# myscale/MyScaleDB

Hardware: NVIDIA B200
Metric: QPS @ recall@10>=0.95 (exact: recall 1.0), FLAT brute-force IP top-10, 10M x 768-d bf16, batch 1024 (higher is better)
Workload: dtype bf16

## Files before the change

include/b200_search.h:

```cpp
#ifndef B200_SEARCH_H
#define B200_SEARCH_H

#include <stddef.h>
#include <stdint.h>

#ifdef __cplusplus
extern "C" {
#endif

#define B200_OK 0
#define B200_ERR_INVALID 1
#define B200_ERR_CUDA 2
#define B200_ERR_UNSUPPORTED 3
#define B200_ERR_NO_DEVICE 4
#define B200_ERR_NOMEM 5
#define B200_ERR_NOT_FOUND 6

#define B200_METRIC_L2 0
#define B200_METRIC_IP 1
#define B200_METRIC_COSINE 2
#define B200_METRIC_HAMMING 3
#define B200_METRIC_JACCARD 4

#define B200_DTYPE_F32 0
#define B200_DTYPE_BF16 1
#define B200_DTYPE_BIN 2

const char *b200_last_error(void);
const char *b200_version(void);
int b200_device_count(int *out_n);
int b200_set_device(int device);

int b200_flat_knn(int metric, const float *x, int64_t nx, const float *y, int64_t ny, int d, int k,
                  const uint8_t *alive_bits , float *out_dis, int64_t *out_ids);

int b200_binary_knn(int metric, const uint8_t *x, int64_t nx, const uint8_t *y, int64_t ny, int nbytes, int k,
                    const uint8_t *alive_bits , float *out_dis, int64_t *out_ids);

int b200_part_scan(int metric, const void *x, int64_t nx, const void *y, int64_t ny, int d, int k,
                   int64_t block_rows, const uint8_t *row_exists , const uint8_t *filter_bits ,
                   float *out_dis, int64_t *out_ids);

typedef struct b200_corpus b200_corpus;

int b200_corpus_create(int metric, int dtype, int d, int64_t capacity_rows, b200_corpus **out);
int b200_corpus_append(b200_corpus *c, const void *rows, int64_t n);
int b200_corpus_adopt_device(b200_corpus *c, const void *device_rows, int64_t n);
int b200_corpus_size(const b200_corpus *c, int64_t *out_rows);
int b200_corpus_free(b200_corpus *c);

int b200_corpus_search(b200_corpus *c, const float *queries, int64_t nq, int k, const uint8_t *alive_bits ,
                       float *out_dis, int64_t *out_ids);
int b200_corpus_search_device(b200_corpus *c, const float *d_queries, int64_t nq, int k,
                              const uint8_t *d_alive_bits , int64_t id_offset, float *d_out_dis,
                              int64_t *d_out_ids, void *stream);
int b200_corpus_set_path(b200_corpus *c, int path);
#define B200_KERNEL_SCAN 1
#define B200_KERNEL_GEMM_BF16 2
#define B200_KERNEL_GEMM_TS 3
#define B200_KERNEL_GEMM_TF32X3 4
int b200_corpus_last_variant(b200_corpus *c, int *kernel, int *cta_group, int *pairs_per_cluster, int *grid);
int b200_corpus_enable_timing(b200_corpus *c, int on);
int b200_corpus_kernel_time(b200_corpus *c, int reset, double *out_total_ms, int64_t *out_launches);
int64_t b200_launch_count(int reset);
int b200_thread_release(void);

int b200_topk_merge_device(const float *d_dis, const int64_t *d_ids, int n_lists, int64_t nq, int k, int descending,
                           float *d_out_dis, int64_t *d_out_ids, void *stream);

int b200_topk_merge_device_strided(const float *d_dis, const int64_t *d_ids, int n_lists, int64_t dis_list_stride,
                                   int64_t ids_list_stride, int64_t nq, int k, int descending, float *d_out_dis,
                                   int64_t *d_out_ids, void *stream);
int b200_topk_merge_device_ex(const float *d_dis, const int64_t *d_ids, int n_lists, int64_t dis_list_stride,
                              int64_t ids_list_stride, int64_t nq, int k_in, int k, int descending, int tie_mode,
                              float *d_out_dis, int64_t *d_out_ids, int32_t *d_out_list , void *stream);

typedef struct b200_index b200_index;
int b200_index_create(const char *type, int metric, int d, const char *params, b200_index **out);
int b200_index_build(b200_index *ix, const float *rows, int64_t n);
int b200_index_reserve(b200_index *ix, int64_t total_rows);
int b200_index_train(b200_index *ix, const float *rows, int64_t n);
int b200_index_train_device(b200_index *ix, const float *d_rows, int64_t n);
int b200_index_add(b200_index *ix, const float *rows, int64_t n);
int b200_index_add_device(b200_index *ix, const float *d_rows, int64_t n);
int b200_index_finalize(b200_index *ix);
int b200_index_info(const b200_index *ix, int64_t *n, int *nlist, int *m, int *uses_ivf);
int b200_index_search(b200_index *ix, const float *queries, int64_t nq, int k, const char *params, int first_stage_only,
                      const uint8_t *alive_bits , float *out_dis, int64_t *out_ids, int64_t *out_num_candidates);
int b200_index_search_device(b200_index *ix, const float *d_queries, int64_t nq, int k, const char *params, int first_stage_only,
                             const uint8_t *d_alive_bits , int64_t id_offset, float *d_out_dis, int64_t *d_out_ids,
                             void *stream);
int b200_index_phase_ms(b200_index *ix, double out_ms[5]);
int b200_index_list_sizes(const b200_index *ix, uint32_t *out_sizes , int capacity);
int b200_index_enable_timing(b200_index *ix, int on);
int b200_index_last_scan(b200_index *ix, int64_t *rows_streamed, int64_t *payload_row_bytes, int64_t *work_items,
                         double *kernel_ms_total, int64_t *kernel_launches, int reset);
int b200_index_refine(b200_index *ix, const float *queries, int64_t nq, const int64_t *cand_ids, int64_t ncand, int k,
                      float *out_dis, int64_t *out_ids);
int b200_index_save(b200_index *ix, const char *path);
int b200_index_load(const char *path, b200_index **out);
int b200_index_save_cb(b200_index *ix, int (*write)(void *ctx, const void *data, size_t bytes), void *ctx);
int b200_index_load_cb(int (*read)(void *ctx, void *data, size_t bytes), void *ctx, b200_index **out);
int b200_index_free(b200_index *ix);

typedef struct b200_comm b200_comm;
int b200_comm_unique_id(const char *nccl_lib_path , void *out_id_128_bytes);
int b200_comm_create(const char *nccl_lib_path , const void *unique_id_128_bytes, int rank, int world, b200_comm **out);
int b200_comm_info(const b200_comm *c, int *rank, int *world);
int b200_comm_free(b200_comm *c);
int b200_comm_local_buffers(b200_comm *c, int64_t nq, int k, float **d_dis, int64_t **d_ids);
int b200_comm_gather_merge(b200_comm *c, int64_t nq, int k, int descending, float *d_out_dis, int64_t *d_out_ids, void *stream);
int b200_comm_gather_merge_host(b200_comm *c, const float *h_dis, const int64_t *h_ids, int64_t nq, int k, int descending,
                                float *h_out_dis, int64_t *h_out_ids);
int b200_comm_allreduce_sum_u64(b200_comm *c, uint64_t *host_counters, int64_t n);
int b200_sharded_corpus_search(b200_comm *cm, b200_corpus *corpus, const float *d_queries, int64_t nq, int k,
                               const uint8_t *d_alive_bits , int64_t id_offset, float *d_out_dis, int64_t *d_out_ids,
                               void *stream, int use_graph);
int b200_sharded_corpus_search_host(b200_comm *cm, b200_corpus *corpus, const float *queries, int64_t nq, int d, int k,
                                    int64_t id_offset, float *out_dis, int64_t *out_ids, void *stream, int use_graph);
int b200_sharded_index_search(b200_comm *cm, b200_index *ix, int metric, const float *d_queries, int64_t nq, int k, const char *params,
                              const uint8_t *d_alive_bits , int64_t id_offset, float *d_out_dis, int64_t *d_out_ids,
                              void *stream);

#define B200_CACHE_CORPUS 0
#define B200_CACHE_INDEX 1
#define B200_CACHE_BM25 2
#define B200_CACHE_OPAQUE 3
int b200_cache_set_capacity(uint64_t bytes);
int b200_cache_get(const char *key, void **handle, int *kind);
int b200_cache_put(const char *key, int kind, void *handle, uint64_t bytes, void **resident);
int b200_cache_put_opaque(const char *key, void *handle, uint64_t bytes, void (*deleter)(void *), void **resident);
int b200_cache_release_handle(const char *key, const void *handle);
int b200_cache_release(const char *key);
int b200_cache_expire(const char *key);
int b200_cache_expire_prefix(const char *prefix, int64_t *out_removed);
int b200_cache_stats(uint64_t *capacity, uint64_t *used, uint64_t *items, uint64_t *hits, uint64_t *misses,
                     uint64_t *evictions);
int b200_corpus_memory_bytes(const b200_corpus *c, uint64_t *out_bytes);
int b200_index_memory_bytes(const b200_index *ix, uint64_t *out_bytes);

int b200_bitmap_from_offsets_device(const uint64_t *d_offsets, int64_t n, int64_t nbits, uint8_t *d_out_bits, void *stream);
int b200_bitmap_from_row_exists_device(const uint8_t *d_row_exists, int64_t n, uint8_t *d_out_bits, void *stream);
int b200_bitmap_and_device(const uint8_t *d_a, const uint8_t *d_b, int64_t nbits, uint8_t *d_out, void *stream);
int b200_bitmap_and(const uint8_t *a, const uint8_t *b, int64_t nbits, uint8_t *out);
int b200_real_bitmap(const uint8_t *filter_bits, int64_t n_new_rows, const uint64_t *inverted_row_ids_map,
                     const uint8_t *inverted_row_sources_map, uint32_t own_id, int64_t total_vec, uint8_t *out_bits);
int b200_remap_labels(const uint64_t *row_ids_map, int64_t map_len, int64_t *labels, int64_t n);
int b200_transfer_to_old_row_ids(const int64_t *new_ids, const float *new_dis, int64_t num_candidates,
                                 const uint64_t *inverted_row_ids_map, const uint8_t *inverted_row_sources_map, int64_t map_len,
                                 uint32_t own_id, int64_t *out_ids, float *out_dis, int64_t *out_n);

typedef struct b200_bm25 b200_bm25;
int b200_bm25_create(uint32_t n_fields, b200_bm25 **out);
int b200_bm25_free(b200_bm25 *ix);
int b200_bm25_add_doc(b200_bm25 *ix, uint64_t row_id);
int b200_bm25_add_text(b200_bm25 *ix, uint32_t field, const char *text);
int b200_bm25_commit(b200_bm25 *ix);
int b200_bm25_save(b200_bm25 *ix, const char *path);
int b200_bm25_load(const char *path, b200_bm25 **out);
int b200_bm25_total_docs(const b200_bm25 *ix, uint64_t *out);
int b200_bm25_total_tokens(const b200_bm25 *ix, uint32_t field, uint64_t *out);
int b200_bm25_doc_freq(const b200_bm25 *ix, uint32_t field, const char *term, uint64_t *out);
int b200_bm25_query_terms(const char *sentence, char *buf, size_t buf_len, uint32_t *out_n);
int b200_bm25_search(b200_bm25 *ix, const char *sentence, const uint32_t *fields, uint32_t n_fields_q, uint32_t topk,
                     const uint8_t *alive_bits , int use_filter, int operator_or, uint64_t stat_total_docs,
                     const uint64_t *stat_total_tokens, const uint64_t *stat_doc_freq, uint64_t *out_rows,
                     float *out_scores, uint32_t *out_n);
int b200_bm25_last_timing(b200_bm25 *ix, double *kernel_ms, double *call_ms, uint64_t *postings);
int b200_bm25_search_batch(b200_bm25 *ix, const char *const *sentences, int64_t nq, const uint32_t *fields,
                           uint32_t n_fields_q, uint32_t topk, const uint8_t *alive_bits, int use_filter, int operator_or,
                           uint64_t stat_total_docs, const uint64_t *stat_total_tokens, const uint64_t *stat_doc_freq,
                           uint64_t *out_rows , float *out_scores, uint32_t *out_counts );

int b200_hybrid_fusion_batch(int fusion_type, int64_t nq, const uint32_t *vec_shard, const uint64_t *vec_part,
                             const uint64_t *vec_label, const float *vec_score, const uint32_t *vec_count, int64_t vec_stride,
                             const uint32_t *txt_shard, const uint64_t *txt_part, const uint64_t *txt_label,
                             const float *txt_score, const uint32_t *txt_count, int64_t txt_stride, float fusion_weight,
                             uint64_t fusion_k, int vector_scan_direction, uint32_t top_k, uint32_t *out_shard,
                             uint64_t *out_part, uint64_t *out_label, float *out_score, uint32_t *out_count);

#ifdef __cplusplus
}
#endif
#endif
```

myscaledb_b200/csrc/capi.cu:

```cuda
#include <algorithm>
#include <cstdlib>
#include <cstring>
#include <mutex>
#include <vector>

#include "common.cuh"
#include "kernels.h"

namespace b200 {

thread_local std::string g_error;
thread_local int64_t g_launches = 0;

void set_error(const std::string &msg) { g_error = msg; }
int fail(int code, const std::string &msg) {
    g_error = msg;
    return code;
}

static int ensure_device() {
    int n = 0;
    cudaError_t e = cudaGetDeviceCount(&n);
    if (e != cudaSuccess || n == 0) {
        cudaGetLastError();
        return fail(B200_ERR_NO_DEVICE, std::string("no CUDA device visible (") +
                                            (e != cudaSuccess ? cudaGetErrorString(e) : "count = 0") +
                                            "); libb200search has no CPU fallback");
    }
    int dev = 0;
    B200_CUDA_OK(cudaGetDevice(&dev));
    int major = 0;
    B200_CUDA_OK(cudaDeviceGetAttribute(&major, cudaDevAttrComputeCapabilityMajor, dev));
    if (major != 10)
        return fail(B200_ERR_NO_DEVICE, "device compute capability major is " + std::to_string(major) +
                                            "; this library carries sm_100a code only");
    return B200_OK;
}

static int num_sms() {
    int dev = 0, n = 148;
    if (cudaGetDevice(&dev) == cudaSuccess) cudaDeviceGetAttribute(&n, cudaDevAttrMultiProcessorCount, dev);
    return n;
}

struct DevBuf {
    void *p = nullptr;
    size_t cap = 0;
    int reserve(size_t bytes) {
        if (bytes <= cap) return B200_OK;
        if (p) cudaFree(p);
        p = nullptr;
        cap = 0;
        size_t want = bytes + bytes / 4 + 256;
        cudaError_t e = cudaMalloc(&p, want);
        if (e != cudaSuccess) {
            cudaGetLastError();
            return fail(B200_ERR_NOMEM, "cudaMalloc(" + std::to_string(want) + ") failed: " + cudaGetErrorString(e));
        }
        cap = want;
        return B200_OK;
    }
    void release() {
        if (p) cudaFree(p);
        p = nullptr;
        cap = 0;
    }
    template <typename T>
    T *as() {
        return reinterpret_cast<T *>(p);
    }
};

}

using namespace b200;

struct b200_corpus {
    int metric = 0, dtype = 0, d = 0, d_pad = 0;
    int64_t cap = 0, n = 0;
    int64_t row_bytes = 0;
    void *data = nullptr;
    size_t data_cap_bytes = 0;
    int64_t side_cap_rows = 0;
    bool owns = true;
    float *row_scale = nullptr;
    float *row_bias = nullptr;
    int device = 0;
    int path = 0;
    int gemm_cta_group = 0;
    int sms = 148;
    cudaStream_t stream = nullptr;
    std::mutex mu;
    DevBuf w_raw, w_q32, w_qbf, w_qlo, w_qnorm, w_pk, w_pi, w_lk, w_li, w_alive, w_odis, w_oids, w_stage, w_prog;
    int sync_slack = 2;
    void *h_pin = nullptr;
    size_t h_pin_bytes = 0;
    unsigned int *d_tickets = nullptr;
    unsigned int fused_seq = 0;
    int d_tickets_d = 0;
    int fused_enabled = 1;
    int rescore_l2 = 1;
    int gemm_multicast = 1;
    int gemm_ts = 0;
    int last_cg = 0, last_mc = 0, last_ts = 0, last_grid = 0, last_kernel = 0;
    bool timing = false;
    std::vector<std::pair<cudaEvent_t, cudaEvent_t>> ev_used, ev_free;
    double timed_ms = 0;
    int64_t timed_launches = 0;
};

static void timing_begin(b200_corpus *c, cudaStream_t s, std::pair<cudaEvent_t, cudaEvent_t> &ev) {
    if (!c->timing) return;
    if (c->ev_free.empty()) {
        cudaEventCreate(&ev.first);
        cudaEventCreate(&ev.second);
    } else {
        ev = c->ev_free.back();
        c->ev_free.pop_back();
    }
    cudaEventRecord(ev.first, s);
}
static void timing_drain(b200_corpus *c) {
    for (auto &ev : c->ev_used) {
        float ms = 0;
        if (cudaEventSynchronize(ev.second) == cudaSuccess && cudaEventElapsedTime(&ms, ev.first, ev.second) == cudaSuccess) {
            c->timed_ms += ms;
            c->timed_launches++;
        }
        c->ev_free.push_back(ev);
    }
    c->ev_used.clear();
}
static void timing_end(b200_corpus *c, cudaStream_t s, std::pair<cudaEvent_t, cudaEvent_t> &ev) {
    if (!c->timing) return;
    cudaEventRecord(ev.second, s);
    c->ev_used.push_back(ev);
    if (c->ev_used.size() >= 1024) timing_drain(c);
}

static int corpus_alloc(b200_corpus *c, int64_t rows);
static int corpus_norms(b200_corpus *c, int64_t first, int64_t n);

namespace b200 {
int corpus_metric(const b200_corpus *c) { return c->metric; }
bool corpus_timing_enabled(const b200_corpus *c) { return c->timing; }
const void *corpus_device_rows(const b200_corpus *c) { return c->data; }
int corpus_append_device(b200_corpus *c, const float *d_rows, int64_t n, cudaStream_t s) {
    if (!c || (!d_rows && n > 0) || n < 0) return fail(B200_ERR_INVALID, "bad arguments");
    if (c->dtype == B200_DTYPE_BIN) return fail(B200_ERR_UNSUPPORTED, "device append: float corpora only");
    if (n == 0) return B200_OK;
    std::lock_guard<std::mutex> lk(c->mu);
    B200_CUDA_OK(cudaSetDevice(c->device));
    B200_TRY(corpus_alloc(c, std::max(c->n + n, c->cap)));
    char *dst = reinterpret_cast<char *>(c->data) + c->n * c->row_bytes;
    if (c->dtype == B200_DTYPE_BF16) B200_CUDA_OK(launch_f32_to_bf16_rows(d_rows, c->d, dst, c->d_pad, n, s));
    else B200_CUDA_OK(launch_pad_rows_f32(d_rows, c->d, reinterpret_cast<float *>(dst), c->d_pad, n, s));
    B200_CUDA_OK(cudaStreamSynchronize(s));
    B200_TRY(corpus_norms(c, c->n, n));
    B200_CUDA_OK(cudaStreamSynchronize(c->stream));
    c->n += n;
    return B200_OK;
}
int corpus_normalize_rows(b200_corpus *c) {
    if (c->dtype != B200_DTYPE_F32) return fail(B200_ERR_UNSUPPORTED, "normalise: fp32 corpora only");
    B200_CUDA_OK(cudaSetDevice(c->device));
    B200_CUDA_OK(launch_normalize_rows_f32(reinterpret_cast<float *>(c->data), c->d_pad, c->n, c->stream));
    B200_CUDA_OK(cudaStreamSynchronize(c->stream));
    return B200_OK;
}
}

static bool is_float_metric(int m) { return m == B200_METRIC_L2 || m == B200_METRIC_IP || m == B200_METRIC_COSINE; }
static bool is_bin_metric(int m) { return m == B200_METRIC_HAMMING || m == B200_METRIC_JACCARD; }

static int pad_for(int dtype, int d) {
    if (dtype == B200_DTYPE_BF16) return (int)round_up(d, 64);
    if (dtype == B200_DTYPE_F32) return (int)round_up(d, 4);
    return d / 8;
}

extern "C" const char *b200_last_error(void) { return g_error.c_str(); }
extern "C" const char *b200_version(void) { return "b200search 0.1 (sm_100a)"; }

extern "C" int b200_device_count(int *out_n) {
    if (!out_n) return fail(B200_ERR_INVALID, "out_n is null");
    int n = 0;
    if (cudaGetDeviceCount(&n) != cudaSuccess) {
        cudaGetLastError();
        n = 0;
    }
    *out_n = n;
    return B200_OK;
}

extern "C" int b200_set_device(int device) {
    B200_TRY(ensure_device());
    B200_CUDA_OK(cudaSetDevice(device));
    return B200_OK;
}

extern "C" int64_t b200_launch_count(int reset) {
    int64_t v = g_launches;
    if (reset) g_launches = 0;
    return v;
}

extern "C" int b200_corpus_create(int metric, int dtype, int d, int64_t capacity_rows, b200_corpus **out) {
    if (!out) return fail(B200_ERR_INVALID, "out is null");
    *out = nullptr;
    if (d <= 0 || capacity_rows < 0) return fail(B200_ERR_INVALID, "bad d / capacity");
    if (dtype == B200_DTYPE_BIN) {
        if (!is_bin_metric(metric)) return fail(B200_ERR_INVALID, "binary corpus needs HAMMING or JACCARD");
        if (d % 8) return fail(B200_ERR_INVALID, "binary dimension must be a multiple of 8 bits");
    } else if (dtype == B200_DTYPE_F32 || dtype == B200_DTYPE_BF16) {
        if (!is_float_metric(metric)) return fail(B200_ERR_INVALID, "float corpus needs L2, IP or COSINE");
    } else {
        return fail(B200_ERR_INVALID, "unknown dtype");
    }
    B200_TRY(ensure_device());
    b200_corpus *c = new b200_corpus();
    c->metric = metric;
    c->dtype = dtype;
    c->d = d;
    c->d_pad = pad_for(dtype, d);
    c->row_bytes = dtype == B200_DTYPE_BIN ? c->d_pad : (int64_t)c->d_pad * (dtype == B200_DTYPE_BF16 ? 2 : 4);
    c->cap = capacity_rows;
    cudaGetDevice(&c->device);
    c->sms = num_sms();
    if (const char *ev = getenv("B200_GEMM_SYNC_SLACK")) c->sync_slack = atoi(ev);
    if (const char *ev = getenv("B200_GEMM_RESCORE_L2")) c->rescore_l2 = atoi(ev);
    if (const char *ev = getenv("B200_FUSED_SCAN")) c->fused_enabled = atoi(ev);
    if (const char *ev = getenv("B200_GEMM_TS")) c->gemm_ts = atoi(ev);
    if (const char *ev = getenv("B200_GEMM_MULTICAST")) c->gemm_multicast = atoi(ev);
    cudaError_t e = cudaStreamCreateWithFlags(&c->stream, cudaStreamNonBlocking);
    if (e != cudaSuccess) {
        delete c;
        return fail(B200_ERR_CUDA, std::string("cudaStreamCreate: ") + cudaGetErrorString(e));
    }
    *out = c;
    return B200_OK;
}

static int corpus_alloc(b200_corpus *c, int64_t rows) {
    if (c->data && !c->owns) return fail(B200_ERR_INVALID, "corpus adopted device memory; cannot append");
    const size_t need = (size_t)(rows + 1) * c->row_bytes + 256;
    const bool want_scale = c->metric == B200_METRIC_COSINE, want_bias = c->metric == B200_METRIC_L2;
    if (!c->data || c->data_cap_bytes < need) {
        void *nd = nullptr;
        cudaError_t e = cudaMalloc(&nd, need);
        if (e != cudaSuccess) {
            cudaGetLastError();
            return fail(B200_ERR_NOMEM, std::string("cudaMalloc corpus: ") + cudaGetErrorString(e));
        }
        if (c->data && c->n) {
            cudaMemcpyAsync(nd, c->data, (size_t)c->n * c->row_bytes, cudaMemcpyDeviceToDevice, c->stream);
            cudaStreamSynchronize(c->stream);
        }
        if (c->data) cudaFree(c->data);
        c->data = nd;
        c->data_cap_bytes = need;
    }
    if ((want_scale && (!c->row_scale || c->side_cap_rows < rows)) || (want_bias && (!c->row_bias || c->side_cap_rows < rows))) {
        float *ns = nullptr, *nb = nullptr;
        if (want_scale && cudaMalloc(&ns, (size_t)rows * 4 + 256) != cudaSuccess) return fail(B200_ERR_NOMEM, "cudaMalloc row_scale");
        if (want_bias && cudaMalloc(&nb, (size_t)rows * 4 + 256) != cudaSuccess) return fail(B200_ERR_NOMEM, "cudaMalloc row_bias");
        if (c->n) {
            if (ns && c->row_scale) cudaMemcpyAsync(ns, c->row_scale, (size_t)c->n * 4, cudaMemcpyDeviceToDevice, c->stream);
            if (nb && c->row_bias) cudaMemcpyAsync(nb, c->row_bias, (size_t)c->n * 4, cudaMemcpyDeviceToDevice, c->stream);
            cudaStreamSynchronize(c->stream);
        }
        if (c->row_scale) cudaFree(c->row_scale);
        if (c->row_bias) cudaFree(c->row_bias);
        c->row_scale = ns;
        c->row_bias = nb;
        c->side_cap_rows = rows;
    }
    c->cap = std::max(c->cap, rows);
    c->owns = true;
    return B200_OK;
}

static int corpus_norms(b200_corpus *c, int64_t first, int64_t n) {
    const char *rows = reinterpret_cast<const char *>(c->data) + first * c->row_bytes;
    if (c->metric == B200_METRIC_COSINE)
        B200_CUDA_OK(launch_row_norms(rows, c->dtype == B200_DTYPE_BF16, c->d_pad, n, 1, c->row_scale + first, c->stream));
    if (c->metric == B200_METRIC_L2)
        B200_CUDA_OK(launch_row_norms(rows, c->dtype == B200_DTYPE_BF16, c->d_pad, n, 0, c->row_bias + first, c->stream));
    return B200_OK;
}

extern "C" int b200_corpus_append(b200_corpus *c, const void *rows, int64_t n) {
    if (!c || (!rows && n > 0) || n < 0) return fail(B200_ERR_INVALID, "bad arguments");
    if (n == 0) return B200_OK;
    std::lock_guard<std::mutex> lk(c->mu);
    B200_CUDA_OK(cudaSetDevice(c->device));
    B200_TRY(corpus_alloc(c, std::max(c->n + n, c->cap)));
    char *dst = reinterpret_cast<char *>(c->data) + c->n * c->row_bytes;
    if (c->dtype == B200_DTYPE_BIN || (c->dtype == B200_DTYPE_F32 && c->d == c->d_pad)) {
        B200_TRY(staged_h2d(dst, rows, (size_t)n * c->row_bytes, c->device, c->stream));
    } else {
        const int64_t chunk = std::max<int64_t>(1, (int64_t)(256ll << 20) / ((int64_t)c->d * 4));
        for (int64_t off = 0; off < n; off += chunk) {
            const int64_t m = std::min(chunk, n - off);
            B200_TRY(c->w_raw.reserve((size_t)m * c->d * 4));
            B200_TRY(staged_h2d(c->w_raw.p, reinterpret_cast<const float *>(rows) + off * c->d, (size_t)m * c->d * 4, c->device,
                                c->stream));
            char *dd = dst + off * c->row_bytes;
            if (c->dtype == B200_DTYPE_BF16)
                B200_CUDA_OK(launch_f32_to_bf16_rows(c->w_raw.as<float>(), c->d, dd, c->d_pad, m, c->stream));
            else
                B200_CUDA_OK(launch_pad_rows_f32(c->w_raw.as<float>(), c->d, reinterpret_cast<float *>(dd), c->d_pad, m, c->stream));
            B200_CUDA_OK(cudaStreamSynchronize(c->stream));
        }
    }
    if (c->dtype != B200_DTYPE_BIN) B200_TRY(corpus_norms(c, c->n, n));
    B200_CUDA_OK(cudaStreamSynchronize(c->stream));
    c->n += n;
    return B200_OK;
}

extern "C" int b200_corpus_memory_bytes(const b200_corpus *c, uint64_t *out_bytes) {
    if (!c || !out_bytes) return fail(B200_ERR_INVALID, "bad arguments");
    uint64_t b = c->owns ? (uint64_t)c->data_cap_bytes : (uint64_t)c->n * (uint64_t)c->row_bytes;
    if (c->row_scale) b += (uint64_t)std::max(c->side_cap_rows, c->n) * 4;
    if (c->row_bias) b += (uint64_t)std::max(c->side_cap_rows, c->n) * 4;
    *out_bytes = b;
    return B200_OK;
}

extern "C" int b200_corpus_adopt_device(b200_corpus *c, const void *device_rows, int64_t n) {
    if (!c || !device_rows || n < 0) return fail(B200_ERR_INVALID, "bad arguments");
    std::lock_guard<std::mutex> lk(c->mu);
    if (c->data) return fail(B200_ERR_INVALID, "corpus already holds data");
    if (c->dtype != B200_DTYPE_BIN && c->d != c->d_pad)
        return fail(B200_ERR_INVALID, "adopted rows must already be padded (d % 64 == 0 for bf16, d % 4 == 0 for f32)");
    B200_CUDA_OK(cudaSetDevice(c->device));
    c->data = const_cast<void *>(device_rows);
    c->owns = false;
    c->n = n;
    c->cap = n;
    if (c->metric == B200_METRIC_COSINE) B200_CUDA_OK(cudaMalloc(&c->row_scale, (size_t)n * 4 + 256));
    if (c->metric == B200_METRIC_L2) B200_CUDA_OK(cudaMalloc(&c->row_bias, (size_t)n * 4 + 256));
    c->side_cap_rows = n;
    if (c->dtype != B200_DTYPE_BIN) B200_TRY(corpus_norms(c, 0, n));
    B200_CUDA_OK(cudaStreamSynchronize(c->stream));
    return B200_OK;
}

extern "C" int b200_corpus_size(const b200_corpus *c, int64_t *out_rows) {
    if (!c || !out_rows) return fail(B200_ERR_INVALID, "null argument");
    *out_rows = c->n;
    return B200_OK;
}

namespace b200 {
int list_cap_for(int k) {
    static const int min_k = getenv("B200_LIST_APPEND_MIN_K") ? atoi(getenv("B200_LIST_APPEND_MIN_K")) : 0;
    static const int tourn_k = getenv("B200_LIST_TOURN_MIN_K") ? atoi(getenv("B200_LIST_TOURN_MIN_K")) : 17;
    if (min_k > 0 && k >= min_k) return list_cap_append(k);
    if (tourn_k > 0 && k >= tourn_k) return list_cap_tourn(k);
    return k;
}
}

extern "C" int b200_corpus_set_path(b200_corpus *c, int path) {
    if (!c || path < 0 || path > 7) return fail(B200_ERR_INVALID, "path must be 0..7");
    std::lock_guard<std::mutex> lk(c->mu);
    c->path = path >= 2 ? 2 : path;
    c->gemm_cta_group = path == 3 ? 1 : 0;
    c->gemm_ts = path == 7 ? 2 : 0;
    c->gemm_multicast = path == 4 ? 0 : path == 5 ? 2 : 1;
    if (path == 0) {
        if (const char *ev = getenv("B200_GEMM_TS")) c->gemm_ts = atoi(ev);
        if (const char *ev = getenv("B200_GEMM_MULTICAST")) c->gemm_multicast = atoi(ev);
    }
    return B200_OK;
}

extern "C" int b200_corpus_last_variant(b200_corpus *c, int *kernel, int *cta_group, int *pairs_per_cluster, int *grid) {
    if (!c) return fail(B200_ERR_INVALID, "null corpus");
    std::lock_guard<std::mutex> lk(c->mu);
    if (kernel) *kernel = c->last_kernel;
    if (cta_group) *cta_group = c->last_cg;
    if (pairs_per_cluster) *pairs_per_cluster = c->last_mc;
    if (grid) *grid = c->last_grid;
    return B200_OK;
}

extern "C" int b200_corpus_enable_timing(b200_corpus *c, int on) {
    if (!c) return fail(B200_ERR_INVALID, "null corpus");
    std::lock_guard<std::mutex> lk(c->mu);
    c->timing = on != 0;
    return B200_OK;
}

extern "C" int b200_corpus_kernel_time(b200_corpus *c, int reset, double *out_total_ms, int64_t *out_launches) {
    if (!c || !out_total_ms || !out_launches) return fail(B200_ERR_INVALID, "null argument");
    std::lock_guard<std::mutex> lk(c->mu);
    B200_CUDA_OK(cudaSetDevice(c->device));
    timing_drain(c);
    *out_total_ms = c->timed_ms;
    *out_launches = c->timed_launches;
    if (reset) {
        c->timed_ms = 0;
        c->timed_launches = 0;
    }
    return B200_OK;
}

extern "C" int b200_corpus_free(b200_corpus *c) {
    if (!c) return B200_OK;
    cudaSetDevice(c->device);
    if (c->stream) cudaStreamSynchronize(c->stream);
    if (c->data && c->owns) cudaFree(c->data);
    if (c->row_scale) cudaFree(c->row_scale);
    if (c->row_bias) cudaFree(c->row_bias);
    if (c->h_pin) cudaFreeHost(c->h_pin);
    if (c->d_tickets) cudaFree(c->d_tickets);
    for (DevBuf *b : {&c->w_raw, &c->w_q32, &c->w_qbf, &c->w_qlo, &c->w_qnorm, &c->w_pk, &c->w_pi, &c->w_lk, &c->w_li, &c->w_alive,
                      &c->w_odis, &c->w_oids, &c->w_stage, &c->w_prog})
        b->release();
    for (auto *v : {&c->ev_used, &c->ev_free})
        for (auto &ev : *v) {
            cudaEventDestroy(ev.first);
            cudaEventDestroy(ev.second);
        }
    if (c->stream) cudaStreamDestroy(c->stream);
    delete c;
    return B200_OK;
}

static int search_core(b200_corpus *c, const void *d_queries, int64_t nq, int k, const uint8_t *d_alive, int64_t id_offset,
                       int ip_min_quirk, float *d_out_dis, int64_t *d_out_ids, cudaStream_t s) {
    if (k <= 0) return fail(B200_ERR_INVALID, "k must be positive");
    if (nq == 0) return B200_OK;
    if (c->n >= (int64_t)0xffffffffll) return fail(B200_ERR_UNSUPPORTED, "corpus shards are limited to 2^32 - 1 rows");
    const int sms = c->sms;

    if (c->dtype == B200_DTYPE_BIN) {
        if (k > 1024) return fail(B200_ERR_UNSUPPORTED, "k > 1024 not supported on the binary scan path");
        int blocks_x = (int)std::min<int64_t>(std::max<int64_t>(1, ceil_div(c->n, 256)), std::max<int64_t>(1, (2 * sms) / std::max<int64_t>(1, std::min<int64_t>(nq, 2 * sms))));
        B200_TRY(c->w_pk.reserve((size_t)nq * blocks_x * k * 4));
        B200_TRY(c->w_pi.reserve((size_t)nq * blocks_x * k * 4));
        BinaryScanParams bp{};
        bp.corpus = reinterpret_cast<const uint8_t *>(c->data);
        bp.queries = reinterpret_cast<const uint8_t *>(d_queries);
        bp.alive = d_alive;
        bp.part_keys = c->w_pk.as<float>();
        bp.part_ids = c->w_pi.as<uint32_t>();
        bp.n = c->n;
        bp.nq = nq;
        bp.nbytes = c->d_pad;
        bp.k = k;
        bp.jaccard = c->metric == B200_METRIC_JACCARD;
        B200_CUDA_OK(launch_binary_scan(bp, blocks_x, s));
        MergeParams mp{};
        mp.in_keys = bp.part_keys;
        mp.in_ids = bp.part_ids;
        mp.list_stride = k;
        mp.q_stride = (int64_t)blocks_x * k;
        mp.n_lists = blocks_x;
        mp.k_in = k;
        mp.k = k;
        mp.nq = nq;
        mp.out_mode = kOutKey;
        mp.id_offset = id_offset;
        mp.out_dis = d_out_dis;
        mp.out_ids = d_out_ids;
        B200_CUDA_OK(launch_topk_merge(mp, false, s));
        return B200_OK;
    }

    B200_TRY(c->w_q32.reserve((size_t)nq * c->d_pad * 4));
    float *q32 = c->w_q32.as<float>();
    B200_CUDA_OK(launch_pad_rows_f32(reinterpret_cast<const float *>(d_queries), c->d, q32, c->d_pad, nq, s));
    int path = c->path;
    if (path == 0) {
        const int64_t min_nq = c->metric == B200_METRIC_L2 ? 20 : (c->dtype == B200_DTYPE_BF16 ? 2 : 5);
        path = (nq >= min_nq && k <= (c->dtype == B200_DTYPE_BF16 ? 1024 : 256)) ? 2 : 1;
    }
    if (c->n == 0) path = 1;
    if (c->metric == B200_METRIC_COSINE && path == 1) B200_CUDA_OK(launch_normalize_rows_f32(q32, c->d_pad, nq, s));

    const int out_mode_scan = c->metric == B200_METRIC_L2 ? kOutKey : c->metric == B200_METRIC_IP ? kOutNeg : kOutOnePlus;

    if (path == 1) {
        if (k > 2048) return fail(B200_ERR_UNSUPPORTED, "k > 2048 not supported on the scan path");
        int qt = nq == 1 ? 1 : nq <= 4 ? 4 : 8;
        while (qt > 1 && scan_smem_bytes(qt, c->d_pad, k) > 100 * 1024) qt = qt == 8 ? 4 : 1;
        if (scan_smem_bytes(qt, c->d_pad, k) > 200 * 1024)
            return fail(B200_ERR_UNSUPPORTED, "d * 4 + 64 * k exceeds the shared-memory budget of the scan kernel");
        const int elems = c->dtype == B200_DTYPE_BF16 ? 8 : 4;
        const int chunks = c->d_pad / elems;
        int group = 1;
        while (group < 32 && group < chunks) group <<= 1;
        const int64_t y_tiles = ceil_div(nq, qt);
        const int64_t rows_per_block_step = 8 * (32 / group);
        int64_t bx = std::max<int64_t>(1, (2 * sms) / std::min<int64_t>(y_tiles, 2 * sms));
        bx = std::min<int64_t>(bx, std::max<int64_t>(1, ceil_div(c->n, rows_per_block_step)));
        const int blocks_x = (int)bx;
        B200_TRY(c->w_pk.reserve((size_t)nq * blocks_x * k * 4));
        B200_TRY(c->w_pi.reserve((size_t)nq * blocks_x * k * 4));
        ScanParams sp{};
        sp.corpus = c->data;
        sp.queries = q32;
        sp.row_scale = c->metric == B200_METRIC_COSINE ? c->row_scale : nullptr;
        sp.alive = d_alive;
        sp.part_keys = c->w_pk.as<float>();
        sp.part_ids = c->w_pi.as<uint32_t>();
        sp.n = c->n;
        sp.nq = nq;
        sp.row_bytes = c->row_bytes;
        sp.d_pad = c->d_pad;
        sp.k = k;
        sp.group = group;
        sp.l2 = c->metric == B200_METRIC_L2;
        sp.bf16 = c->dtype == B200_DTYPE_BF16;
        std::pair<cudaEvent_t, cudaEvent_t> ev;
        timing_begin(c, s, ev);
        B200_CUDA_OK(launch_flat_scan(sp, qt, blocks_x, s));
        timing_end(c, s, ev);
        c->last_kernel = B200_KERNEL_SCAN; c->last_cg = 0; c->last_mc = 0; c->last_grid = blocks_x;
        MergeParams mp{};
        mp.in_keys = sp.part_keys;
        mp.in_ids = sp.part_ids;
        mp.list_stride = k;
        mp.q_stride = (int64_t)blocks_x * k;
        mp.n_lists = blocks_x;
        mp.k_in = k;
        mp.k = k;
        mp.nq = nq;
        mp.out_mode = out_mode_scan;
        mp.ip_min_quirk = ip_min_quirk && c->metric == B200_METRIC_IP;
        mp.id_offset = id_offset;
        mp.out_dis = d_out_dis;
        mp.out_ids = d_out_ids;
        B200_CUDA_OK(launch_topk_merge(mp, false, s));
        return B200_OK;
    }

    if (k > 1024) return fail(B200_ERR_UNSUPPORTED, "k > 1024 not supported on the GEMM path");
    const int64_t QCHUNK = 1024;
    for (int64_t qb = 0; qb < nq; qb += QCHUNK) {
        const int64_t nq_c = std::min(QCHUNK, nq - qb);
        const bool f32 = c->dtype == B200_DTYPE_F32;
        const int cta_group = (nq_c > 128 && c->gemm_cta_group != 1) ? 2 : 1;
        const int nq_pad = (int)round_up(nq_c, 128 * cta_group);
        const int q_tiles = nq_pad / 128;
        if (f32) {
            B200_TRY(c->w_qbf.reserve((size_t)nq_pad * c->d_pad * 4));
            B200_TRY(c->w_qlo.reserve((size_t)nq_pad * c->d_pad * 4));
            B200_CUDA_OK(launch_split_tf32(q32 + qb * c->d_pad, nq_c, c->d_pad, c->w_qbf.as<float>(), c->w_qlo.as<float>(), nq_pad, s));
        } else {
            B200_TRY(c->w_qbf.reserve((size_t)nq_pad * c->d_pad * 2));
            B200_CUDA_OK(cudaMemsetAsync(c->w_qbf.p, 0, (size_t)nq_pad * c->d_pad * 2, s));
            B200_CUDA_OK(launch_f32_to_bf16_rows(q32 + qb * c->d_pad, c->d_pad, c->w_qbf.p, c->d_pad, nq_c, s));
        }
        const float *q_add = nullptr;
        if (c->metric == B200_METRIC_L2 || c->metric == B200_METRIC_COSINE) {
            B200_TRY(c->w_qnorm.reserve((size_t)nq_pad * 4));
            if (f32)
                B200_CUDA_OK(launch_row_norms(q32 + qb * c->d_pad, 0, c->d_pad, nq_c, c->metric == B200_METRIC_L2 ? 0 : 1,
                                              c->w_qnorm.as<float>(), s));
            else
                B200_CUDA_OK(launch_row_norms(c->w_qbf.p, 1, c->d_pad, nq_c, c->metric == B200_METRIC_L2 ? 0 : 1,
                                              c->w_qnorm.as<float>(), s));
            q_add = c->w_qnorm.as<float>();
        }
        int pairs = 1;
        if (cta_group == 2 && c->gemm_multicast && !f32) {
            const int want = c->gemm_multicast == 1 ? 4 : c->gemm_multicast;
            if (want >= 4 && q_tiles % 8 == 0) pairs = 4;
            else if (want >= 2 && q_tiles % 4 == 0) pairs = 2;
        }
        int grid = gemm_topk_grid(q_tiles, c->n, sms);
        while (pairs > 1) {
            const int maxc = gemm_topk_max_clusters(2, pairs, k);
            const int groups = q_tiles / (2 * pairs);
            const int per_group = maxc / groups;
            if (per_group >= 1) {
                grid = std::min(grid, per_group * groups * 2 * pairs);
                break;
            }
            pairs /= 2;
        }
        grid = (grid / q_tiles) * q_tiles;
        if (grid < q_tiles) grid = q_tiles;
        B200_TRY(c->w_pk.reserve((size_t)grid * 128 * k * 4));
        B200_TRY(c->w_pi.reserve((size_t)grid * 128 * k * 4));
        GemmTopkParams gp{};
        gp.corpus_bf16 = c->data;
        gp.queries_bf16 = c->w_qbf.p;
        gp.queries_lo = f32 ? c->w_qlo.p : nullptr;
        gp.row_scale = c->metric == B200_METRIC_COSINE ? c->row_scale : nullptr;
        gp.scale_const = c->metric == B200_METRIC_L2 ? -2.f : -1.f;
        gp.row_bias = c->metric == B200_METRIC_L2 ? c->row_bias : nullptr;
        gp.alive = d_alive;
        gp.part_keys = c->w_pk.as<float>();
        gp.part_ids = c->w_pi.as<uint32_t>();
        {
            B200_TRY(c->w_lk.reserve((size_t)grid * 128 * list_cap_for(k) * 4));
            B200_TRY(c->w_li.reserve((size_t)grid * 128 * list_cap_for(k) * 4));
            gp.list_keys_gmem = c->w_lk.as<float>();
            gp.list_ids_gmem = c->w_li.as<uint32_t>();
        }
        gp.n = c->n;
        gp.nq_pad = nq_pad;
        gp.nq_valid = (int)nq_c;
        gp.d_pad = c->d_pad;
        gp.k = k;
        gp.q_tiles = q_tiles;
        gp.cta_group = cta_group;
        gp.pairs_per_cluster = pairs;
        if (const char *dv = getenv("B200_GEMM_DEBUG")) gp.debug = atoi(dv);
        if (q_tiles > cta_group && c->sync_slack > 0) {
            B200_TRY(c->w_prog.reserve((size_t)grid * 4));
            B200_CUDA_OK(cudaMemsetAsync(c->w_prog.p, 0, (size_t)grid * 4, s));
            gp.progress = c->w_prog.as<int>();
            gp.sync_slack = c->sync_slack;
        }
        const char *detail = nullptr;
        std::pair<cudaEvent_t, cudaEvent_t> ev;
        timing_begin(c, s, ev);
        const bool use_ts = !f32 && cta_group == 2 && k <= 30 && gemm_topk_ts_supported(c->d_pad, q_tiles) &&
                            (c->gemm_ts == 2 || (c->gemm_ts == 1 && c->d_pad <= 512));
        cudaError_t e = f32 ? launch_gemm3_topk(gp, grid, s, &detail)
                            : use_ts ? launch_gemm_topk_ts(gp, grid, s, &detail) : launch_gemm_topk(gp, grid, s, &detail);
        timing_end(c, s, ev);
        c->last_kernel = f32 ? B200_KERNEL_GEMM_TF32X3 : use_ts ? B200_KERNEL_GEMM_TS : B200_KERNEL_GEMM_BF16;
        c->last_cg = cta_group; c->last_mc = (f32 || use_ts) ? 1 : pairs; c->last_grid = grid;
        if (e != cudaSuccess)
            return fail(B200_ERR_CUDA, std::string("gemm_topk launch: ") + (detail ? detail : cudaGetErrorString(e)));
        MergeParams mp{};
        mp.in_keys = gp.part_keys;
        mp.in_ids = gp.part_ids;
        mp.list_stride = (int64_t)nq_pad * k;
        mp.q_stride = k;
        mp.n_lists = grid / q_tiles;
        mp.k_in = k;
        mp.k = k;
        mp.nq = nq_c;
        mp.out_mode = c->metric == B200_METRIC_L2 ? kOutAddQ : c->metric == B200_METRIC_IP ? kOutNeg : kOutCosQ;
        mp.q_add = q_add;
        mp.ip_min_quirk = ip_min_quirk && c->metric == B200_METRIC_IP;
        mp.id_offset = id_offset;
        mp.out_dis = d_out_dis + qb * k;
        mp.out_ids = d_out_ids + qb * k;
        B200_CUDA_OK(launch_topk_merge(mp, false, s));
        if (c->metric == B200_METRIC_L2 && k <= 1024 && c->rescore_l2)
            B200_CUDA_OK(launch_rescore_l2(c->data, c->dtype == B200_DTYPE_BF16, c->row_bytes, c->d_pad, q32 + qb * c->d_pad, nq_c, id_offset, k,
                                           d_out_dis + qb * k, d_out_ids + qb * k, s));
    }
    return B200_OK;
}

extern "C" int b200_corpus_search_device(b200_corpus *c, const float *d_queries, int64_t nq, int k,
                                         const uint8_t *d_alive_bits, int64_t id_offset, float *d_out_dis,
                                         int64_t *d_out_ids, void *stream) {
    if (!c || (!d_queries && nq > 0) || !d_out_dis || !d_out_ids || nq < 0)
        return fail(B200_ERR_INVALID, "bad arguments");
    std::lock_guard<std::mutex> lk(c->mu);
    B200_CUDA_OK(cudaSetDevice(c->device));
    cudaStream_t s = stream ? reinterpret_cast<cudaStream_t>(stream) : c->stream;
    B200_TRY(search_core(c, d_queries, nq, k, d_alive_bits, id_offset, 0, d_out_dis, d_out_ids, s));
    if (!stream) B200_CUDA_OK(cudaStreamSynchronize(s));
    return B200_OK;
}

static int search_host_fused(b200_corpus *c, const float *queries, int64_t nq, int k, const uint8_t *alive_bits, int ip_min_quirk,
                             float *out_dis, int64_t *out_ids, bool *done) {
    *done = false;
    if (!c->fused_enabled || c->dtype == B200_DTYPE_BIN || nq > 8 || k > 1024 || c->n == 0) return B200_OK;
    int path = c->path;
    if (path == 0) {
        const int64_t min_nq = c->metric == B200_METRIC_L2 ? 20 : (c->dtype == B200_DTYPE_BF16 ? 2 : 5);
        path = (nq >= min_nq) ? 2 : 1;
    }
    if (path != 1) return B200_OK;
    int qt = nq == 1 ? 1 : nq <= 4 ? 4 : 8;
    while (qt > 1 && scan_smem_bytes(qt, c->d_pad, k) > 100 * 1024) qt = qt == 8 ? 4 : 1;
    if (scan_smem_bytes(qt, c->d_pad, k) > 200 * 1024) return B200_OK;
    cudaStream_t s = c->stream;
    const size_t need = (size_t)8 * c->d * 4 + (size_t)8 * k * 12 + 64;
    if (need > c->h_pin_bytes) {
        if (c->h_pin) cudaFreeHost(c->h_pin);
        c->h_pin = nullptr;
        c->h_pin_bytes = 0;
        if (cudaHostAlloc(&c->h_pin, need, cudaHostAllocMapped) != cudaSuccess) {
            cudaGetLastError();
            return B200_OK;
        }
        c->h_pin_bytes = need;
    }
    if (!c->d_tickets || c->d_tickets_d != c->d) {
        if (c->d_tickets) cudaFree(c->d_tickets);
        c->d_tickets = nullptr;
        B200_CUDA_OK(cudaMalloc(&c->d_tickets, 64 + (size_t)8 * c->d * 4));
        B200_CUDA_OK(cudaMemsetAsync(c->d_tickets, 0, 64, s));
        c->d_tickets_d = c->d;
    }
    float *d_q = reinterpret_cast<float *>(reinterpret_cast<char *>(c->d_tickets) + 64);
    char *hp = reinterpret_cast<char *>(c->h_pin);
    float *h_q = reinterpret_cast<float *>(hp);
    float *h_dis = reinterpret_cast<float *>(hp + (size_t)8 * c->d * 4);
    int64_t *h_ids = reinterpret_cast<int64_t *>(hp + (size_t)8 * c->d * 4 + (size_t)round_up(8 * k * 4, 8));
    volatile unsigned int *h_flag = reinterpret_cast<volatile unsigned int *>(hp + need - 16);
    void *dp = nullptr;
    B200_CUDA_OK(cudaHostGetDevicePointer(&dp, c->h_pin, 0));
    char *dpc = reinterpret_cast<char *>(dp);
    const bool q_inline = nq * c->d <= 256;
    if (!q_inline) {
        memcpy(h_q, queries, (size_t)nq * c->d * 4);
        B200_CUDA_OK(cudaMemcpyAsync(d_q, h_q, (size_t)nq * c->d * 4, cudaMemcpyHostToDevice, s));
    }
    const uint8_t *d_alive = nullptr;
    if (alive_bits) {
        const size_t ab = (size_t)ceil_div(c->n, 8);
        B200_TRY(c->w_alive.reserve(ab + 16));
        B200_CUDA_OK(cudaMemcpyAsync(c->w_alive.p, alive_bits, ab, cudaMemcpyHostToDevice, s));
        d_alive = c->w_alive.as<uint8_t>();
    }
    const int elems = c->dtype == B200_DTYPE_BF16 ? 8 : 4;
    const int chunks = c->d_pad / elems;
    int group = 1;
    while (group < 32 && group < chunks) group <<= 1;
    const int64_t y_tiles = ceil_div(nq, qt);
    const int64_t rows_per_block_step = 8 * (32 / group);
    int64_t bx = std::max<int64_t>(1, (2 * c->sms) / std::min<int64_t>(y_tiles, 2 * c->sms));
    bx = std::min<int64_t>(bx, std::max<int64_t>(1, ceil_div(c->n, rows_per_block_step)));
    const int blocks_x = (int)bx;
    B200_TRY(c->w_pk.reserve((size_t)nq * blocks_x * k * 4));
    B200_TRY(c->w_pi.reserve((size_t)nq * blocks_x * k * 4));
    ScanParams sp{};
    sp.corpus = c->data;
    sp.queries = d_q;
    sp.row_scale = c->metric == B200_METRIC_COSINE ? c->row_scale : nullptr;
    sp.alive = d_alive;
    sp.part_keys = c->w_pk.as<float>();
    sp.part_ids = c->w_pi.as<uint32_t>();
    sp.n = c->n;
    sp.nq = nq;
    sp.row_bytes = c->row_bytes;
    sp.d_pad = c->d_pad;
    sp.k = k;
    sp.group = group;
    sp.l2 = c->metric == B200_METRIC_L2;
    sp.bf16 = c->dtype == B200_DTYPE_BF16;
    sp.fused = 1;
    sp.q_dim = c->d;
    sp.cosine = c->metric == B200_METRIC_COSINE;
    sp.out_mode = c->metric == B200_METRIC_L2 ? kOutKey : c->metric == B200_METRIC_IP ? kOutNeg : kOutOnePlus;
    sp.ip_min_quirk = ip_min_quirk && c->metric == B200_METRIC_IP;
    sp.id_offset = 0;
    sp.tickets = c->d_tickets;
    sp.tiles_done = c->d_tickets + 8;
    sp.out_dis = reinterpret_cast<float *>(dpc + (reinterpret_cast<char *>(h_dis) - hp));
    sp.out_ids = reinterpret_cast<int64_t *>(dpc + (reinterpret_cast<char *>(h_ids) - hp));
    sp.done_flag = reinterpret_cast<volatile unsigned int *>(dpc + need - 16);
    sp.done_value = ++c->fused_seq ? c->fused_seq : ++c->fused_seq;
    sp.q_inline = q_inline ? 1 : 0;
    if (q_inline) memcpy(sp.qinline, queries, (size_t)nq * c->d * 4);
    static unsigned long long *dbg_ts = nullptr;
    static const bool dbg_on = getenv("B200_FUSED_DEBUG_TS") && atoi(getenv("B200_FUSED_DEBUG_TS"));
    if (dbg_on && !dbg_ts) cudaMallocManaged(&dbg_ts, 16 * sizeof(unsigned long long));
    sp.debug_ts = dbg_on ? dbg_ts : nullptr;
    *h_flag = 0;
    std::pair<cudaEvent_t, cudaEvent_t> ev;
    timing_begin(c, s, ev);
    B200_CUDA_OK(launch_flat_scan(sp, qt, blocks_x, s));
    timing_end(c, s, ev);
    c->last_kernel = B200_KERNEL_SCAN; c->last_cg = 0; c->last_mc = 0; c->last_grid = blocks_x;
    for (uint64_t spin = 1;; spin++) {
        if (*h_flag == sp.done_value) break;
        if ((spin & 0x3fff) == 0) {
            const cudaError_t qe = cudaStreamQuery(s);
            if (qe == cudaSuccess) {
                if (*h_flag == sp.done_value) break;
                return fail(B200_ERR_CUDA, "fused scan finished without publishing its result");
            }
            if (qe != cudaErrorNotReady) return fail(B200_ERR_CUDA, std::string("fused scan: ") + cudaGetErrorString(qe));
        }
#if defined(__x86_64__)
        __builtin_ia32_pause();
#endif
    }
    if (dbg_on && (c->fused_seq & 63) == 0) {
        cudaStreamSynchronize(s);
        fprintf(stderr, "fused ts (us since block 0 start): scan_done %.1f tail_start %.1f fence %.1f staged %.1f bounds %.1f compacted %.1f lists %.1f merged %.1f written %.1f sysfence %.1f survivors %llu\n",
                (dbg_ts[1] - dbg_ts[0]) * 1e-3, (dbg_ts[2] - dbg_ts[0]) * 1e-3, (dbg_ts[3] - dbg_ts[0]) * 1e-3, (dbg_ts[4] - dbg_ts[0]) * 1e-3,
                (dbg_ts[5] - dbg_ts[0]) * 1e-3, (dbg_ts[6] - dbg_ts[0]) * 1e-3, (dbg_ts[7] - dbg_ts[0]) * 1e-3, (dbg_ts[8] - dbg_ts[0]) * 1e-3,
                (dbg_ts[9] - dbg_ts[0]) * 1e-3, (dbg_ts[10] - dbg_ts[0]) * 1e-3, dbg_ts[15]);
    }
    memcpy(out_dis, h_dis, (size_t)nq * k * 4);
    memcpy(out_ids, h_ids, (size_t)nq * k * 8);
    *done = true;
    return B200_OK;
}

static int search_host(b200_corpus *c, const void *queries, int64_t nq, int k, const uint8_t *alive_bits, int ip_min_quirk,
                       float *out_dis, int64_t *out_ids) {
    if (!c || (!queries && nq > 0) || !out_dis || !out_ids || nq < 0 || k <= 0)
        return fail(B200_ERR_INVALID, "bad arguments");
    if (nq == 0) return B200_OK;
    std::lock_guard<std::mutex> lk(c->mu);
    B200_CUDA_OK(cudaSetDevice(c->device));
    {
        bool done = false;
        B200_TRY(search_host_fused(c, reinterpret_cast<const float *>(queries), nq, k, alive_bits, ip_min_quirk, out_dis, out_ids, &done));
        if (done) return B200_OK;
    }
    cudaStream_t s = c->stream;
    const size_t q_bytes = c->dtype == B200_DTYPE_BIN ? (size_t)nq * c->d_pad : (size_t)nq * c->d * 4;
    B200_TRY(c->w_stage.reserve(q_bytes));
    B200_TRY(c->w_odis.reserve((size_t)nq * k * 4));
    B200_TRY(c->w_oids.reserve((size_t)nq * k * 8));
    B200_CUDA_OK(cudaMemcpyAsync(c->w_stage.p, queries, q_bytes, cudaMemcpyHostToDevice, s));
    const uint8_t *d_alive = nullptr;
    if (alive_bits) {
        const size_t ab = (size_t)ceil_div(c->n, 8);
        B200_TRY(c->w_alive.reserve(ab + 16));
        B200_CUDA_OK(cudaMemcpyAsync(c->w_alive.p, alive_bits, ab, cudaMemcpyHostToDevice, s));
        d_alive = c->w_alive.as<uint8_t>();
    }
    B200_TRY(search_core(c, c->w_stage.p, nq, k, d_alive, 0, ip_min_quirk, c->w_odis.as<float>(), c->w_oids.as<int64_t>(), s));
    B200_CUDA_OK(cudaMemcpyAsync(out_dis, c->w_odis.p, (size_t)nq * k * 4, cudaMemcpyDeviceToHost, s));
    B200_CUDA_OK(cudaMemcpyAsync(out_ids, c->w_oids.p, (size_t)nq * k * 8, cudaMemcpyDeviceToHost, s));
    B200_CUDA_OK(cudaStreamSynchronize(s));
    return B200_OK;
}

extern "C" int b200_corpus_search(b200_corpus *c, const float *queries, int64_t nq, int k, const uint8_t *alive_bits,
                                  float *out_dis, int64_t *out_ids) {
    return search_host(c, queries, nq, k, alive_bits, 0, out_dis, out_ids);
}

struct ScratchCorpus {
    b200_corpus *c = nullptr;
    ~ScratchCorpus() {
        if (c) b200_corpus_free(c);
    }
};
static thread_local ScratchCorpus t_scratch;

extern "C" int b200_thread_release(void) {
    if (t_scratch.c) {
        b200_corpus_free(t_scratch.c);
        t_scratch.c = nullptr;
    }
    return B200_OK;
}

static int scratch_corpus(int metric, int dtype, int d, int64_t rows, b200_corpus **out) {
    b200_corpus *c = t_scratch.c;
    int dev = 0;
    cudaGetDevice(&dev);
    if (c && (c->device != dev || !c->owns)) {
        b200_corpus_free(c);
        c = t_scratch.c = nullptr;
    }
    if (!c) {
        B200_TRY(b200_corpus_create(metric, dtype, d, rows, &c));
        t_scratch.c = c;
        *out = c;
        return B200_OK;
    }
    c->metric = metric;
    c->dtype = dtype;
    c->d = d;
    c->d_pad = pad_for(dtype, d);
    c->row_bytes = dtype == B200_DTYPE_BIN ? c->d_pad : (int64_t)c->d_pad * (dtype == B200_DTYPE_BF16 ? 2 : 4);
    c->n = 0;
    c->cap = 0;
    c->path = 0;
    (void)rows;
    *out = c;
    return B200_OK;
}

static void fill_empty(int metric, int64_t n, float *dis, int64_t *ids, int quirk) {
    for (int64_t i = 0; i < n; i++) {
        ids[i] = -1;
        dis[i] = quirk ? FLT_MIN : (metric == B200_METRIC_IP ? -FLT_MAX : FLT_MAX);
    }
}

extern "C" int b200_flat_knn(int metric, const float *x, int64_t nx, const float *y, int64_t ny, int d, int k,
                             const uint8_t *alive_bits, float *out_dis, int64_t *out_ids) {
    if (!is_float_metric(metric)) return fail(B200_ERR_INVALID, "b200_flat_knn: metric must be L2, IP or COSINE");
    if (nx < 0 || ny < 0 || d <= 0 || k <= 0 || !out_dis || !out_ids) return fail(B200_ERR_INVALID, "bad arguments");
    B200_TRY(ensure_device());
    if (nx == 0) return B200_OK;
    if (ny == 0) {
        fill_empty(metric, nx * k, out_dis, out_ids, 0);
        return B200_OK;
    }
    b200_corpus *c = nullptr;
    B200_TRY(scratch_corpus(metric, B200_DTYPE_F32, d, ny, &c));
    int rc = b200_corpus_append(c, y, ny);
    if (rc == B200_OK) rc = search_host(c, x, nx, k, alive_bits, 0, out_dis, out_ids);
    return rc;
}

extern "C" int b200_binary_knn(int metric, const uint8_t *x, int64_t nx, const uint8_t *y, int64_t ny, int nbytes, int k,
                               const uint8_t *alive_bits, float *out_dis, int64_t *out_ids) {
    if (!is_bin_metric(metric)) return fail(B200_ERR_INVALID, "b200_binary_knn: metric must be HAMMING or JACCARD");
    if (nx < 0 || ny < 0 || nbytes <= 0 || k <= 0 || !out_dis || !out_ids) return fail(B200_ERR_INVALID, "bad arguments");
    B200_TRY(ensure_device());
    if (nx == 0) return B200_OK;
    if (ny == 0) {
        fill_empty(metric, nx * k, out_dis, out_ids, 0);
        return B200_OK;
    }
    b200_corpus *c = nullptr;
    B200_TRY(scratch_corpus(metric, B200_DTYPE_BIN, nbytes * 8, ny, &c));
    int rc = b200_corpus_append(c, y, ny);
    if (rc == B200_OK) rc = search_host(c, x, nx, k, alive_bits, 0, out_dis, out_ids);
    return rc;
}

extern "C" int b200_part_scan(int metric, const void *x, int64_t nx, const void *y, int64_t ny, int d, int k,
                              int64_t block_rows, const uint8_t *row_exists, const uint8_t *filter_bits, float *out_dis,
                              int64_t *out_ids) {
    (void)block_rows;
    if (nx < 0 || ny < 0 || d <= 0 || k <= 0 || !out_dis || !out_ids) return fail(B200_ERR_INVALID, "bad arguments");
    if (!is_float_metric(metric) && !is_bin_metric(metric)) return fail(B200_ERR_INVALID, "unknown metric");
    B200_TRY(ensure_device());
    if (nx == 0) return B200_OK;
    const int quirk = metric == B200_METRIC_IP;
    if (ny == 0) {
        fill_empty(metric, nx * k, out_dis, out_ids, quirk);
        return B200_OK;
    }
    std::vector<uint8_t> alive;
    const uint8_t *alive_ptr = filter_bits;
    if (!filter_bits && row_exists) {
        alive.assign((size_t)ceil_div(ny, 8), 0);
        for (int64_t i = 0; i < ny; i++)
            if (row_exists[i]) alive[i >> 3] |= (uint8_t)(1u << (i & 7));
        alive_ptr = alive.data();
    }
    b200_corpus *c = nullptr;
    const bool bin = is_bin_metric(metric);
    B200_TRY(scratch_corpus(metric, bin ? B200_DTYPE_BIN : B200_DTYPE_F32, d, ny, &c));
    int rc = b200_corpus_append(c, y, ny);
    if (rc == B200_OK) rc = search_host(c, x, nx, k, alive_ptr, quirk, out_dis, out_ids);
    return rc;
}

extern "C" int b200_topk_merge_device(const float *d_dis, const int64_t *d_ids, int n_lists, int64_t nq, int k,
                                      int descending, float *d_out_dis, int64_t *d_out_ids, void *stream) {
    return b200_topk_merge_device_strided(d_dis, d_ids, n_lists, nq * k, nq * k, nq, k, descending, d_out_dis, d_out_ids,
                                          stream);
}

extern "C" int b200_topk_merge_device_strided(const float *d_dis, const int64_t *d_ids, int n_lists,
                                              int64_t dis_list_stride, int64_t ids_list_stride, int64_t nq, int k,
                                              int descending, float *d_out_dis, int64_t *d_out_ids, void *stream) {
    return b200_topk_merge_device_ex(d_dis, d_ids, n_lists, dis_list_stride, ids_list_stride, nq, k, k, descending, 0, d_out_dis,
                                     d_out_ids, nullptr, stream);
}

extern "C" int b200_topk_merge_device_ex(const float *d_dis, const int64_t *d_ids, int n_lists, int64_t dis_list_stride,
                                         int64_t ids_list_stride, int64_t nq, int k_in, int k, int descending, int tie_mode,
                                         float *d_out_dis, int64_t *d_out_ids, int32_t *d_out_list, void *stream) {
    if (!d_dis || !d_ids || !d_out_dis || !d_out_ids || n_lists <= 0 || nq < 0 || k <= 0 || k_in <= 0 || tie_mode < 0 || tie_mode > 1)
        return fail(B200_ERR_INVALID, "bad arguments");
    if (k > 2048) return fail(B200_ERR_UNSUPPORTED, "k > 2048 not supported by the merge kernel");
    B200_TRY(ensure_device());
    if (nq == 0) return B200_OK;
    MergeParams mp{};
    mp.in_keys = d_dis;
    mp.in_ids = d_ids;
    mp.list_stride = dis_list_stride;
    mp.id_list_stride = ids_list_stride;
    mp.q_stride = k_in;
    mp.n_lists = n_lists;
    mp.k_in = k_in;
    mp.k = k;
    mp.nq = nq;
    mp.descending = descending;
    mp.tie_mode = tie_mode;
    mp.out_list = d_out_list;
    mp.out_dis = d_out_dis;
    mp.out_ids = d_out_ids;
    cudaStream_t s = reinterpret_cast<cudaStream_t>(stream);
    B200_CUDA_OK(launch_topk_merge(mp, true, s));
    if (!stream) B200_CUDA_OK(cudaStreamSynchronize(s));
    return B200_OK;
}
```

myscaledb_b200/csrc/gemm_common.cuh:

```cuda
#pragma once
#include <cuda.h>

#include "common.cuh"
#include "kernels.h"

namespace b200 {
namespace gemm {


constexpr int BM = 128;
constexpr int BN = 256;
constexpr int BK = 64;
constexpr int ACC_STAGES = 2;
constexpr int UMMA_K = 16;
constexpr int A_BYTES = BM * BK * 2;
constexpr int NUM_THREADS = 192;
constexpr int EPI_THREADS = 128;
constexpr int TMEM_COLS = 512;
constexpr int SMEM_ALIGN_SLACK = 1024;
constexpr int MAX_STAGES = 6;

constexpr int SCRATCH_BYTES = 32 * EPI_THREADS * 4;

template <int CG>
struct Cfg {
    static constexpr int B_ROWS = BN / CG;
    static constexpr int B_BYTES = B_ROWS * BK * 2;
    static constexpr int STAGE_BYTES = A_BYTES + B_BYTES;
    static constexpr int TX_BYTES = STAGE_BYTES * CG;
    __host__ __device__ static constexpr int off_a() { return 0; }
    __host__ __device__ static constexpr int off_b(int stages) { return stages * A_BYTES; }
    __host__ __device__ static constexpr int off_side(int stages) { return stages * STAGE_BYTES; }
    __host__ __device__ static constexpr int off_bar(int stages) { return off_side(stages) + 2 * BN * 4; }
    __host__ __device__ static constexpr int off_scratch(int stages) { return off_bar(stages) + 256; }
    __host__ __device__ static constexpr int off_list(int stages) { return off_scratch(stages) + SCRATCH_BYTES; }
    __host__ __device__ static int stages_for(int k_smem) {
        const int max_stages = CG == 1 ? 4 : 6;
        int st = max_stages;
        while (st > 2 && off_list(st) + k_smem * EPI_THREADS * 8 + SMEM_ALIGN_SLACK > 232448) st--;
        return st;
    }
    __host__ __device__ static bool lists_fit(int k) {
        return off_list(2) + k * EPI_THREADS * 8 + SMEM_ALIGN_SLACK <= 232448;
    }
};

__device__ __forceinline__ void mbar_init(uint64_t *bar, uint32_t count) {
    asm volatile("mbarrier.init.shared::cta.b64 [%0], %1;" ::"r"(smem_u32(bar)), "r"(count));
}
__device__ __forceinline__ void mbar_arrive_expect_tx(uint64_t *bar, uint32_t bytes) {
    asm volatile("mbarrier.arrive.expect_tx.shared::cta.b64 _, [%0], %1;" ::"r"(smem_u32(bar)), "r"(bytes) : "memory");
}
__device__ __forceinline__ void mbar_arrive(uint64_t *bar) {
    asm volatile("mbarrier.arrive.shared::cta.b64 _, [%0];" ::"r"(smem_u32(bar)) : "memory");
}
__device__ __forceinline__ bool mbar_try_wait(uint32_t addr, uint32_t parity) {
    uint32_t ok;
    asm volatile(
        "{\n\t"
        ".reg .pred p;\n\t"
        "mbarrier.try_wait.parity.shared::cta.b64 p, [%1], %2;\n\t"
        "selp.u32 %0, 1, 0, p;\n\t"
        "}\n"
        : "=r"(ok)
        : "r"(addr), "r"(parity)
        : "memory");
    return ok != 0;
}
#ifndef B200_MBAR_BACKOFF_NS
#define B200_MBAR_BACKOFF_NS 0
#endif
__device__ __forceinline__ void mbar_wait(uint64_t *bar, uint32_t parity) {
    const uint32_t addr = smem_u32(bar);
    while (!mbar_try_wait(addr, parity)) {
#if B200_MBAR_BACKOFF_NS > 0
        __nanosleep(B200_MBAR_BACKOFF_NS);
#endif
    }
}

__device__ __forceinline__ void tma_load_2d(const CUtensorMap *map, uint64_t *bar, void *dst, int c0, int c1) {
    asm volatile(
        "cp.async.bulk.tensor.2d.shared::cluster.global.mbarrier::complete_tx::bytes [%0], [%1, {%3, %4}], [%2];" ::"r"(
            smem_u32(dst)),
        "l"(reinterpret_cast<uint64_t>(map)), "r"(smem_u32(bar)), "r"(c0), "r"(c1)
        : "memory");
}

__device__ __forceinline__ void tma_load_2d_cg2(const CUtensorMap *map, uint64_t *bar, void *dst, int c0, int c1) {
    asm volatile(
        "cp.async.bulk.tensor.2d.cta_group::2.shared::cluster.global.mbarrier::complete_tx::bytes [%0], [%1, {%3, %4}], "
        "[%2];" ::"r"(smem_u32(dst)),
        "l"(reinterpret_cast<uint64_t>(map)), "r"(smem_u32(bar) & 0xFEFFFFFFu), "r"(c0), "r"(c1)
        : "memory");
}

__device__ __forceinline__ void tma_load_2d_cg2_mc(const CUtensorMap *map, uint64_t *bar, void *dst, int c0, int c1, uint16_t cta_mask) {
    asm volatile(
        "cp.async.bulk.tensor.2d.cta_group::2.shared::cluster.global.mbarrier::complete_tx::bytes.multicast::cluster "
        "[%0], [%1, {%3, %4}], [%2], %5;" ::"r"(smem_u32(dst)),
        "l"(reinterpret_cast<uint64_t>(map)), "r"(smem_u32(bar) & 0xFEFFFFFFu), "r"(c0), "r"(c1), "h"(cta_mask)
        : "memory");
}

__device__ __forceinline__ uint32_t cluster_ctarank() {
    uint32_t r;
    asm volatile("mov.u32 %0, %%cluster_ctarank;" : "=r"(r));
    return r;
}
__device__ __forceinline__ void cluster_sync_all() {
    asm volatile("barrier.cluster.arrive.release.aligned;" ::: "memory");
    asm volatile("barrier.cluster.wait.acquire.aligned;" ::: "memory");
}
__device__ __forceinline__ void mbar_arrive_remote(uint64_t *bar, uint32_t cta) {
    asm volatile(
        "{\n\t"
        ".reg .b32 remote;\n\t"
        "mapa.shared::cluster.u32 remote, %0, %1;\n\t"
        "mbarrier.arrive.shared::cluster.b64 _, [remote];\n\t"
        "}\n" ::"r"(smem_u32(bar)),
        "r"(cta)
        : "memory");
}
__device__ __forceinline__ bool elect_one() {
    uint32_t pred;
    asm volatile(
        "{\n\t"
        ".reg .pred P;\n\t"
        "elect.sync _|P, 0xffffffff;\n\t"
        "selp.b32 %0, 1, 0, P;\n\t"
        "}\n"
        : "=r"(pred));
    return pred != 0;
}

__device__ __forceinline__ uint64_t make_smem_desc(uint32_t smem_addr) {
    uint64_t d = 0;
    d |= (uint64_t)((smem_addr >> 4) & 0x3FFF);
    d |= (uint64_t)1 << 16;
    d |= (uint64_t)(1024 >> 4) << 32;
    d |= (uint64_t)1 << 46;
    d |= (uint64_t)2 << 61;
    return d;
}

__device__ __forceinline__ constexpr uint32_t make_idesc(int cg) {
    return (1u << 4) | (1u << 7) | (1u << 10) | ((uint32_t)(BN >> 3) << 17) | ((uint32_t)((BM * cg) >> 4) << 24);
}

__device__ __forceinline__ void umma(uint32_t tmem_d, uint64_t adesc, uint64_t bdesc, uint32_t idesc, uint32_t accum) {
    asm volatile(
        "{\n\t"
        ".reg .pred p;\n\t"
        "setp.ne.b32 p, %4, 0;\n\t"
        "tcgen05.mma.cta_group::1.kind::f16 [%0], %1, %2, %3, p;\n\t"
        "}\n" ::"r"(tmem_d),
        "l"(adesc), "l"(bdesc), "r"(idesc), "r"(accum)
        : "memory");
}
__device__ __forceinline__ void umma_commit(uint64_t *bar) {
    asm volatile("tcgen05.commit.cta_group::1.mbarrier::arrive::one.shared::cluster.b64 [%0];" ::"r"(smem_u32(bar))
                 : "memory");
}
__device__ __forceinline__ void umma_cg2(uint32_t tmem_d, uint64_t adesc, uint64_t bdesc, uint32_t idesc, uint32_t accum) {
    asm volatile(
        "{\n\t"
        ".reg .pred p;\n\t"
        "setp.ne.b32 p, %4, 0;\n\t"
        "tcgen05.mma.cta_group::2.kind::f16 [%0], %1, %2, %3, p;\n\t"
        "}\n" ::"r"(tmem_d),
        "l"(adesc), "l"(bdesc), "r"(idesc), "r"(accum)
        : "memory");
}
__device__ __forceinline__ void umma_commit_cg2(uint64_t *bar, uint16_t mask = 3) {
    asm volatile(
        "tcgen05.commit.cta_group::2.mbarrier::arrive::one.shared::cluster.multicast::cluster.b64 [%0], %1;" ::"r"(
            smem_u32(bar)),
        "h"(mask)
        : "memory");
}
__device__ __forceinline__ void tc_fence_before() { asm volatile("tcgen05.fence::before_thread_sync;" ::: "memory"); }
__device__ __forceinline__ void tc_fence_after() { asm volatile("tcgen05.fence::after_thread_sync;" ::: "memory"); }

__device__ __forceinline__ void tmem_ld32_issue(uint32_t taddr, float (&v)[32]) {
    asm volatile(
        "tcgen05.ld.sync.aligned.32x32b.x32.b32 "
        "{%0, %1, %2, %3, %4, %5, %6, %7, %8, %9, %10, %11, %12, %13, %14, %15, "
        "%16, %17, %18, %19, %20, %21, %22, %23, %24, %25, %26, %27, %28, %29, %30, %31}, [%32];"
        : "=f"(v[0]), "=f"(v[1]), "=f"(v[2]), "=f"(v[3]), "=f"(v[4]), "=f"(v[5]), "=f"(v[6]), "=f"(v[7]), "=f"(v[8]),
          "=f"(v[9]), "=f"(v[10]), "=f"(v[11]), "=f"(v[12]), "=f"(v[13]), "=f"(v[14]), "=f"(v[15]), "=f"(v[16]),
          "=f"(v[17]), "=f"(v[18]), "=f"(v[19]), "=f"(v[20]), "=f"(v[21]), "=f"(v[22]), "=f"(v[23]), "=f"(v[24]),
          "=f"(v[25]), "=f"(v[26]), "=f"(v[27]), "=f"(v[28]), "=f"(v[29]), "=f"(v[30]), "=f"(v[31])
        : "r"(taddr)
        : "memory");
}
__device__ __forceinline__ void tmem_ld_wait() { asm volatile("tcgen05.wait::ld.sync.aligned;" ::: "memory"); }

struct ThreadTopK {
    float *keys;
    uint32_t *ids;
    int k, n, worst;
    int cap;
    int stride;
    int coop;
    int append;
    int tourn;
    float thr_key;
    uint32_t thr_id;
};

#ifndef B200_LIST_COOP_MIN_K
#define B200_LIST_COOP_MIN_K (1 << 30)
#endif
constexpr int kListCoopMinK = B200_LIST_COOP_MIN_K;
#if B200_LIST_COOP_MIN_K >= (1 << 30)
#define LIST_STRIDE(t) EPI_THREADS
#else
#define LIST_STRIDE(t) ((t).stride)
#endif
__device__ __forceinline__ void list_bind(ThreadTopK &t, float *keys_base, uint32_t *ids_base, int row, int k, int cap) {
    t.k = k;
    t.cap = cap;
    t.append = cap >= 2 * k + 32 ? 1 : 0;
    t.tourn = (!t.append && cap > k && cap == list_cap_tourn(k)) ? 1 : 0;
    t.coop = (cap == k && k >= kListCoopMinK) ? 1 : 0;
    t.stride = t.coop ? 1 : EPI_THREADS;
    t.keys = keys_base + (t.coop ? (size_t)row * cap : (size_t)row);
    t.ids = ids_base + (t.coop ? (size_t)row * cap : (size_t)row);
}


struct ListThr {
    float key;
    uint32_t id;
};

#ifdef B200_LIST_STATS
__device__ unsigned long long g_list_stats[4];
#define B200_LIST_STAT(i, v) atomicAdd(&g_list_stats[i], (unsigned long long)(v))
#else
#define B200_LIST_STAT(i, v)
#endif

static __device__ __noinline__ ListThr list_compact(float *keys, uint32_t *ids, int k, int n, int stride) {
    float lo_k = 0.f, hi_k = 0.f;
    uint32_t lo_i = 0, hi_i = 0;
    bool have_lo = false, have_hi = false;
    float pk = keys[(n - 1) * stride];
    uint32_t pi = ids[(n - 1) * stride];
    uint32_t salt = 0x9E3779B1u;
    for (;;) {
        int rank = 0;
        float ck_lo = 0.f, ck_hi = 0.f;
        uint32_t ci_lo = 0, ci_hi = 0, h_lo = 0xffffffffu, h_hi = 0xffffffffu;
        for (int j = 0; j < n; j++) {
            const float kj = keys[j * stride];
            const uint32_t ij = ids[j * stride];
            const uint32_t h = ((uint32_t)j + 1u) * salt;
            if (better(kj, ij, pk, pi)) {
                rank++;
                if ((!have_lo || better(lo_k, lo_i, kj, ij)) && h <= h_lo) {
                    h_lo = h;
                    ck_lo = kj;
                    ci_lo = ij;
                }
            } else if (better(pk, pi, kj, ij)) {
                if ((!have_hi || better(kj, ij, hi_k, hi_i)) && h <= h_hi) {
                    h_hi = h;
                    ck_hi = kj;
                    ci_hi = ij;
                }
            }
        }
        rank++;
        B200_LIST_STAT(2, 1);
        if (rank == k) break;
        if (rank < k) {
            lo_k = pk; lo_i = pi; have_lo = true;
            pk = ck_hi; pi = ci_hi;
        } else {
            hi_k = pk; hi_i = pi; have_hi = true;
            pk = ck_lo; pi = ci_lo;
        }
        salt = salt * 0x85EBCA6Bu + 0xC2B2AE35u;
        salt |= 1u;
    }
    int dst = 0;
    for (int j = k; j < n; j++) {
        const float kj = keys[j * stride];
        const uint32_t ij = ids[j * stride];
        if (!better(pk, pi, kj, ij)) {
            while (!better(pk, pi, keys[dst * stride], ids[dst * stride])) dst++;
            keys[dst * stride] = kj;
            ids[dst * stride] = ij;
            dst++;
        }
    }
    ListThr r;
    r.key = pk;
    r.id = pi;
    return r;
}

__device__ __forceinline__ void list_compact_if_over(ThreadTopK &t) {
    if (t.n > t.k) {
        const ListThr r = list_compact(t.keys, t.ids, t.k, t.n, LIST_STRIDE(t));
        t.n = t.k;
        t.thr_key = r.key;
        t.thr_id = r.id;
    }
}

__device__ __forceinline__ void list_insert(ThreadTopK &t, float key, uint32_t id) {
    if (!better(key, id, t.thr_key, t.thr_id)) return;
    if (t.append) {
        B200_LIST_STAT(3, 1);
        t.keys[t.n * LIST_STRIDE(t)] = key;
        t.ids[t.n * LIST_STRIDE(t)] = id;
        t.n++;
        return;
    }
    if (t.tourn) {
        const int G = list_tourn_group(t.k);
        const int ng = (t.k + G - 1) / G;
        float *gk = t.keys + (size_t)t.k * LIST_STRIDE(t);
        uint32_t *gi = t.ids + (size_t)t.k * LIST_STRIDE(t);
        if (t.n < t.k) {
            t.keys[t.n * LIST_STRIDE(t)] = key;
            t.ids[t.n * LIST_STRIDE(t)] = id;
            t.n++;
            if (t.n < t.k) return;
            for (int g = 0; g < ng; g++) {
                const int base = g * G, end = base + G < t.k ? base + G : t.k;
                float wk = t.keys[base * LIST_STRIDE(t)];
                uint32_t wi = t.ids[base * LIST_STRIDE(t)];
                for (int j = base + 1; j < end; j++) {
                    const float kj = t.keys[j * LIST_STRIDE(t)];
                    const uint32_t ij = t.ids[j * LIST_STRIDE(t)];
                    if (better(wk, wi, kj, ij)) {
                        wk = kj;
                        wi = ij;
                    }
                }
                gk[g * LIST_STRIDE(t)] = wk;
                gi[g * LIST_STRIDE(t)] = wi;
            }
        } else {
            const int g = t.worst;
            const int base = g * G, end = base + G < t.k ? base + G : t.k;
            float wk = 0.f;
            uint32_t wi = 0;
            int slot = -1;
            bool have = false;
            for (int j = base; j < end; j++) {
                float kj = t.keys[j * LIST_STRIDE(t)];
                uint32_t ij = t.ids[j * LIST_STRIDE(t)];
                if (slot < 0 && kj == t.thr_key && ij == t.thr_id) {
                    slot = j;
                    kj = key;
                    ij = id;
                }
                if (!have || better(wk, wi, kj, ij)) {
                    wk = kj;
                    wi = ij;
                    have = true;
                }
            }
            if (slot < 0) slot = base;
            t.keys[slot * LIST_STRIDE(t)] = key;
            t.ids[slot * LIST_STRIDE(t)] = id;
            gk[g * LIST_STRIDE(t)] = wk;
            gi[g * LIST_STRIDE(t)] = wi;
        }
        float wk = gk[0];
        uint32_t wi = gi[0];
        int wg = 0;
        for (int g = 1; g < ng; g++) {
            const float kg = gk[g * LIST_STRIDE(t)];
            const uint32_t ig = gi[g * LIST_STRIDE(t)];
            if (better(wk, wi, kg, ig)) {
                wk = kg;
                wi = ig;
                wg = g;
            }
        }
        t.worst = wg;
        t.thr_key = wk;
        t.thr_id = wi;
        return;
    }
    if (t.n < t.k) {
        t.keys[t.n * LIST_STRIDE(t)] = key;
        t.ids[t.n * LIST_STRIDE(t)] = id;
        t.n++;
        if (t.n < t.k) return;
    } else {
        t.keys[t.worst * LIST_STRIDE(t)] = key;
        t.ids[t.worst * LIST_STRIDE(t)] = id;
    }
    float wk = t.keys[0];
    uint32_t wi = t.ids[0];
    int wp = 0;
    for (int j = 1; j < t.k; j++) {
        const float kj = t.keys[j * LIST_STRIDE(t)];
        const uint32_t ij = t.ids[j * LIST_STRIDE(t)];
        if (better(wk, wi, kj, ij)) {
            wk = kj;
            wi = ij;
            wp = j;
        }
    }
    t.worst = wp;
    t.thr_key = wk;
    t.thr_id = wi;
}

static __device__ __noinline__ void list_publish(ThreadTopK &t, float *out_keys, uint32_t *out_ids) {
    list_compact_if_over(t);
    for (int i = 1; i < t.n; i++) {
        const float ki = t.keys[i * LIST_STRIDE(t)];
        const uint32_t ii = t.ids[i * LIST_STRIDE(t)];
        int j = i;
        while (j > 0 && better(ki, ii, t.keys[(j - 1) * LIST_STRIDE(t)], t.ids[(j - 1) * LIST_STRIDE(t)])) {
            t.keys[j * LIST_STRIDE(t)] = t.keys[(j - 1) * LIST_STRIDE(t)];
            t.ids[j * LIST_STRIDE(t)] = t.ids[(j - 1) * LIST_STRIDE(t)];
            j--;
        }
        t.keys[j * LIST_STRIDE(t)] = ki;
        t.ids[j * LIST_STRIDE(t)] = ii;
    }
    for (int j = 0; j < t.k; j++) {
        out_keys[j] = j < t.n ? t.keys[j * LIST_STRIDE(t)] : FLT_MAX;
        out_ids[j] = j < t.n ? t.ids[j * LIST_STRIDE(t)] : kNoId;
    }
}

__device__ __forceinline__ void side_fma32(float (&v)[32], const float *scale, const float *bias) {
    const uint32_t sa = smem_u32(scale), ba = smem_u32(bias);
#pragma unroll
    for (int j = 0; j < 32; j += 4) {
        float s0, s1, s2, s3, b0, b1, b2, b3;
        asm volatile("ld.shared.v4.f32 {%0, %1, %2, %3}, [%4];" : "=f"(s0), "=f"(s1), "=f"(s2), "=f"(s3) : "r"(sa + j * 4));
        asm volatile("ld.shared.v4.f32 {%0, %1, %2, %3}, [%4];" : "=f"(b0), "=f"(b1), "=f"(b2), "=f"(b3) : "r"(ba + j * 4));
        v[j] = fmaf(v[j], s0, b0);
        v[j + 1] = fmaf(v[j + 1], s1, b1);
        v[j + 2] = fmaf(v[j + 2], s2, b2);
        v[j + 3] = fmaf(v[j + 3], s3, b3);
    }
}

__device__ __forceinline__ void list_insert_coop(ThreadTopK &t, int src, float key, uint32_t id) {
    const int lane = threadIdx.x & 31;
    key = __shfl_sync(0xffffffffu, key, src);
    id = __shfl_sync(0xffffffffu, id, src);
    const float thr_key = __shfl_sync(0xffffffffu, t.thr_key, src);
    const uint32_t thr_id = __shfl_sync(0xffffffffu, t.thr_id, src);
    if (!better(key, id, thr_key, thr_id)) return;
    const unsigned long long kp = __shfl_sync(0xffffffffu, (unsigned long long)reinterpret_cast<uintptr_t>(t.keys), src);
    const unsigned long long ip = __shfl_sync(0xffffffffu, (unsigned long long)reinterpret_cast<uintptr_t>(t.ids), src);
    float *lk = reinterpret_cast<float *>((uintptr_t)kp);
    uint32_t *li = reinterpret_cast<uint32_t *>((uintptr_t)ip);
    int n = __shfl_sync(0xffffffffu, t.n, src);
    const int k = t.k;
    if (n < k) {
        if (lane == 0) {
            lk[n] = key;
            li[n] = id;
        }
        n++;
        if (n < k) {
            if (lane == src) t.n = n;
            return;
        }
    } else {
        const int worst = __shfl_sync(0xffffffffu, t.worst, src);
        if (lane == 0) {
            lk[worst] = key;
            li[worst] = id;
        }
    }
    __syncwarp();
    float wk = 0.f;
    uint32_t wi = 0;
    int wp = -1;
    for (int j = lane; j < k; j += 32) {
        const float kj = lk[j];
        const uint32_t ij = li[j];
        if (wp < 0 || better(wk, wi, kj, ij)) {
            wk = kj;
            wi = ij;
            wp = j;
        }
    }
#pragma unroll
    for (int o = 16; o > 0; o >>= 1) {
        const float ok = __shfl_xor_sync(0xffffffffu, wk, o);
        const uint32_t oi = __shfl_xor_sync(0xffffffffu, wi, o);
        const int op = __shfl_xor_sync(0xffffffffu, wp, o);
        if (op >= 0 && (wp < 0 || better(wk, wi, ok, oi))) {
            wk = ok;
            wi = oi;
            wp = op;
        }
    }
    if (lane == src) {
        t.n = n;
        t.worst = wp;
        t.thr_key = wk;
        t.thr_id = wi;
    }
    __syncwarp();
}

__device__ __forceinline__ void epilogue_chunk(ThreadTopK &list, float (&v)[32], bool use_side, const float *scale,
                                               const float *bias, uint32_t id0, bool tail, int64_t n, float *scratch,
                                               float ext_bound = FLT_MAX ) {
    float thr = fminf(list.thr_key, ext_bound);
    bool mine;
    if (use_side) {
        side_fma32(v, scale, bias);
        float m0 = fminf(v[0], v[1]), m1 = fminf(v[2], v[3]), m2 = fminf(v[4], v[5]), m3 = fminf(v[6], v[7]);
#pragma unroll
        for (int j = 8; j < 32; j += 8) {
            m0 = fminf(m0, fminf(v[j], v[j + 1]));
            m1 = fminf(m1, fminf(v[j + 2], v[j + 3]));
            m2 = fminf(m2, fminf(v[j + 4], v[j + 5]));
            m3 = fminf(m3, fminf(v[j + 6], v[j + 7]));
        }
        mine = fminf(fminf(m0, m1), fminf(m2, m3)) <= thr;
    } else {
        float m0 = fmaxf(v[0], v[1]), m1 = fmaxf(v[2], v[3]), m2 = fmaxf(v[4], v[5]), m3 = fmaxf(v[6], v[7]);
#pragma unroll
        for (int j = 8; j < 32; j += 8) {
            m0 = fmaxf(m0, fmaxf(v[j], v[j + 1]));
            m1 = fmaxf(m1, fmaxf(v[j + 2], v[j + 3]));
            m2 = fmaxf(m2, fmaxf(v[j + 4], v[j + 5]));
            m3 = fmaxf(m3, fmaxf(v[j + 6], v[j + 7]));
        }
        mine = fmaxf(fmaxf(m0, m1), fmaxf(m2, m3)) >= -thr;
    }
    if (__any_sync(0xffffffffu, mine)) {
        if ((threadIdx.x & 31) == 0) B200_LIST_STAT(0, 1);
        if (list.append && __any_sync(0xffffffffu, list.n + 32 > list.cap)) {
            if ((threadIdx.x & 31) == 0) B200_LIST_STAT(1, 1);
            list_compact_if_over(list);
            thr = fminf(list.thr_key, ext_bound);
        }
        uint32_t mask = 0;
#pragma unroll
        for (int j = 0; j < 32; j++) {
            const float key = use_side ? v[j] : -v[j];
            scratch[j * EPI_THREADS] = key;
            if (key <= thr) mask |= 1u << j;
        }
        if (tail && !use_side) {
            const int64_t left = n - (int64_t)id0;
            mask = left >= 32 ? mask : left <= 0 ? 0u : (mask & ((1u << left) - 1u));
        }
        if (list.coop) {
            unsigned pending = __ballot_sync(0xffffffffu, mask != 0);
            while (pending) {
                const int src = __ffs(pending) - 1;
                float ckey = 0.f;
                uint32_t cid = 0;
                if ((int)(threadIdx.x & 31) == src) {
                    const int j = __ffs(mask) - 1;
                    mask &= mask - 1;
                    ckey = scratch[j * EPI_THREADS];
                    cid = id0 + (uint32_t)j;
                }
                list_insert_coop(list, src, ckey, cid);
                pending = __ballot_sync(0xffffffffu, mask != 0);
            }
        } else {
            while (__any_sync(0xffffffffu, mask != 0)) {
                if (mask) {
                    const int j = __ffs(mask) - 1;
                    mask &= mask - 1;
                    list_insert(list, scratch[j * EPI_THREADS], id0 + (uint32_t)j);
                }
            }
        }
    }
}

typedef CUresult (*EncodeTiledFn)(CUtensorMap *, CUtensorMapDataType, cuuint32_t, void *, const cuuint64_t *,
                                  const cuuint64_t *, const cuuint32_t *, const cuuint32_t *, CUtensorMapInterleave,
                                  CUtensorMapSwizzle, CUtensorMapL2promotion, CUtensorMapFloatOOBfill);

inline EncodeTiledFn get_encode_fn() {
    static EncodeTiledFn fn = nullptr;
    static bool tried = false;
    if (!tried) {
        tried = true;
        void *ptr = nullptr;
        cudaDriverEntryPointQueryResult qres;
        if (cudaGetDriverEntryPoint("cuTensorMapEncodeTiled", &ptr, cudaEnableDefault, &qres) == cudaSuccess &&
            qres == cudaDriverEntryPointSuccess)
            fn = reinterpret_cast<EncodeTiledFn>(ptr);
    }
    return fn;
}

inline bool encode_rows_map(CUtensorMap *map, const void *base, int64_t rows, int d_pad, int box_rows) {
    EncodeTiledFn fn = get_encode_fn();
    if (!fn) return false;
    const cuuint64_t dims[2] = {(cuuint64_t)d_pad, (cuuint64_t)rows};
    const cuuint64_t strides[1] = {(cuuint64_t)d_pad * 2};
    const cuuint32_t box[2] = {(cuuint32_t)BK, (cuuint32_t)box_rows};
    const cuuint32_t estr[2] = {1, 1};
    return fn(map, CU_TENSOR_MAP_DATA_TYPE_BFLOAT16, 2, const_cast<void *>(base), dims, strides, box, estr,
              CU_TENSOR_MAP_INTERLEAVE_NONE, CU_TENSOR_MAP_SWIZZLE_128B, CU_TENSOR_MAP_L2_PROMOTION_L2_256B,
              CU_TENSOR_MAP_FLOAT_OOB_FILL_NONE) == CUDA_SUCCESS;
}

}
}
```

myscaledb_b200/csrc/ip_gemm_sm100.cu:

```cuda
#include <cstdlib>

#include "gemm_common.cuh"

namespace b200 {
namespace gemm {

template <int CG, int MC>
__global__ void __launch_bounds__(NUM_THREADS, 1)
gemm_topk_kernel(const __grid_constant__ CUtensorMap map_q, const __grid_constant__ CUtensorMap map_c,
                 const GemmTopkParams p) {
    using C = Cfg<CG>;
    const int STAGES = p.stages;
    extern __shared__ unsigned char smem_dyn[];
    unsigned char *smem = reinterpret_cast<unsigned char *>((reinterpret_cast<uintptr_t>(smem_dyn) + 1023) & ~(uintptr_t)1023);
    unsigned char *sA = smem + C::off_a();
    unsigned char *sB = smem + C::off_b(STAGES);
    float *side_scale = reinterpret_cast<float *>(smem + C::off_side(STAGES));
    float *side_bias = side_scale + BN;
    uint64_t *full_bar = reinterpret_cast<uint64_t *>(smem + C::off_bar(STAGES));
    uint64_t *empty_bar = full_bar + MAX_STAGES;
    uint64_t *tmem_full_bar = empty_bar + MAX_STAGES;
    uint64_t *tmem_empty_bar = tmem_full_bar + ACC_STAGES;
    uint32_t *tmem_base_slot = reinterpret_cast<uint32_t *>(tmem_empty_bar + ACC_STAGES);

    const int warp = threadIdx.x >> 5, lane = threadIdx.x & 31;
    const uint32_t cta_rank = CG == 2 ? cluster_ctarank() : 0;
    const uint32_t half = cta_rank & 1;
    const uint32_t pair_in_cluster = cta_rank >> 1;
    const uint32_t leader_rank = cta_rank & ~1u;
    const bool is_leader = half == 0;
    const bool paces = cta_rank == 0;

    const int qt = blockIdx.x % p.q_tiles;
    const int worker = blockIdx.x / p.q_tiles;
    const int W = gridDim.x / p.q_tiles;
    const int64_t n_tiles = (p.n + BN - 1) / BN;
    const int kb_count = p.d_pad / BK;
    const int KPS = p.kps;
    const int NST = STAGES / KPS;

    if (warp == 0 && lane == 0) {
        asm volatile("prefetch.tensormap [%0];" ::"l"(reinterpret_cast<uint64_t>(&map_q)) : "memory");
        asm volatile("prefetch.tensormap [%0];" ::"l"(reinterpret_cast<uint64_t>(&map_c)) : "memory");
        for (int i = 0; i < STAGES; i++) {
            mbar_init(&full_bar[i], 1);
            mbar_init(&empty_bar[i], MC);
        }
        for (int i = 0; i < ACC_STAGES; i++) {
            mbar_init(&tmem_full_bar[i], 1);
            mbar_init(&tmem_empty_bar[i], 4 * CG);
        }
        asm volatile("fence.mbarrier_init.release.cluster;" ::: "memory");
    }
    if (warp == 1) {
        if (CG == 1) {
            asm volatile("tcgen05.alloc.cta_group::1.sync.aligned.shared::cta.b32 [%0], %1;" ::"r"(smem_u32(tmem_base_slot)),
                         "n"(TMEM_COLS)
                         : "memory");
            asm volatile("tcgen05.relinquish_alloc_permit.cta_group::1.sync.aligned;" ::: "memory");
        } else {
            asm volatile("tcgen05.alloc.cta_group::2.sync.aligned.shared::cta.b32 [%0], %1;" ::"r"(smem_u32(tmem_base_slot)),
                         "n"(TMEM_COLS)
                         : "memory");
            asm volatile("tcgen05.relinquish_alloc_permit.cta_group::2.sync.aligned;" ::: "memory");
        }
    }
    tc_fence_before();
    if (CG == 2) cluster_sync_all(); else __syncthreads();
    tc_fence_after();
    const uint32_t tmem_base = *tmem_base_slot;

    if (warp == 0) {
        int stage = 0;
        uint32_t phase = 0;
        int ordinal = 0;
        bool pacing = p.progress != nullptr;
        for (int64_t t = worker; t < n_tiles; t += W, ordinal++) {
            if (pacing && paces) {
                int ok = 1;
                if (lane == 0) {
                    volatile int *prog = p.progress + (size_t)worker * p.q_tiles;
                    prog[qt] = ordinal + 1;
                    int spins = 0;
                    for (int g = 0; g < p.q_tiles; g += CG * MC)
                        while (prog[g] < ordinal + 1 - p.sync_slack && spins < 256) {
                            __nanosleep(200);
                            spins++;
                        }
                    if (spins >= 256) prog[qt] = 0x7fffffff;
                    ok = spins < 256;
                }
                pacing = __shfl_sync(0xffffffffu, ok, 0) != 0;
            }
            __syncwarp();
            for (int kb0 = 0; kb0 < kb_count; kb0 += KPS) {
                mbar_wait(&empty_bar[stage], phase ^ 1);
                if (p.debug & 4) {
                    if (is_leader && elect_one()) mbar_arrive(&full_bar[stage]);
                } else if (elect_one()) {
                    if (CG == 1 || is_leader) mbar_arrive_expect_tx(&full_bar[stage], C::TX_BYTES * KPS);
                    for (int sub = 0; sub < KPS; sub++) {
                        const int kb = kb0 + sub, slot = stage * KPS + sub;
                        if (CG == 1) {
                            tma_load_2d(&map_q, &full_bar[stage], sA + slot * A_BYTES, kb * BK, qt * BM);
                            tma_load_2d(&map_c, &full_bar[stage], sB + slot * C::B_BYTES, kb * BK, (int)(t * BN));
                        } else {
                            tma_load_2d_cg2(&map_q, &full_bar[stage], sA + slot * A_BYTES, kb * BK, qt * BM);
                            if (MC == 1) {
                                tma_load_2d_cg2(&map_c, &full_bar[stage], sB + slot * C::B_BYTES, kb * BK,
                                                (int)(t * BN + half * C::B_ROWS));
                            } else {
                                constexpr int SLICE_ROWS = C::B_ROWS / MC;
                                uint16_t mask = 0;
                                for (int pp = 0; pp < MC; pp++) mask |= (uint16_t)(1u << (pp * 2 + half));
                                tma_load_2d_cg2_mc(&map_c, &full_bar[stage],
                                                   sB + slot * C::B_BYTES + pair_in_cluster * (SLICE_ROWS * BK * 2), kb * BK,
                                                   (int)(t * BN + half * C::B_ROWS + pair_in_cluster * SLICE_ROWS), mask);
                            }
                        }
                    }
                }
                __syncwarp();
                if (++stage == NST) {
                    stage = 0;
                    phase ^= 1;
                }
            }
        }
    } else if (warp == 1) {
        if (is_leader) {
            constexpr uint32_t idesc = make_idesc(CG);
            const uint64_t adesc0 = make_smem_desc(smem_u32(sA));
            const uint64_t bdesc0 = make_smem_desc(smem_u32(sB));
            int stage = 0, as = 0;
            uint32_t phase = 0, aphase = 0;
            for (int64_t t = worker; t < n_tiles; t += W) {
                mbar_wait(&tmem_empty_bar[as], aphase ^ 1);
                tc_fence_after();
                const uint32_t tmem_d = tmem_base + (uint32_t)(as * BN);
                for (int kb0 = 0; kb0 < kb_count; kb0 += KPS) {
                    mbar_wait(&full_bar[stage], phase);
                    tc_fence_after();
                    if (elect_one()) {
                        for (int sub = 0; sub < KPS; sub++) {
                            const int slot = stage * KPS + sub;
                            const uint64_t adesc = adesc0 + (uint64_t)(slot * (A_BYTES >> 4));
                            const uint64_t bdesc = bdesc0 + (uint64_t)(slot * (C::B_BYTES >> 4));
#pragma unroll
                            for (int k = 0; k < BK / UMMA_K; k++) {
                                const uint32_t acc = (kb0 | sub | k) != 0 ? 1u : 0u;
                                if (CG == 1) umma(tmem_d, adesc + k * (UMMA_K * 2 >> 4), bdesc + k * (UMMA_K * 2 >> 4), idesc, acc);
                                else umma_cg2(tmem_d, adesc + k * (UMMA_K * 2 >> 4), bdesc + k * (UMMA_K * 2 >> 4), idesc, acc);
                            }
                        }
                        if (CG == 1) umma_commit(&empty_bar[stage]);
                        else umma_commit_cg2(&empty_bar[stage], (uint16_t)((1u << (CG * MC)) - 1));
                        if (kb0 + KPS >= kb_count) {
                            if (CG == 1) umma_commit(&tmem_full_bar[as]);
                            else umma_commit_cg2(&tmem_full_bar[as], (uint16_t)(3u << leader_rank));
                        }
                    }
                    __syncwarp();
                    if (++stage == NST) {
                        stage = 0;
                        phase ^= 1;
                    }
                }
                if (++as == ACC_STAGES) {
                    as = 0;
                    aphase ^= 1;
                }
            }
        }
    } else {
        const int quarter = warp & 3;
        const int row = quarter * 32 + lane;
        const int et = threadIdx.x - 64;
        const bool use_side = p.row_scale || p.row_bias || p.alive || p.scale_const != -1.f;
        float *scratch = reinterpret_cast<float *>(smem + C::off_scratch(STAGES)) + et;
        ThreadTopK list;
        list.n = 0;
        list.worst = 0;
        list.thr_key = (qt * BM + row < p.nq_valid) ? FLT_MAX : -FLT_MAX;
        list.thr_id = 0;
        if (p.lists_in_smem)
            list_bind(list, reinterpret_cast<float *>(smem + C::off_list(STAGES)),
                      reinterpret_cast<uint32_t *>(smem + C::off_list(STAGES) + (size_t)p.list_cap * EPI_THREADS * 4), row, p.k, p.list_cap);
        else
            list_bind(list, p.list_keys_gmem + (size_t)blockIdx.x * p.list_cap * EPI_THREADS,
                      p.list_ids_gmem + (size_t)blockIdx.x * p.list_cap * EPI_THREADS, row, p.k, p.list_cap);
        int as = 0;
        uint32_t aphase = 0;
        for (int64_t t = worker; t < n_tiles; t += W) {
            const int64_t n0 = t * BN;
            if (use_side) {
                asm volatile("bar.sync 1, 128;" ::: "memory");
                for (int c = et; c < BN; c += EPI_THREADS) {
                    const int64_t r = n0 + c;
                    bool ok = r < p.n;
                    if (ok && p.alive) ok = (p.alive[r >> 3] >> (r & 7)) & 1;
                    side_scale[c] = ok ? (p.row_scale ? p.row_scale[r] : p.scale_const) : 0.f;
                    side_bias[c] = ok ? (p.row_bias ? p.row_bias[r] : 0.f) : __int_as_float(0x7f800000);
                }
                asm volatile("bar.sync 1, 128;" ::: "memory");
            }
#if defined(B200_EPI_SINGLE_POLL) && B200_EPI_SINGLE_POLL
            if (lane == 0) mbar_wait(&tmem_full_bar[as], aphase);
            __syncwarp();
#else
            mbar_wait(&tmem_full_bar[as], aphase);
#endif
            tc_fence_after();
            const uint32_t taddr = tmem_base + ((uint32_t)(quarter * 32) << 16) + (uint32_t)(as * BN);
            const bool tail = n0 + BN > p.n;
            if (p.debug & 1) {
                tc_fence_before();
                __syncwarp();
                if (lane == 0) {
                    if (CG == 1 || is_leader) mbar_arrive(&tmem_empty_bar[as]);
                    else mbar_arrive_remote(&tmem_empty_bar[as], leader_rank);
                }
                if (++as == ACC_STAGES) {
                    as = 0;
                    aphase ^= 1;
                }
                continue;
            }
            float va[32], vb[32];
            __syncwarp();
            tmem_ld32_issue(taddr, va);
            tmem_ld_wait();
#pragma unroll 1
            for (int chunk = 0; chunk < BN / 32; chunk += 2) {
                __syncwarp();
                tmem_ld32_issue(taddr + (chunk + 1) * 32, vb);
                if (!(p.debug & 2))
                    epilogue_chunk(list, va, use_side, side_scale + chunk * 32, side_bias + chunk * 32,
                                   (uint32_t)(n0 + chunk * 32), tail, p.n, scratch);
                else if (va[3] == 12345.678f) list.n = 0;
                tmem_ld_wait();
                __syncwarp();
                if (chunk + 2 < BN / 32) tmem_ld32_issue(taddr + (chunk + 2) * 32, va);
                if (!(p.debug & 2))
                    epilogue_chunk(list, vb, use_side, side_scale + (chunk + 1) * 32, side_bias + (chunk + 1) * 32,
                                   (uint32_t)(n0 + (chunk + 1) * 32), tail, p.n, scratch);
                else if (vb[3] == 12345.678f) list.n = 0;
                tmem_ld_wait();
            }
            tc_fence_before();
            __syncwarp();
            if (lane == 0) {
                if (CG == 1 || is_leader) mbar_arrive(&tmem_empty_bar[as]);
                else mbar_arrive_remote(&tmem_empty_bar[as], leader_rank);
            }
            if (++as == ACC_STAGES) {
                as = 0;
                aphase ^= 1;
            }
        }
        float *ok = p.part_keys + ((size_t)blockIdx.x * BM + row) * p.k;
        uint32_t *oi = p.part_ids + ((size_t)blockIdx.x * BM + row) * p.k;
        list_publish(list, ok, oi);
    }

    tc_fence_before();
    if (CG == 2) cluster_sync_all(); else __syncthreads();
    if (warp == 1) {
        tc_fence_after();
        if (CG == 1)
            asm volatile("tcgen05.dealloc.cta_group::1.sync.aligned.b32 %0, %1;" ::"r"(tmem_base), "n"(TMEM_COLS) : "memory");
        else
            asm volatile("tcgen05.dealloc.cta_group::2.sync.aligned.b32 %0, %1;" ::"r"(tmem_base), "n"(TMEM_COLS) : "memory");
    }
}

template <int CG, int MC>
static cudaError_t launch_cg(const CUtensorMap &map_q, const CUtensorMap &map_c, const GemmTopkParams &p_in, int grid,
                             cudaStream_t s) {
    GemmTopkParams p = p_in;
    static const int min_stages = getenv("B200_GEMM_LIST_SMEM_MIN_STAGES") ? atoi(getenv("B200_GEMM_LIST_SMEM_MIN_STAGES")) : 2;
    p.list_cap = list_cap_for(p.k);
    p.lists_in_smem = (Cfg<CG>::lists_fit(p.list_cap) && Cfg<CG>::stages_for(p.list_cap) >= min_stages) ? 1 : 0;
    const int k_smem = p.lists_in_smem ? p.list_cap : 0;
    p.stages = Cfg<CG>::stages_for(k_smem);
    {
        static const int env_kps = getenv("B200_GEMM_KPS") ? atoi(getenv("B200_GEMM_KPS")) : 1;
        p.kps = (env_kps == 2 && (p.d_pad / BK) % 2 == 0 && p.stages >= 4) ? 2 : 1;
    }
    const size_t smem = (size_t)Cfg<CG>::off_list(p.stages) + (size_t)k_smem * EPI_THREADS * 8 + SMEM_ALIGN_SLACK;
    auto kern = gemm_topk_kernel<CG, MC>;
    cudaError_t e = cudaFuncSetAttribute(kern, cudaFuncAttributeMaxDynamicSharedMemorySize, (int)smem);
    if (e != cudaSuccess) return e;
    cudaLaunchConfig_t cfg{};
    cfg.gridDim = dim3((unsigned)grid);
    cfg.blockDim = dim3(NUM_THREADS);
    cfg.dynamicSmemBytes = smem;
    cfg.stream = s;
    cudaLaunchAttribute attr[1];
    attr[0].id = cudaLaunchAttributeClusterDimension;
    attr[0].val.clusterDim.x = CG * MC;
    attr[0].val.clusterDim.y = 1;
    attr[0].val.clusterDim.z = 1;
    cfg.attrs = attr;
    cfg.numAttrs = 1;
    e = cudaLaunchKernelEx(&cfg, kern, map_q, map_c, p);
    g_launches++;
    return e != cudaSuccess ? e : cudaGetLastError();
}

template <int CG, int MC>
static int max_clusters(int k) {
    static const int min_stages = getenv("B200_GEMM_LIST_SMEM_MIN_STAGES") ? atoi(getenv("B200_GEMM_LIST_SMEM_MIN_STAGES")) : 2;
    const int cap = list_cap_for(k);
    const int k_smem = (Cfg<CG>::lists_fit(cap) && Cfg<CG>::stages_for(cap) >= min_stages) ? cap : 0;
    const int stages = Cfg<CG>::stages_for(k_smem);
    const size_t smem = (size_t)Cfg<CG>::off_list(stages) + (size_t)k_smem * EPI_THREADS * 8 + SMEM_ALIGN_SLACK;
    auto kern = gemm_topk_kernel<CG, MC>;
    if (cudaFuncSetAttribute(kern, cudaFuncAttributeMaxDynamicSharedMemorySize, (int)smem) != cudaSuccess) return 0;
    cudaLaunchConfig_t cfg{};
    cfg.gridDim = dim3(CG * MC * 64);
    cfg.blockDim = dim3(NUM_THREADS);
    cfg.dynamicSmemBytes = smem;
    cudaLaunchAttribute attr[1];
    attr[0].id = cudaLaunchAttributeClusterDimension;
    attr[0].val.clusterDim.x = CG * MC;
    attr[0].val.clusterDim.y = 1;
    attr[0].val.clusterDim.z = 1;
    cfg.attrs = attr;
    cfg.numAttrs = 1;
    int n = 0;
    if (cudaOccupancyMaxActiveClusters(&n, kern, &cfg) != cudaSuccess) {
        cudaGetLastError();
        return 0;
    }
    return n;
}

}

int gemm_topk_grid(int q_tiles, int64_t n, int num_sms) {
    const int64_t n_tiles = ceil_div(n, gemm::BN);
    int64_t g = (int64_t)q_tiles * (n_tiles < 1 ? 1 : n_tiles);
    if (g > num_sms) g = num_sms;
    if (g < q_tiles) g = q_tiles;
    return (int)g;
}

int gemm_topk_max_clusters(int cta_group, int pairs_per_cluster, int k) {
    if (cta_group == 2 && pairs_per_cluster == 4) return gemm::max_clusters<2, 4>(k);
    if (cta_group == 2 && pairs_per_cluster == 2) return gemm::max_clusters<2, 2>(k);
    if (cta_group == 2) return gemm::max_clusters<2, 1>(k);
    return gemm::max_clusters<1, 1>(k);
}

cudaError_t launch_gemm_topk(const GemmTopkParams &p, int grid, cudaStream_t s, const char **err_detail) {
    *err_detail = nullptr;
    const int cg = p.cta_group == 2 ? 2 : 1;
    const int mc = (cg == 2 && (p.pairs_per_cluster == 2 || p.pairs_per_cluster == 4)) ? p.pairs_per_cluster : 1;
    if (grid % p.q_tiles != 0 || p.q_tiles % (cg * mc) != 0) {
        *err_detail = "grid must be a multiple of q_tiles, q_tiles a multiple of the cluster size";
        return cudaErrorInvalidValue;
    }
    CUtensorMap map_q, map_c;
    if (!gemm::encode_rows_map(&map_q, p.queries_bf16, p.nq_pad, p.d_pad, gemm::BM) ||
        !gemm::encode_rows_map(&map_c, p.corpus_bf16, p.n, p.d_pad, gemm::BN / cg / mc)) {
        *err_detail = "cuTensorMapEncodeTiled failed";
        return cudaErrorInvalidValue;
    }
    if (mc == 4) return gemm::launch_cg<2, 4>(map_q, map_c, p, grid, s);
    if (mc == 2) return gemm::launch_cg<2, 2>(map_q, map_c, p, grid, s);
    return cg == 2 ? gemm::launch_cg<2, 1>(map_q, map_c, p, grid, s) : gemm::launch_cg<1, 1>(map_q, map_c, p, grid, s);
}

}
```

myscaledb_b200/csrc/ip_gemm_tf32x3_sm100.cu:

```cuda
#include "gemm_common.cuh"

namespace b200 {
namespace gemm3 {

using namespace gemm;

constexpr int BK3 = 32;
constexpr int UMMA_K3 = 8;
constexpr int A3_BYTES = BM * BK3 * 4;
constexpr int CONV_WARPS = 4;
constexpr int NUM_THREADS3 = 64 + EPI_THREADS + CONV_WARPS * 32;
constexpr int SMEM_LIMIT = 232448;

template <int CG>
struct Cfg3 {
    static constexpr int STAGES = CG == 2 ? 3 : 2;
    static constexpr int B_ROWS = BN / CG;
    static constexpr int B_BYTES = B_ROWS * BK3 * 4;
    static constexpr int STAGE_BYTES = 2 * A3_BYTES + 2 * B_BYTES;
    static constexpr int OFF_AHI = 0;
    static constexpr int OFF_ALO = STAGES * A3_BYTES;
    static constexpr int OFF_B = 2 * STAGES * A3_BYTES;
    static constexpr int OFF_BLO = OFF_B + STAGES * B_BYTES;
    static constexpr int OFF_SIDE = STAGES * STAGE_BYTES;
    static constexpr int OFF_BAR = OFF_SIDE + 2 * BN * 4;
    static constexpr int OFF_SCRATCH = OFF_BAR + 256;
    static constexpr int OFF_LIST = OFF_SCRATCH + SCRATCH_BYTES;
    static constexpr int CONV_ITERS = B_BYTES / 16 / (CONV_WARPS * 32);
    static bool lists_fit(int k) { return OFF_LIST + k * EPI_THREADS * 8 + SMEM_ALIGN_SLACK <= SMEM_LIMIT; }
};

__device__ __forceinline__ constexpr uint32_t make_idesc_tf32(int cg) {
    return (1u << 4) | (2u << 7) | (2u << 10) | ((uint32_t)(BN >> 3) << 17) | ((uint32_t)((BM * cg) >> 4) << 24);
}

__device__ __forceinline__ void umma_tf32_cg1(uint32_t tmem_d, uint64_t adesc, uint64_t bdesc, uint32_t idesc, uint32_t accum) {
    asm volatile(
        "{\n\t"
        ".reg .pred p;\n\t"
        "setp.ne.b32 p, %4, 0;\n\t"
        "tcgen05.mma.cta_group::1.kind::tf32 [%0], %1, %2, %3, p;\n\t"
        "}\n" ::"r"(tmem_d),
        "l"(adesc), "l"(bdesc), "r"(idesc), "r"(accum)
        : "memory");
}
__device__ __forceinline__ void umma_tf32_cg2(uint32_t tmem_d, uint64_t adesc, uint64_t bdesc, uint32_t idesc, uint32_t accum) {
    asm volatile(
        "{\n\t"
        ".reg .pred p;\n\t"
        "setp.ne.b32 p, %4, 0;\n\t"
        "tcgen05.mma.cta_group::2.kind::tf32 [%0], %1, %2, %3, p;\n\t"
        "}\n" ::"r"(tmem_d),
        "l"(adesc), "l"(bdesc), "r"(idesc), "r"(accum)
        : "memory");
}

__device__ __forceinline__ void split_tf32(uint32_t x, uint32_t &hi, uint32_t &lo) {
    hi = x & 0xffffe000u;
    const float r = __uint_as_float(x) - __uint_as_float(hi);
    asm("cvt.rna.tf32.f32 %0, %1;" : "=r"(lo) : "f"(r));
}

__global__ void split_tf32_kernel(const float *__restrict__ src, int64_t n_src, int d_pad, float *__restrict__ hi,
                                  float *__restrict__ lo, int64_t n_pad) {
    const int64_t total = n_pad * d_pad;
    for (int64_t i = (int64_t)blockIdx.x * blockDim.x + threadIdx.x; i < total; i += (int64_t)gridDim.x * blockDim.x) {
        const int64_t r = i / d_pad;
        uint32_t h = 0, l = 0;
        if (r < n_src) split_tf32(__float_as_uint(src[i]), h, l);
        hi[i] = __uint_as_float(h);
        lo[i] = __uint_as_float(l);
    }
}

template <int CG>
__global__ void __launch_bounds__(NUM_THREADS3, 1)
gemm3_topk_kernel(const __grid_constant__ CUtensorMap map_qhi, const __grid_constant__ CUtensorMap map_qlo,
                  const __grid_constant__ CUtensorMap map_c, const GemmTopkParams p) {
    using C = Cfg3<CG>;
    constexpr int STAGES = C::STAGES;
    extern __shared__ unsigned char smem_dyn[];
    unsigned char *smem = reinterpret_cast<unsigned char *>((reinterpret_cast<uintptr_t>(smem_dyn) + 1023) & ~(uintptr_t)1023);
    unsigned char *sAhi = smem + C::OFF_AHI;
    unsigned char *sAlo = smem + C::OFF_ALO;
    unsigned char *sB = smem + C::OFF_B;
    unsigned char *sBlo = smem + C::OFF_BLO;
    float *side_scale = reinterpret_cast<float *>(smem + C::OFF_SIDE);
    float *side_bias = side_scale + BN;
    uint64_t *full_bar = reinterpret_cast<uint64_t *>(smem + C::OFF_BAR);
    uint64_t *bfull_bar = full_bar + STAGES;
    uint64_t *conv_bar = bfull_bar + STAGES;
    uint64_t *empty_bar = conv_bar + STAGES;
    uint64_t *tmem_full_bar = empty_bar + STAGES;
    uint64_t *tmem_empty_bar = tmem_full_bar + ACC_STAGES;
    uint32_t *tmem_base_slot = reinterpret_cast<uint32_t *>(tmem_empty_bar + ACC_STAGES);

    const int warp = threadIdx.x >> 5, lane = threadIdx.x & 31;
    const uint32_t cta_rank = CG == 2 ? cluster_ctarank() : 0;
    const uint32_t half = cta_rank & 1;
    const bool is_leader = half == 0;

    const int qt = blockIdx.x % p.q_tiles;
    const int worker = blockIdx.x / p.q_tiles;
    const int W = gridDim.x / p.q_tiles;
    const int64_t n_tiles = (p.n + BN - 1) / BN;
    const int kb_count = (p.d_pad + BK3 - 1) / BK3;

    if (warp == 0 && lane == 0) {
        asm volatile("prefetch.tensormap [%0];" ::"l"(reinterpret_cast<uint64_t>(&map_qhi)) : "memory");
        asm volatile("prefetch.tensormap [%0];" ::"l"(reinterpret_cast<uint64_t>(&map_qlo)) : "memory");
        asm volatile("prefetch.tensormap [%0];" ::"l"(reinterpret_cast<uint64_t>(&map_c)) : "memory");
        for (int i = 0; i < STAGES; i++) {
            mbar_init(&full_bar[i], 1);
            mbar_init(&bfull_bar[i], 1);
            mbar_init(&conv_bar[i], CG * CONV_WARPS);
            mbar_init(&empty_bar[i], 1);
        }
        for (int i = 0; i < ACC_STAGES; i++) {
            mbar_init(&tmem_full_bar[i], 1);
            mbar_init(&tmem_empty_bar[i], 4 * CG);
        }
        asm volatile("fence.mbarrier_init.release.cluster;" ::: "memory");
    }
    if (warp == 1) {
        if (CG == 1) {
            asm volatile("tcgen05.alloc.cta_group::1.sync.aligned.shared::cta.b32 [%0], %1;" ::"r"(smem_u32(tmem_base_slot)),
                         "n"(TMEM_COLS)
                         : "memory");
            asm volatile("tcgen05.relinquish_alloc_permit.cta_group::1.sync.aligned;" ::: "memory");
        } else {
            asm volatile("tcgen05.alloc.cta_group::2.sync.aligned.shared::cta.b32 [%0], %1;" ::"r"(smem_u32(tmem_base_slot)),
                         "n"(TMEM_COLS)
                         : "memory");
            asm volatile("tcgen05.relinquish_alloc_permit.cta_group::2.sync.aligned;" ::: "memory");
        }
    }
    tc_fence_before();
    if (CG == 2) cluster_sync_all(); else __syncthreads();
    tc_fence_after();
    const uint32_t tmem_base = *tmem_base_slot;

    if (warp == 0) {
        int stage = 0;
        uint32_t phase = 0;
        int ordinal = 0;
        bool pacing = p.progress != nullptr;
        for (int64_t t = worker; t < n_tiles; t += W, ordinal++) {
            if (pacing && is_leader) {
                int ok = 1;
                if (lane == 0) {
                    volatile int *prog = p.progress + (size_t)worker * p.q_tiles;
                    prog[qt] = ordinal + 1;
                    int spins = 0;
                    for (int g = 0; g < p.q_tiles; g += CG)
                        while (prog[g] < ordinal + 1 - p.sync_slack && spins < 256) {
                            __nanosleep(200);
                            spins++;
                        }
                    if (spins >= 256) prog[qt] = 0x7fffffff;
                    ok = spins < 256;
                }
                pacing = __shfl_sync(0xffffffffu, ok, 0) != 0;
            }
            __syncwarp();
            for (int kb = 0; kb < kb_count; kb++) {
                mbar_wait(&empty_bar[stage], phase ^ 1);
                if (elect_one()) {
                    if (CG == 1) {
                        mbar_arrive_expect_tx(&full_bar[stage], 2 * A3_BYTES);
                        tma_load_2d(&map_qhi, &full_bar[stage], sAhi + stage * A3_BYTES, kb * BK3, qt * BM);
                        tma_load_2d(&map_qlo, &full_bar[stage], sAlo + stage * A3_BYTES, kb * BK3, qt * BM);
                    } else {
                        if (is_leader) mbar_arrive_expect_tx(&full_bar[stage], 2 * 2 * A3_BYTES);
                        tma_load_2d_cg2(&map_qhi, &full_bar[stage], sAhi + stage * A3_BYTES, kb * BK3, qt * BM);
                        tma_load_2d_cg2(&map_qlo, &full_bar[stage], sAlo + stage * A3_BYTES, kb * BK3, qt * BM);
                    }
                    mbar_arrive_expect_tx(&bfull_bar[stage], C::B_BYTES);
                    tma_load_2d(&map_c, &bfull_bar[stage], sB + stage * C::B_BYTES, kb * BK3, (int)(t * BN + half * C::B_ROWS));
                }
                __syncwarp();
                if (++stage == STAGES) {
                    stage = 0;
                    phase ^= 1;
                }
            }
        }
    } else if (warp == 1) {
        if (is_leader) {
            constexpr uint32_t idesc = make_idesc_tf32(CG);
            const uint64_t ahi0 = make_smem_desc(smem_u32(sAhi));
            const uint64_t alo0 = make_smem_desc(smem_u32(sAlo));
            const uint64_t b0 = make_smem_desc(smem_u32(sB));
            const uint64_t blo0 = make_smem_desc(smem_u32(sBlo));
            int stage = 0, as = 0;
            uint32_t phase = 0, aphase = 0;
            for (int64_t t = worker; t < n_tiles; t += W) {
                mbar_wait(&tmem_empty_bar[as], aphase ^ 1);
                tc_fence_after();
                const uint32_t tmem_d = tmem_base + (uint32_t)(as * BN);
                for (int kb = 0; kb < kb_count; kb++) {
                    mbar_wait(&full_bar[stage], phase);
                    mbar_wait(&conv_bar[stage], phase);
                    tc_fence_after();
                    if (elect_one()) {
                        const uint64_t ahi = ahi0 + (uint64_t)(stage * (A3_BYTES >> 4));
                        const uint64_t alo = alo0 + (uint64_t)(stage * (A3_BYTES >> 4));
                        const uint64_t b = b0 + (uint64_t)(stage * (C::B_BYTES >> 4));
                        const uint64_t blo = blo0 + (uint64_t)(stage * (C::B_BYTES >> 4));
#pragma unroll
                        for (int k = 0; k < BK3 / UMMA_K3; k++) {
                            const uint64_t off = (uint64_t)(k * (UMMA_K3 * 4 >> 4));
                            const uint32_t acc0 = (kb | k) != 0 ? 1u : 0u;
                            if (CG == 1) {
                                umma_tf32_cg1(tmem_d, alo + off, b + off, idesc, acc0);
                                umma_tf32_cg1(tmem_d, ahi + off, blo + off, idesc, 1u);
                                umma_tf32_cg1(tmem_d, ahi + off, b + off, idesc, 1u);
                            } else {
                                umma_tf32_cg2(tmem_d, alo + off, b + off, idesc, acc0);
                                umma_tf32_cg2(tmem_d, ahi + off, blo + off, idesc, 1u);
                                umma_tf32_cg2(tmem_d, ahi + off, b + off, idesc, 1u);
                            }
                        }
                        if (CG == 1) {
                            umma_commit(&empty_bar[stage]);
                            if (kb == kb_count - 1) umma_commit(&tmem_full_bar[as]);
                        } else {
                            umma_commit_cg2(&empty_bar[stage], 3);
                            if (kb == kb_count - 1) umma_commit_cg2(&tmem_full_bar[as], 3);
                        }
                    }
                    __syncwarp();
                    if (++stage == STAGES) {
                        stage = 0;
                        phase ^= 1;
                    }
                }
                if (++as == ACC_STAGES) {
                    as = 0;
                    aphase ^= 1;
                }
            }
        }
    } else if (warp >= 6) {
        const int ct = threadIdx.x - (64 + EPI_THREADS);
        int stage = 0;
        uint32_t phase = 0;
        for (int64_t t = worker; t < n_tiles; t += W) {
            for (int kb = 0; kb < kb_count; kb++) {
                mbar_wait(&bfull_bar[stage], phase);
                uint4 *b = reinterpret_cast<uint4 *>(sB + stage * C::B_BYTES);
                uint4 *bl = reinterpret_cast<uint4 *>(sBlo + stage * C::B_BYTES);
#pragma unroll
                for (int i0 = 0; i0 < C::CONV_ITERS; i0 += 8) {
                    uint4 raw[8];
#pragma unroll
                    for (int i = 0; i < 8; i++) raw[i] = b[ct + (i0 + i) * (CONV_WARPS * 32)];
#pragma unroll
                    for (int i = 0; i < 8; i++) {
                        uint4 h, l;
                        split_tf32(raw[i].x, h.x, l.x);
                        split_tf32(raw[i].y, h.y, l.y);
                        split_tf32(raw[i].z, h.z, l.z);
                        split_tf32(raw[i].w, h.w, l.w);
                        b[ct + (i0 + i) * (CONV_WARPS * 32)] = h;
                        bl[ct + (i0 + i) * (CONV_WARPS * 32)] = l;
                    }
                }
                asm volatile("fence.proxy.async.shared::cta;" ::: "memory");
                __syncwarp();
                if (lane == 0) {
                    if (is_leader) mbar_arrive(&conv_bar[stage]);
                    else mbar_arrive_remote(&conv_bar[stage], 0);
                }
                if (++stage == STAGES) {
                    stage = 0;
                    phase ^= 1;
                }
            }
        }
    } else {
        const int quarter = warp & 3;
        const int row = quarter * 32 + lane;
        const int et = threadIdx.x - 64;
        const bool use_side = p.row_scale || p.row_bias || p.alive || p.scale_const != -1.f;
        float *scratch = reinterpret_cast<float *>(smem + C::OFF_SCRATCH) + et;
        ThreadTopK list;
        list.n = 0;
        list.worst = 0;
        list.thr_key = (qt * BM + row < p.nq_valid) ? FLT_MAX : -FLT_MAX;
        list.thr_id = 0;
        if (p.lists_in_smem)
            list_bind(list, reinterpret_cast<float *>(smem + C::OFF_LIST),
                      reinterpret_cast<uint32_t *>(smem + C::OFF_LIST + (size_t)p.list_cap * EPI_THREADS * 4), row, p.k, p.list_cap);
        else
            list_bind(list, p.list_keys_gmem + (size_t)blockIdx.x * p.list_cap * EPI_THREADS,
                      p.list_ids_gmem + (size_t)blockIdx.x * p.list_cap * EPI_THREADS, row, p.k, p.list_cap);
        int as = 0;
        uint32_t aphase = 0;
        for (int64_t t = worker; t < n_tiles; t += W) {
            const int64_t n0 = t * BN;
            if (use_side) {
                asm volatile("bar.sync 1, 128;" ::: "memory");
                for (int c = et; c < BN; c += EPI_THREADS) {
                    const int64_t r = n0 + c;
                    bool ok = r < p.n;
                    if (ok && p.alive) ok = (p.alive[r >> 3] >> (r & 7)) & 1;
                    side_scale[c] = ok ? (p.row_scale ? p.row_scale[r] : p.scale_const) : 0.f;
                    side_bias[c] = ok ? (p.row_bias ? p.row_bias[r] : 0.f) : __int_as_float(0x7f800000);
                }
                asm volatile("bar.sync 1, 128;" ::: "memory");
            }
            mbar_wait(&tmem_full_bar[as], aphase);
            tc_fence_after();
            const uint32_t taddr = tmem_base + ((uint32_t)(quarter * 32) << 16) + (uint32_t)(as * BN);
            const bool tail = n0 + BN > p.n;
            float va[32], vb[32];
            __syncwarp();
            tmem_ld32_issue(taddr, va);
            tmem_ld_wait();
#pragma unroll 1
            for (int chunk = 0; chunk < BN / 32; chunk += 2) {
                __syncwarp();
                tmem_ld32_issue(taddr + (chunk + 1) * 32, vb);
                epilogue_chunk(list, va, use_side, side_scale + chunk * 32, side_bias + chunk * 32, (uint32_t)(n0 + chunk * 32),
                               tail, p.n, scratch);
                tmem_ld_wait();
                __syncwarp();
                if (chunk + 2 < BN / 32) tmem_ld32_issue(taddr + (chunk + 2) * 32, va);
                epilogue_chunk(list, vb, use_side, side_scale + (chunk + 1) * 32, side_bias + (chunk + 1) * 32,
                               (uint32_t)(n0 + (chunk + 1) * 32), tail, p.n, scratch);
                tmem_ld_wait();
            }
            tc_fence_before();
            __syncwarp();
            if (lane == 0) {
                if (is_leader) mbar_arrive(&tmem_empty_bar[as]);
                else mbar_arrive_remote(&tmem_empty_bar[as], 0);
            }
            if (++as == ACC_STAGES) {
                as = 0;
                aphase ^= 1;
            }
        }
        float *ok = p.part_keys + ((size_t)blockIdx.x * BM + row) * p.k;
        uint32_t *oi = p.part_ids + ((size_t)blockIdx.x * BM + row) * p.k;
        list_publish(list, ok, oi);
    }

    tc_fence_before();
    if (CG == 2) cluster_sync_all(); else __syncthreads();
    if (warp == 1) {
        tc_fence_after();
        if (CG == 1)
            asm volatile("tcgen05.dealloc.cta_group::1.sync.aligned.b32 %0, %1;" ::"r"(tmem_base), "n"(TMEM_COLS) : "memory");
        else
            asm volatile("tcgen05.dealloc.cta_group::2.sync.aligned.b32 %0, %1;" ::"r"(tmem_base), "n"(TMEM_COLS) : "memory");
    }
}

static bool encode_rows_map_f32(CUtensorMap *map, const void *base, int64_t rows, int d_pad, int box_rows) {
    EncodeTiledFn fn = get_encode_fn();
    if (!fn) return false;
    const cuuint64_t dims[2] = {(cuuint64_t)d_pad, (cuuint64_t)rows};
    const cuuint64_t strides[1] = {(cuuint64_t)d_pad * 4};
    const cuuint32_t box[2] = {(cuuint32_t)BK3, (cuuint32_t)box_rows};
    const cuuint32_t estr[2] = {1, 1};
    return fn(map, CU_TENSOR_MAP_DATA_TYPE_FLOAT32, 2, const_cast<void *>(base), dims, strides, box, estr,
              CU_TENSOR_MAP_INTERLEAVE_NONE, CU_TENSOR_MAP_SWIZZLE_128B, CU_TENSOR_MAP_L2_PROMOTION_L2_256B,
              CU_TENSOR_MAP_FLOAT_OOB_FILL_NONE) == CUDA_SUCCESS;
}

}

cudaError_t launch_split_tf32(const float *src, int64_t n_src, int d_pad, float *hi, float *lo, int64_t n_pad, cudaStream_t s) {
    if (n_pad == 0) return cudaSuccess;
    int64_t b = ceil_div(n_pad * d_pad, 256);
    if (b > 148 * 8) b = 148 * 8;
    gemm3::split_tf32_kernel<<<(int)b, 256, 0, s>>>(src, n_src, d_pad, hi, lo, n_pad);
    g_launches++;
    return cudaGetLastError();
}

template <int CG>
static cudaError_t launch3_cg(const CUtensorMap &map_qhi, const CUtensorMap &map_qlo, const CUtensorMap &map_c,
                              const GemmTopkParams &p_in, int grid, cudaStream_t s) {
    using namespace gemm3;
    using C = Cfg3<CG>;
    GemmTopkParams p = p_in;
    p.list_cap = list_cap_for(p.k);
    p.lists_in_smem = C::lists_fit(p.list_cap) ? 1 : 0;
    p.stages = C::STAGES;
    const size_t smem = (size_t)C::OFF_LIST + (p.lists_in_smem ? (size_t)p.list_cap * EPI_THREADS * 8 : 0) + SMEM_ALIGN_SLACK;
    auto kern = gemm3_topk_kernel<CG>;
    cudaError_t e = cudaFuncSetAttribute(kern, cudaFuncAttributeMaxDynamicSharedMemorySize, (int)smem);
    if (e != cudaSuccess) return e;
    cudaLaunchConfig_t cfg{};
    cfg.gridDim = dim3((unsigned)grid);
    cfg.blockDim = dim3(NUM_THREADS3);
    cfg.dynamicSmemBytes = smem;
    cfg.stream = s;
    cudaLaunchAttribute attr[1];
    attr[0].id = cudaLaunchAttributeClusterDimension;
    attr[0].val.clusterDim.x = CG;
    attr[0].val.clusterDim.y = 1;
    attr[0].val.clusterDim.z = 1;
    cfg.attrs = attr;
    cfg.numAttrs = 1;
    e = cudaLaunchKernelEx(&cfg, kern, map_qhi, map_qlo, map_c, p);
    g_launches++;
    return e != cudaSuccess ? e : cudaGetLastError();
}

cudaError_t launch_gemm3_topk(const GemmTopkParams &p, int grid, cudaStream_t s, const char **err_detail) {
    using namespace gemm3;
    *err_detail = nullptr;
    const int cg = p.cta_group == 2 ? 2 : 1;
    if (p.q_tiles % cg != 0 || grid % p.q_tiles != 0 || !p.queries_lo) {
        *err_detail = "gemm3: q_tiles must be a multiple of cta_group, grid a multiple of q_tiles, queries_lo set";
        return cudaErrorInvalidValue;
    }
    CUtensorMap map_qhi, map_qlo, map_c;
    if (!encode_rows_map_f32(&map_qhi, p.queries_bf16, p.nq_pad, p.d_pad, BM) ||
        !encode_rows_map_f32(&map_qlo, p.queries_lo, p.nq_pad, p.d_pad, BM) ||
        !encode_rows_map_f32(&map_c, p.corpus_bf16, p.n, p.d_pad, BN / cg)) {
        *err_detail = "cuTensorMapEncodeTiled failed";
        return cudaErrorInvalidValue;
    }
    return cg == 2 ? launch3_cg<2>(map_qhi, map_qlo, map_c, p, grid, s) : launch3_cg<1>(map_qhi, map_qlo, map_c, p, grid, s);
}

}
```

myscaledb_b200/csrc/kernels.h:

```cpp
#pragma once
#include <cuda_runtime.h>
#include <stdint.h>

namespace b200 {

struct ScanParams {
    const void *corpus;
    const float *queries;
    const float *row_scale;
    const uint8_t *alive;
    float *part_keys;
    uint32_t *part_ids;
    int64_t n, nq;
    int64_t row_bytes;
    int d_pad, k, group;
    int l2, bf16;
    int fused;
    int q_dim;
    int cosine;
    int out_mode, ip_min_quirk;
    int64_t id_offset;
    unsigned int *tickets;
    float *out_dis;
    int64_t *out_ids;
    volatile unsigned int *done_flag;
    unsigned int done_value;
    unsigned int *tiles_done;
    int q_inline;
    unsigned long long *debug_ts;
    int stage_cap;
    float qinline[256];
};

struct BinaryScanParams {
    const uint8_t *corpus;
    const uint8_t *queries;
    const uint8_t *alive;
    float *part_keys;
    uint32_t *part_ids;
    int64_t n, nq;
    int nbytes, k, jaccard;
};

enum { kOutKey = 0, kOutNeg = 1, kOutOnePlus = 2, kOutAddQ = 3, kOutCosQ = 4 };

struct MergeParams {
    const void *in_keys;
    const void *in_ids;
    int64_t list_stride, q_stride;
    int64_t id_list_stride;
    int n_lists, k_in, k;
    int64_t nq;
    int descending;
    int tie_mode;
    int32_t *out_list;
    int out_mode;
    int ip_min_quirk;
    const float *q_add;
    int64_t id_offset;
    float *out_dis;
    int64_t *out_ids;
};

size_t scan_smem_bytes(int qt, int d_pad, int k);
cudaError_t launch_flat_scan(const ScanParams &p, int qt, int blocks_x, cudaStream_t s);
cudaError_t launch_binary_scan(const BinaryScanParams &p, int blocks_x, cudaStream_t s);
cudaError_t launch_topk_merge(const MergeParams &p, bool external, cudaStream_t s);
cudaError_t launch_rescore_l2(const void *corpus, int bf16, int64_t row_bytes, int d_pad, const float *queries, int64_t nq, int64_t id_offset,
                              int k, float *dis, int64_t *ids, cudaStream_t s);

struct GemmTopkParams {
    const void *corpus_bf16;
    const void *queries_bf16;
    const void *queries_lo;
    const float *row_scale;
    float scale_const;
    const float *row_bias;
    const uint8_t *alive;
    float *part_keys;
    uint32_t *part_ids;
    float *list_keys_gmem;
    uint32_t *list_ids_gmem;
    int64_t n;
    int nq_pad, d_pad, k;
    int nq_valid;
    int q_tiles;
    int cta_group;
    int pairs_per_cluster;
    int *progress;
    int stages;
    int kps;
    int lists_in_smem;
    int list_cap;
    int debug;
    int sync_slack;
};
constexpr int kGemmSmemK = 128;
__host__ __device__ inline int list_cap_append(int k) { return 2 * k + 32; }
__host__ __device__ inline int list_tourn_group(int k) { return k <= 64 ? 8 : 16; }
__host__ __device__ inline int list_cap_tourn(int k) { return k + (k + list_tourn_group(k) - 1) / list_tourn_group(k); }
int list_cap_for(int k);
int gemm_topk_grid(int q_tiles, int64_t n, int num_sms);
cudaError_t launch_gemm_topk(const GemmTopkParams &p, int grid, cudaStream_t s, const char **err_detail);
int gemm_topk_max_clusters(int cta_group, int pairs_per_cluster, int k);
bool gemm_topk_ts_supported(int d_pad, int q_tiles);
int gemm_topk_ts_tile_rows(int d_pad);
cudaError_t launch_gemm_topk_ts(const GemmTopkParams &p, int grid, cudaStream_t s, const char **err_detail);

cudaError_t launch_split_tf32(const float *src, int64_t n_src, int d_pad, float *hi, float *lo, int64_t n_pad, cudaStream_t s);
cudaError_t launch_gemm3_topk(const GemmTopkParams &p, int grid, cudaStream_t s, const char **err_detail);

int staged_h2d(void *dst, const void *src, size_t bytes, int device, cudaStream_t s);

cudaError_t launch_f32_to_bf16_rows(const float *src, int d, void *dst, int d_pad, int64_t n, cudaStream_t s);
cudaError_t launch_pad_rows_f32(const float *src, int d, float *dst, int d_pad, int64_t n, cudaStream_t s);
cudaError_t launch_row_norms(const void *rows, int bf16, int d_pad, int64_t n, int mode, float *out, cudaStream_t s);
cudaError_t launch_normalize_rows_f32(float *rows, int d_pad, int64_t n, cudaStream_t s);

}
```

myscaledb_b200/search.py:

```python
from __future__ import annotations

import ctypes as C

import numpy as np

from ._lib import lib

L2, IP, COSINE, HAMMING, JACCARD = 0, 1, 2, 3, 4
METRIC_NAMES = {"L2": L2, "IP": IP, "COSINE": COSINE, "HAMMING": HAMMING, "JACCARD": JACCARD}
F32, BF16, BIN = 0, 1, 2
PATH_AUTO, PATH_SCAN, PATH_TENSOR, PATH_CG1, PATH_CG2, PATH_CG2_MC2, PATH_CG2_MC4, PATH_TS = range(8)
KERNEL_SCAN, KERNEL_GEMM_BF16, KERNEL_GEMM_TS, KERNEL_GEMM_TF32X3 = 1, 2, 3, 4


class B200Error(RuntimeError):
    def __init__(self, code, msg):
        super().__init__(f"b200 error {code}: {msg}")
        self.code = code


def _check(rc):
    if rc != 0:
        raise B200Error(rc, lib().b200_last_error().decode(errors="replace"))


def _p(a, t):
    return None if a is None else a.ctypes.data_as(C.POINTER(t))


def _bits(a):
    return None if a is None else np.ascontiguousarray(a, np.uint8)


def flat_knn(metric, x, y, k, alive_bits=None):
    x = np.ascontiguousarray(x, np.float32)
    y = np.ascontiguousarray(y, np.float32)
    nx, d = x.shape
    ny = y.shape[0]
    dis = np.empty((nx, k), np.float32)
    ids = np.empty((nx, k), np.int64)
    ab = _bits(alive_bits)
    _check(lib().b200_flat_knn(C.c_int(metric), _p(x, C.c_float), C.c_int64(nx), _p(y, C.c_float), C.c_int64(ny),
                               C.c_int(d), C.c_int(k), _p(ab, C.c_uint8), _p(dis, C.c_float), _p(ids, C.c_int64)))
    return dis, ids


def binary_knn(metric, x, y, k, alive_bits=None):
    x = np.ascontiguousarray(x, np.uint8)
    y = np.ascontiguousarray(y, np.uint8)
    nx, nb = x.shape
    ny = y.shape[0]
    dis = np.empty((nx, k), np.float32)
    ids = np.empty((nx, k), np.int64)
    ab = _bits(alive_bits)
    _check(lib().b200_binary_knn(C.c_int(metric), _p(x, C.c_uint8), C.c_int64(nx), _p(y, C.c_uint8), C.c_int64(ny),
                                 C.c_int(nb), C.c_int(k), _p(ab, C.c_uint8), _p(dis, C.c_float), _p(ids, C.c_int64)))
    return dis, ids


def part_scan(metric, x, y, k, block_rows=8192, row_exists=None, filter_bits=None):
    binary = metric in (HAMMING, JACCARD)
    if binary:
        x = np.ascontiguousarray(x, np.uint8)
        y = np.ascontiguousarray(y, np.uint8)
        d = x.shape[1] * 8
    else:
        x = np.ascontiguousarray(x, np.float32)
        y = np.ascontiguousarray(y, np.float32)
        d = x.shape[1]
    nx, ny = x.shape[0], y.shape[0]
    dis = np.empty((nx, k), np.float32)
    ids = np.empty((nx, k), np.int64)
    re_ = None if row_exists is None else np.ascontiguousarray(row_exists, np.uint8)
    fb = _bits(filter_bits)
    _check(lib().b200_part_scan(C.c_int(metric), x.ctypes.data_as(C.c_void_p), C.c_int64(nx),
                                y.ctypes.data_as(C.c_void_p), C.c_int64(ny), C.c_int(d), C.c_int(k),
                                C.c_int64(block_rows), _p(re_, C.c_uint8), _p(fb, C.c_uint8), _p(dis, C.c_float),
                                _p(ids, C.c_int64)))
    return dis, ids


class Corpus:

    def __init__(self, metric, d, dtype=F32, capacity=0):
        self._h = C.c_void_p()
        self.metric, self.d, self.dtype = metric, d, dtype
        _check(lib().b200_corpus_create(C.c_int(metric), C.c_int(dtype), C.c_int(d), C.c_int64(capacity), C.byref(self._h)))

    @classmethod
    def borrowed(cls, handle: int, metric, d, dtype=F32):
        self = cls.__new__(cls)
        self._h = C.c_void_p(handle)
        self.metric, self.d, self.dtype = metric, d, dtype
        self.close = lambda: None
        return self

    def append(self, rows):
        rows = np.ascontiguousarray(rows, np.uint8 if self.dtype == BIN else np.float32)
        _check(lib().b200_corpus_append(self._h, rows.ctypes.data_as(C.c_void_p), C.c_int64(rows.shape[0])))
        return self

    def adopt_device(self, data_ptr: int, n: int):
        _check(lib().b200_corpus_adopt_device(self._h, C.c_void_p(data_ptr), C.c_int64(n)))
        return self

    def set_path(self, path: int):
        _check(lib().b200_corpus_set_path(self._h, C.c_int(path)))
        return self

    def last_variant(self):
        kern, cg, mc, grid = C.c_int(), C.c_int(), C.c_int(), C.c_int()
        _check(lib().b200_corpus_last_variant(self._h, C.byref(kern), C.byref(cg), C.byref(mc), C.byref(grid)))
        return kern.value, cg.value, mc.value, grid.value

    @property
    def size(self):
        n = C.c_int64()
        _check(lib().b200_corpus_size(self._h, C.byref(n)))
        return n.value

    def search(self, queries, k, alive_bits=None):
        q = np.ascontiguousarray(queries, np.uint8 if self.dtype == BIN else np.float32)
        nq = q.shape[0]
        dis = np.empty((nq, k), np.float32)
        ids = np.empty((nq, k), np.int64)
        ab = _bits(alive_bits)
        _check(lib().b200_corpus_search(self._h, q.ctypes.data_as(C.POINTER(C.c_float)), C.c_int64(nq), C.c_int(k),
                                        _p(ab, C.c_uint8), _p(dis, C.c_float), _p(ids, C.c_int64)))
        return dis, ids

    def search_device(self, q_ptr: int, nq: int, k: int, out_dis_ptr: int, out_ids_ptr: int, id_offset=0,
                      alive_ptr: int = 0, stream: int = 0):
        _check(lib().b200_corpus_search_device(self._h, C.c_void_p(q_ptr), C.c_int64(nq), C.c_int(k),
                                               C.c_void_p(alive_ptr or None), C.c_int64(id_offset),
                                               C.c_void_p(out_dis_ptr), C.c_void_p(out_ids_ptr),
                                               C.c_void_p(stream or None)))

    def enable_timing(self, on=True):
        _check(lib().b200_corpus_enable_timing(self._h, C.c_int(1 if on else 0)))

    def kernel_time(self, reset=False):
        ms, n = C.c_double(), C.c_int64()
        _check(lib().b200_corpus_kernel_time(self._h, C.c_int(1 if reset else 0), C.byref(ms), C.byref(n)))
        return ms.value, n.value

    def close(self):
        if self._h:
            lib().b200_corpus_free(self._h)
            self._h = C.c_void_p()

    def __del__(self):
        try:
            self.close()
        except Exception:
            pass


def topk_merge_device(dis_ptr, ids_ptr, n_lists, nq, k, descending, out_dis_ptr, out_ids_ptr, stream=0):
    _check(lib().b200_topk_merge_device(C.c_void_p(dis_ptr), C.c_void_p(ids_ptr), C.c_int(n_lists), C.c_int64(nq),
                                        C.c_int(k), C.c_int(1 if descending else 0), C.c_void_p(out_dis_ptr),
                                        C.c_void_p(out_ids_ptr), C.c_void_p(stream or None)))


def topk_merge_device_strided(dis_ptr, ids_ptr, n_lists, dis_stride, ids_stride, nq, k, descending, out_dis_ptr,
                              out_ids_ptr, stream=0):
    _check(lib().b200_topk_merge_device_strided(C.c_void_p(dis_ptr), C.c_void_p(ids_ptr), C.c_int(n_lists),
                                                C.c_int64(dis_stride), C.c_int64(ids_stride), C.c_int64(nq), C.c_int(k),
                                                C.c_int(1 if descending else 0), C.c_void_p(out_dis_ptr),
                                                C.c_void_p(out_ids_ptr), C.c_void_p(stream or None)))


def topk_merge_device_ex(dis_ptr, ids_ptr, n_lists, dis_stride, ids_stride, nq, k_in, k, descending, tie_mode, out_dis_ptr,
                         out_ids_ptr, out_list_ptr=0, stream=0):
    _check(lib().b200_topk_merge_device_ex(C.c_void_p(dis_ptr), C.c_void_p(ids_ptr), C.c_int(n_lists), C.c_int64(dis_stride),
                                           C.c_int64(ids_stride), C.c_int64(nq), C.c_int(k_in), C.c_int(k),
                                           C.c_int(1 if descending else 0), C.c_int(tie_mode), C.c_void_p(out_dis_ptr),
                                           C.c_void_p(out_ids_ptr), C.c_void_p(out_list_ptr or None), C.c_void_p(stream or None)))


def launch_count(reset=False) -> int:
    return int(lib().b200_launch_count(C.c_int(1 if reset else 0)))


class BM25Index:

    def __init__(self, n_fields: int = 1):
        self._h = C.c_void_p()
        self.n_fields = n_fields
        _check(lib().b200_bm25_create(C.c_uint32(n_fields), C.byref(self._h)))

    def add_doc(self, row_id: int, texts):
        _check(lib().b200_bm25_add_doc(self._h, C.c_uint64(row_id)))
        if isinstance(texts, str):
            texts = [texts]
        for f, t in enumerate(texts):
            for piece in ([t] if isinstance(t, str) else t):
                _check(lib().b200_bm25_add_text(self._h, C.c_uint32(f), piece.encode()))

    def commit(self):
        _check(lib().b200_bm25_commit(self._h))
        return self

    def save(self, path):
        _check(lib().b200_bm25_save(self._h, str(path).encode()))

    @classmethod
    def load(cls, path, n_fields=1):
        self = cls.__new__(cls)
        self._h = C.c_void_p()
        self.n_fields = n_fields
        _check(lib().b200_bm25_load(str(path).encode(), C.byref(self._h)))
        return self

    @property
    def total_docs(self):
        v = C.c_uint64()
        _check(lib().b200_bm25_total_docs(self._h, C.byref(v)))
        return v.value

    def total_tokens(self, field=0):
        v = C.c_uint64()
        _check(lib().b200_bm25_total_tokens(self._h, C.c_uint32(field), C.byref(v)))
        return v.value

    def doc_freq(self, term, field=0):
        v = C.c_uint64()
        _check(lib().b200_bm25_doc_freq(self._h, C.c_uint32(field), term.encode(), C.byref(v)))
        return v.value

    _qt_tls = __import__("threading").local()

    @staticmethod
    def query_terms(sentence):
        tls = BM25Index._qt_tls
        if not hasattr(tls, "buf"):
            tls.buf = (C.create_string_buffer(4096), C.c_uint32())
        buf, n = tls.buf
        _check(lib().b200_bm25_query_terms(sentence.encode(), buf, C.c_size_t(4096), C.byref(n)))
        out, off = [], 0
        base = C.addressof(buf)
        for _ in range(n.value):
            t = C.string_at(base + off)
            out.append(t.decode())
            off += len(t) + 1
        return out

    def search_batch(self, sentences, topk, fields=(0,), alive_bits=None, operator_or=True, stats=None):
        nq = len(sentences)
        arr = (C.c_char_p * nq)(*[s.encode() for s in sentences])
        f = np.array(fields, np.uint32)
        rows = np.empty((nq, topk), np.uint64)
        scores = np.empty((nq, topk), np.float32)
        counts = np.zeros(nq, np.uint32)
        st_docs, st_tok, st_df = 0, None, None
        if stats is not None:
            st_docs = int(stats["total_docs"])
            st_tok = np.zeros(self.n_fields, np.uint64)
            for fi, v in stats["total_tokens"].items():
                st_tok[fi] = v
            st_df = np.zeros((nq, len(fields), 64), np.uint64)
            for qi, sent in enumerate(sentences):
                for ti, t in enumerate(self.query_terms(sent)[:64]):
                    for fi, fld in enumerate(fields):
                        st_df[qi, fi, ti] = stats["doc_freq"].get((fld, t), 0)
        ab = _bits(alive_bits)
        _check(lib().b200_bm25_search_batch(self._h, arr, C.c_int64(nq), _p(f, C.c_uint32), C.c_uint32(len(fields)),
                                            C.c_uint32(topk), _p(ab, C.c_uint8), C.c_int(0 if ab is None else 1),
                                            C.c_int(1 if operator_or else 0), C.c_uint64(st_docs), _p(st_tok, C.c_uint64),
                                            _p(st_df, C.c_uint64), _p(rows, C.c_uint64), _p(scores, C.c_float),
                                            _p(counts, C.c_uint32)))
        return [(rows[q, :counts[q]].copy(), scores[q, :counts[q]].copy()) for q in range(nq)]

    def last_timing(self):
        km, cm, po = C.c_double(), C.c_double(), C.c_uint64()
        _check(lib().b200_bm25_last_timing(self._h, C.byref(km), C.byref(cm), C.byref(po)))
        return dict(kernel_ms=km.value, call_ms=cm.value, postings=po.value)

    def search(self, sentence, topk, **kw):
        return self.search_batch([sentence], topk, **kw)[0]

    def close(self):
        if self._h:
            lib().b200_bm25_free(self._h)
            self._h = C.c_void_p()

    def __del__(self):
        try:
            self.close()
        except Exception:
            pass


def hybrid_fusion_batch(fusion_type, vec_lists, txt_lists, top_k, fusion_weight=0.5, fusion_k=60, vector_scan_direction=1):
    nq = len(vec_lists)
    assert len(txt_lists) == nq
    vs = max([len(v) for v in vec_lists] + [1])
    ts = max([len(t) for t in txt_lists] + [1])

    def pack(lists, stride):
        sh = np.zeros((nq, stride), np.uint32); pa = np.zeros((nq, stride), np.uint64)
        la = np.zeros((nq, stride), np.uint64); sc = np.zeros((nq, stride), np.float32)
        cnt = np.zeros(nq, np.uint32)
        for q, lst in enumerate(lists):
            cnt[q] = len(lst)
            for i, (a, b, c, d) in enumerate(lst):
                sh[q, i], pa[q, i], la[q, i], sc[q, i] = a, b, c, d
        return sh, pa, la, sc, cnt
    v = pack(vec_lists, vs)
    t = pack(txt_lists, ts)
    o_sh = np.zeros((nq, top_k), np.uint32); o_pa = np.zeros((nq, top_k), np.uint64)
    o_la = np.zeros((nq, top_k), np.uint64); o_sc = np.zeros((nq, top_k), np.float32); o_cnt = np.zeros(nq, np.uint32)
    ft = {"rsf": 0, "rrf": 1}[fusion_type.lower()]
    _check(lib().b200_hybrid_fusion_batch(
        C.c_int(ft), C.c_int64(nq), _p(v[0], C.c_uint32), _p(v[1], C.c_uint64), _p(v[2], C.c_uint64), _p(v[3], C.c_float),
        _p(v[4], C.c_uint32), C.c_int64(vs), _p(t[0], C.c_uint32), _p(t[1], C.c_uint64), _p(t[2], C.c_uint64),
        _p(t[3], C.c_float), _p(t[4], C.c_uint32), C.c_int64(ts), C.c_float(fusion_weight), C.c_uint64(fusion_k),
        C.c_int(vector_scan_direction), C.c_uint32(top_k), _p(o_sh, C.c_uint32), _p(o_pa, C.c_uint64), _p(o_la, C.c_uint64),
        _p(o_sc, C.c_float), _p(o_cnt, C.c_uint32)))
    return [[(int(o_sh[q, i]), int(o_pa[q, i]), int(o_la[q, i]), float(o_sc[q, i])) for i in range(o_cnt[q])]
            for q in range(nq)]


def hybrid_fusion_arrays(fusion_type, vec_ids, vec_scores, txt_ids, txt_scores, top_k, fusion_weight=0.5, fusion_k=60,
                         vector_scan_direction=1):
    vec_ids = np.ascontiguousarray(vec_ids, np.int64); txt_ids = np.ascontiguousarray(txt_ids, np.int64)
    nq, kv = vec_ids.shape
    kt = txt_ids.shape[1]
    v_cnt = (vec_ids >= 0).sum(1).astype(np.uint32); t_cnt = (txt_ids >= 0).sum(1).astype(np.uint32)
    v_la = np.where(vec_ids >= 0, vec_ids, 0).astype(np.uint64); t_la = np.where(txt_ids >= 0, txt_ids, 0).astype(np.uint64)
    v_sc = np.ascontiguousarray(vec_scores, np.float32); t_sc = np.ascontiguousarray(np.where(txt_ids >= 0, txt_scores, 0), np.float32)
    v_sh = np.zeros((nq, kv), np.uint32); v_pa = np.zeros((nq, kv), np.uint64)
    t_sh = np.zeros((nq, kt), np.uint32); t_pa = np.zeros((nq, kt), np.uint64)
    o_sh = np.zeros((nq, top_k), np.uint32); o_pa = np.zeros((nq, top_k), np.uint64)
    o_la = np.zeros((nq, top_k), np.uint64); o_sc = np.zeros((nq, top_k), np.float32); o_cnt = np.zeros(nq, np.uint32)
    ft = {"rsf": 0, "rrf": 1}[fusion_type.lower()]
    _check(lib().b200_hybrid_fusion_batch(
        C.c_int(ft), C.c_int64(nq), _p(v_sh, C.c_uint32), _p(v_pa, C.c_uint64), _p(v_la, C.c_uint64), _p(v_sc, C.c_float),
        _p(v_cnt, C.c_uint32), C.c_int64(kv), _p(t_sh, C.c_uint32), _p(t_pa, C.c_uint64), _p(t_la, C.c_uint64),
        _p(t_sc, C.c_float), _p(t_cnt, C.c_uint32), C.c_int64(kt), C.c_float(fusion_weight), C.c_uint64(fusion_k),
        C.c_int(vector_scan_direction), C.c_uint32(top_k), _p(o_sh, C.c_uint32), _p(o_pa, C.c_uint64), _p(o_la, C.c_uint64),
        _p(o_sc, C.c_float), _p(o_cnt, C.c_uint32)))
    ids = np.where(np.arange(top_k)[None, :] < o_cnt[:, None], o_la.astype(np.int64), -1)
    return ids, o_sc, o_cnt


class VectorIndex:

    def __init__(self, index_type, metric, d, params=""):
        self._h = C.c_void_p()
        self.d = d
        _check(lib().b200_index_create(index_type.encode(), C.c_int(metric), C.c_int(d), params.encode(), C.byref(self._h)))

    def build(self, rows):
        rows = np.ascontiguousarray(rows, np.float32)
        _check(lib().b200_index_build(self._h, _p(rows, C.c_float), C.c_int64(rows.shape[0])))
        return self

    def reserve(self, total_rows):
        _check(lib().b200_index_reserve(self._h, C.c_int64(total_rows)))
        return self

    def train(self, rows):
        rows = np.ascontiguousarray(rows, np.float32)
        _check(lib().b200_index_train(self._h, _p(rows, C.c_float), C.c_int64(rows.shape[0])))
        return self

    def add(self, rows):
        rows = np.ascontiguousarray(rows, np.float32)
        _check(lib().b200_index_add(self._h, _p(rows, C.c_float), C.c_int64(rows.shape[0])))
        return self

    def train_device(self, ptr: int, n: int):
        _check(lib().b200_index_train_device(self._h, C.c_void_p(ptr), C.c_int64(n)))
        return self

    def add_device(self, ptr: int, n: int):
        _check(lib().b200_index_add_device(self._h, C.c_void_p(ptr), C.c_int64(n)))
        return self

    def finalize(self):
        _check(lib().b200_index_finalize(self._h))
        return self

    def search_device(self, q_ptr: int, nq: int, k: int, out_dis_ptr: int, out_ids_ptr: int, params="", first_stage_only=False,
                      id_offset=0, alive_ptr: int = 0, stream: int = 0):
        _check(lib().b200_index_search_device(self._h, C.c_void_p(q_ptr), C.c_int64(nq), C.c_int(k), params.encode(),
                                              C.c_int(1 if first_stage_only else 0), C.c_void_p(alive_ptr or None),
                                              C.c_int64(id_offset), C.c_void_p(out_dis_ptr), C.c_void_p(out_ids_ptr),
                                              C.c_void_p(stream or None)))

    def enable_timing(self, on=True):
        _check(lib().b200_index_enable_timing(self._h, C.c_int(1 if on else 0)))

    def last_scan(self, reset=False):
        rows, rb, items, ms, nl = C.c_int64(), C.c_int64(), C.c_int64(), C.c_double(), C.c_int64()
        _check(lib().b200_index_last_scan(self._h, C.byref(rows), C.byref(rb), C.byref(items), C.byref(ms), C.byref(nl),
                                          C.c_int(1 if reset else 0)))
        return dict(rows_streamed=rows.value, payload_row_bytes=rb.value, work_items=items.value, kernel_ms=ms.value, launches=nl.value)

    def phase_ms(self):
        a = (C.c_double * 5)()
        _check(lib().b200_index_phase_ms(self._h, a))
        return dict(zip(("coarse", "plan", "scan", "merge", "refine"), [round(v, 4) for v in a]))

    def list_sizes(self):
        nl = self.info()["nlist"]
        out = np.zeros(nl, np.uint32)
        _check(lib().b200_index_list_sizes(self._h, _p(out, C.c_uint32), C.c_int(nl)))
        return out

    def memory_bytes(self):
        b = C.c_uint64()
        _check(lib().b200_index_memory_bytes(self._h, C.byref(b)))
        return b.value

    def info(self):
        n, nl, m, ivf = C.c_int64(), C.c_int(), C.c_int(), C.c_int()
        _check(lib().b200_index_info(self._h, C.byref(n), C.byref(nl), C.byref(m), C.byref(ivf)))
        return dict(n=n.value, nlist=nl.value, m=m.value, uses_ivf=bool(ivf.value))

    def search(self, queries, k, params="", first_stage_only=False, alive_bits=None):
        q = np.ascontiguousarray(queries, np.float32)
        nq = q.shape[0]
        dis = np.empty((nq, k), np.float32)
        ids = np.empty((nq, k), np.int64)
        nc = C.c_int64()
        ab = _bits(alive_bits)
        _check(lib().b200_index_search(self._h, _p(q, C.c_float), C.c_int64(nq), C.c_int(k), params.encode(),
                                       C.c_int(1 if first_stage_only else 0), _p(ab, C.c_uint8), _p(dis, C.c_float),
                                       _p(ids, C.c_int64), C.byref(nc)))
        self.last_num_candidates = nc.value
        return dis, ids

    def save(self, path):
        _check(lib().b200_index_save(self._h, str(path).encode()))

    @classmethod
    def load(cls, path, d):
        self = cls.__new__(cls)
        self._h = C.c_void_p()
        self.d = d
        _check(lib().b200_index_load(str(path).encode(), C.byref(self._h)))
        return self

    def refine(self, queries, cand_ids, k):
        q = np.ascontiguousarray(queries, np.float32)
        c = np.ascontiguousarray(cand_ids, np.int64)
        nq = q.shape[0]
        dis = np.empty((nq, k), np.float32)
        ids = np.empty((nq, k), np.int64)
        _check(lib().b200_index_refine(self._h, _p(q, C.c_float), C.c_int64(nq), _p(c, C.c_int64), C.c_int64(c.shape[1]),
                                       C.c_int(k), _p(dis, C.c_float), _p(ids, C.c_int64)))
        return dis, ids

    def close(self):
        if self._h:
            lib().b200_index_free(self._h)
            self._h = C.c_void_p()

    def __del__(self):
        try:
            self.close()
        except Exception:
            pass


def bitmap_and(a, b, nbits):
    a, b = np.ascontiguousarray(a, np.uint8), np.ascontiguousarray(b, np.uint8)
    out = np.zeros((nbits + 7) // 8, np.uint8)
    _check(lib().b200_bitmap_and(_p(a, C.c_uint8), _p(b, C.c_uint8), C.c_int64(nbits), _p(out, C.c_uint8)))
    return out


def real_bitmap(filter_bits, n_new_rows, inverted_row_ids_map, inverted_row_sources_map, own_id, total_vec):
    f = np.ascontiguousarray(filter_bits, np.uint8)
    ids = np.ascontiguousarray(inverted_row_ids_map, np.uint64)
    src = np.ascontiguousarray(inverted_row_sources_map, np.uint8)
    out = np.zeros((total_vec + 7) // 8, np.uint8)
    _check(lib().b200_real_bitmap(_p(f, C.c_uint8), C.c_int64(n_new_rows), _p(ids, C.c_uint64), _p(src, C.c_uint8),
                                  C.c_uint32(own_id), C.c_int64(total_vec), _p(out, C.c_uint8)))
    return out


def remap_labels(row_ids_map, labels):
    m = np.ascontiguousarray(row_ids_map, np.uint64)
    l = np.ascontiguousarray(labels, np.int64).copy()
    _check(lib().b200_remap_labels(_p(m, C.c_uint64), C.c_int64(m.size), _p(l, C.c_int64), C.c_int64(l.size)))
    return l


def transfer_to_old_row_ids(new_ids, new_dis, inverted_row_ids_map, inverted_row_sources_map, own_id):
    ids = np.ascontiguousarray(new_ids, np.int64); dis = np.ascontiguousarray(new_dis, np.float32)
    m = np.ascontiguousarray(inverted_row_ids_map, np.uint64); src = np.ascontiguousarray(inverted_row_sources_map, np.uint8)
    o_i = np.empty(ids.size, np.int64); o_d = np.empty(ids.size, np.float32); n = C.c_int64()
    _check(lib().b200_transfer_to_old_row_ids(_p(ids, C.c_int64), _p(dis, C.c_float), C.c_int64(ids.size), _p(m, C.c_uint64),
                                              _p(src, C.c_uint8), C.c_int64(m.size), C.c_uint32(own_id), _p(o_i, C.c_int64),
                                              _p(o_d, C.c_float), C.byref(n)))
    return o_i[:n.value], o_d[:n.value]


CACHE_CORPUS, CACHE_INDEX, CACHE_BM25, CACHE_OPAQUE = 0, 1, 2, 3
_DELETER = C.CFUNCTYPE(None, C.c_void_p)


class CacheMiss(KeyError):
    pass


def cache_set_capacity(nbytes: int):
    _check(lib().b200_cache_set_capacity(C.c_uint64(nbytes)))


def cache_get(key: str):
    h, kind = C.c_void_p(), C.c_int()
    rc = lib().b200_cache_get(key.encode(), C.byref(h), C.byref(kind))
    if rc == 6:
        raise CacheMiss(key)
    _check(rc)
    return h.value, kind.value


def cache_put(key: str, obj, nbytes: int = None):
    kind = CACHE_CORPUS if isinstance(obj, Corpus) else CACHE_INDEX if isinstance(obj, VectorIndex) else CACHE_BM25
    if nbytes is None:
        b = C.c_uint64()
        if kind == CACHE_CORPUS:
            _check(lib().b200_corpus_memory_bytes(obj._h, C.byref(b)))
        elif kind == CACHE_INDEX:
            _check(lib().b200_index_memory_bytes(obj._h, C.byref(b)))
        nbytes = b.value
    res = C.c_void_p()
    _check(lib().b200_cache_put(key.encode(), C.c_int(kind), obj._h, C.c_uint64(nbytes), C.byref(res)))
    if res.value == (obj._h.value if isinstance(obj._h, C.c_void_p) else obj._h):
        obj._h = C.c_void_p()
    return res.value


def cache_put_opaque(key: str, handle: int, nbytes: int, deleter):
    res = C.c_void_p()
    _check(lib().b200_cache_put_opaque(key.encode(), C.c_void_p(handle), C.c_uint64(nbytes), deleter, C.byref(res)))
    return res.value


def cache_release(key: str, handle: int | None = None):
    if handle is None:
        _check(lib().b200_cache_release(key.encode()))
    else:
        _check(lib().b200_cache_release_handle(key.encode(), C.c_void_p(handle)))


def cache_expire(key: str):
    rc = lib().b200_cache_expire(key.encode())
    if rc == 6:
        raise CacheMiss(key)
    _check(rc)


def cache_expire_prefix(prefix: str) -> int:
    n = C.c_int64()
    _check(lib().b200_cache_expire_prefix(prefix.encode(), C.byref(n)))
    return n.value


def cache_stats() -> dict:
    v = [C.c_uint64() for _ in range(6)]
    _check(lib().b200_cache_stats(*[C.byref(x) for x in v]))
    return dict(zip(("capacity", "used", "items", "hits", "misses", "evictions"), (x.value for x in v)))
```

Before: 78640.

## Keep part of query A-tile resident in shared memory for cta_group 2 GEMM

Reworks the bf16 GEMM top-k pipeline so some of the query (A) k-blocks stay resident in shared memory across corpus tiles, loaded once per CTA, while the rest stream through a unified slot ring shared with B. The shared-memory plan moves from stages to units. This cuts repeated TMA reloads of the query tile and frees ring space for B. It also removes the KPS grouping option and adds resident-count introspection APIs, at the cost of a more complex producer/consumer slot schedule and fewer ring slots for streaming.

Result: slower. 67900, median of 6 (-13.7%).

```diff
diff --git a/include/b200_search.h b/include/b200_search.h
--- a/include/b200_search.h
+++ b/include/b200_search.h
@@ -60,6 +60,8 @@
 #define B200_KERNEL_GEMM_TS 3
 #define B200_KERNEL_GEMM_TF32X3 4
 int b200_corpus_last_variant(b200_corpus *c, int *kernel, int *cta_group, int *pairs_per_cluster, int *grid);
+int b200_corpus_last_gemm_resident(b200_corpus *c, int *kblocks);
+int b200_gemm_resident_kblocks(int cta_group, int d_pad, int k, int *out_kblocks);
 int b200_corpus_enable_timing(b200_corpus *c, int on);
 int b200_corpus_kernel_time(b200_corpus *c, int reset, double *out_total_ms, int64_t *out_launches);
 int64_t b200_launch_count(int reset);
diff --git a/myscaledb_b200/csrc/capi.cu b/myscaledb_b200/csrc/capi.cu
--- a/myscaledb_b200/csrc/capi.cu
+++ b/myscaledb_b200/csrc/capi.cu
@@ -102,7 +102,8 @@
     int rescore_l2 = 1;
     int gemm_multicast = 1;
     int gemm_ts = 0;
-    int last_cg = 0, last_mc = 0, last_ts = 0, last_grid = 0, last_kernel = 0;
+    int gemm_resident = -1;
+    int last_cg = 0, last_mc = 0, last_ts = 0, last_grid = 0, last_kernel = 0, last_resident = 0;
     bool timing = false;
     std::vector<std::pair<cudaEvent_t, cudaEvent_t>> ev_used, ev_free;
     double timed_ms = 0;
@@ -232,6 +233,7 @@
     if (const char *ev = getenv("B200_FUSED_SCAN")) c->fused_enabled = atoi(ev);
     if (const char *ev = getenv("B200_GEMM_TS")) c->gemm_ts = atoi(ev);
     if (const char *ev = getenv("B200_GEMM_MULTICAST")) c->gemm_multicast = atoi(ev);
+    if (const char *ev = getenv("B200_GEMM_RESIDENT")) c->gemm_resident = atoi(ev);
     cudaError_t e = cudaStreamCreateWithFlags(&c->stream, cudaStreamNonBlocking);
     if (e != cudaSuccess) {
         delete c;
@@ -384,6 +386,20 @@
     if (cta_group) *cta_group = c->last_cg;
     if (pairs_per_cluster) *pairs_per_cluster = c->last_mc;
     if (grid) *grid = c->last_grid;
+    return B200_OK;
+}
+
+extern "C" int b200_corpus_last_gemm_resident(b200_corpus *c, int *kblocks) {
+    if (!c || !kblocks) return fail(B200_ERR_INVALID, "null argument");
+    std::lock_guard<std::mutex> lk(c->mu);
+    *kblocks = c->last_resident;
+    return B200_OK;
+}
+
+extern "C" int b200_gemm_resident_kblocks(int cta_group, int d_pad, int k, int *out_kblocks) {
+    if (!out_kblocks || (cta_group != 1 && cta_group != 2) || d_pad <= 0 || d_pad % 64 || k <= 0 || k > 1024)
+        return fail(B200_ERR_INVALID, "cta_group 1 or 2, d_pad a positive multiple of 64, 1 <= k <= 1024");
+    *out_kblocks = gemm_resident_kblocks(cta_group, d_pad, k);
     return B200_OK;
 }
 
@@ -520,7 +536,7 @@
         timing_begin(c, s, ev);
         B200_CUDA_OK(launch_flat_scan(sp, qt, blocks_x, s));
         timing_end(c, s, ev);
-        c->last_kernel = B200_KERNEL_SCAN; c->last_cg = 0; c->last_mc = 0; c->last_grid = blocks_x;
+        c->last_kernel = B200_KERNEL_SCAN; c->last_cg = 0; c->last_mc = 0; c->last_grid = blocks_x; c->last_resident = 0;
         MergeParams mp{};
         mp.in_keys = sp.part_keys;
         mp.in_ids = sp.part_ids;
@@ -624,11 +640,15 @@
         timing_begin(c, s, ev);
         const bool use_ts = !f32 && cta_group == 2 && k <= 30 && gemm_topk_ts_supported(c->d_pad, q_tiles) &&
                             (c->gemm_ts == 2 || (c->gemm_ts == 1 && c->d_pad <= 512));
+        if (!f32 && !use_ts) {
+            const int plan = gemm_resident_kblocks(cta_group, c->d_pad, k);
+            gp.a_resident = c->gemm_resident < 0 ? plan : std::min(plan, c->gemm_resident);
+        }
         cudaError_t e = f32 ? launch_gemm3_topk(gp, grid, s, &detail)
                             : use_ts ? launch_gemm_topk_ts(gp, grid, s, &detail) : launch_gemm_topk(gp, grid, s, &detail);
         timing_end(c, s, ev);
         c->last_kernel = f32 ? B200_KERNEL_GEMM_TF32X3 : use_ts ? B200_KERNEL_GEMM_TS : B200_KERNEL_GEMM_BF16;
-        c->last_cg = cta_group; c->last_mc = (f32 || use_ts) ? 1 : pairs; c->last_grid = grid;
+        c->last_cg = cta_group; c->last_mc = (f32 || use_ts) ? 1 : pairs; c->last_grid = grid; c->last_resident = gp.a_resident;
         if (e != cudaSuccess)
             return fail(B200_ERR_CUDA, std::string("gemm_topk launch: ") + (detail ? detail : cudaGetErrorString(e)));
         MergeParams mp{};
@@ -769,7 +789,7 @@
     timing_begin(c, s, ev);
     B200_CUDA_OK(launch_flat_scan(sp, qt, blocks_x, s));
     timing_end(c, s, ev);
-    c->last_kernel = B200_KERNEL_SCAN; c->last_cg = 0; c->last_mc = 0; c->last_grid = blocks_x;
+    c->last_kernel = B200_KERNEL_SCAN; c->last_cg = 0; c->last_mc = 0; c->last_grid = blocks_x; c->last_resident = 0;
     for (uint64_t spin = 1;; spin++) {
         if (*h_flag == sp.done_value) break;
         if ((spin & 0x3fff) == 0) {
diff --git a/myscaledb_b200/csrc/gemm_common.cuh b/myscaledb_b200/csrc/gemm_common.cuh
--- a/myscaledb_b200/csrc/gemm_common.cuh
+++ b/myscaledb_b200/csrc/gemm_common.cuh
@@ -28,20 +28,22 @@
     static constexpr int B_BYTES = B_ROWS * BK * 2;
     static constexpr int STAGE_BYTES = A_BYTES + B_BYTES;
     static constexpr int TX_BYTES = STAGE_BYTES * CG;
+    static constexpr int UNIT_BYTES = CG == 1 ? STAGE_BYTES : A_BYTES;
+    static constexpr int MIN_UNITS = CG == 1 ? 2 : 4;
+    static constexpr int MAX_UNITS = CG == 1 ? 4 : 12;
     __host__ __device__ static constexpr int off_a() { return 0; }
-    __host__ __device__ static constexpr int off_b(int stages) { return stages * A_BYTES; }
-    __host__ __device__ static constexpr int off_side(int stages) { return stages * STAGE_BYTES; }
-    __host__ __device__ static constexpr int off_bar(int stages) { return off_side(stages) + 2 * BN * 4; }
-    __host__ __device__ static constexpr int off_scratch(int stages) { return off_bar(stages) + 256; }
-    __host__ __device__ static constexpr int off_list(int stages) { return off_scratch(stages) + SCRATCH_BYTES; }
-    __host__ __device__ static int stages_for(int k_smem) {
-        const int max_stages = CG == 1 ? 4 : 6;
-        int st = max_stages;
-        while (st > 2 && off_list(st) + k_smem * EPI_THREADS * 8 + SMEM_ALIGN_SLACK > 232448) st--;
-        return st;
+    __host__ __device__ static constexpr int off_b(int units) { return units * A_BYTES; }
+    __host__ __device__ static constexpr int off_side(int units) { return units * UNIT_BYTES; }
+    __host__ __device__ static constexpr int off_bar(int units) { return off_side(units) + 2 * BN * 4; }
+    __host__ __device__ static constexpr int off_scratch(int units) { return off_bar(units) + 256; }
+    __host__ __device__ static constexpr int off_list(int units) { return off_scratch(units) + SCRATCH_BYTES; }
+    __host__ __device__ static int units_for(int k_smem) {
+        int u = MAX_UNITS;
+        while (u > MIN_UNITS && off_list(u) + k_smem * EPI_THREADS * 8 + SMEM_ALIGN_SLACK > 232448) u--;
+        return u;
     }
     __host__ __device__ static bool lists_fit(int k) {
-        return off_list(2) + k * EPI_THREADS * 8 + SMEM_ALIGN_SLACK <= 232448;
+        return off_list(MIN_UNITS) + k * EPI_THREADS * 8 + SMEM_ALIGN_SLACK <= 232448;
     }
 };
 
diff --git a/myscaledb_b200/csrc/ip_gemm_sm100.cu b/myscaledb_b200/csrc/ip_gemm_sm100.cu
--- a/myscaledb_b200/csrc/ip_gemm_sm100.cu
+++ b/myscaledb_b200/csrc/ip_gemm_sm100.cu
@@ -1,3 +1,4 @@
+#include <algorithm>
 #include <cstdlib>
 
 #include "gemm_common.cuh"
@@ -10,18 +11,22 @@
 gemm_topk_kernel(const __grid_constant__ CUtensorMap map_q, const __grid_constant__ CUtensorMap map_c,
                  const GemmTopkParams p) {
     using C = Cfg<CG>;
-    const int STAGES = p.stages;
+    const int UNITS = p.units;
+    const int S = CG == 2 ? p.a_resident : 0;
+    const int R = UNITS - S;
     extern __shared__ unsigned char smem_dyn[];
     unsigned char *smem = reinterpret_cast<unsigned char *>((reinterpret_cast<uintptr_t>(smem_dyn) + 1023) & ~(uintptr_t)1023);
     unsigned char *sA = smem + C::off_a();
-    unsigned char *sB = smem + C::off_b(STAGES);
-    float *side_scale = reinterpret_cast<float *>(smem + C::off_side(STAGES));
+    unsigned char *sB = smem + C::off_b(UNITS);
+    unsigned char *sRing = smem + S * C::UNIT_BYTES;
+    float *side_scale = reinterpret_cast<float *>(smem + C::off_side(UNITS));
     float *side_bias = side_scale + BN;
-    uint64_t *full_bar = reinterpret_cast<uint64_t *>(smem + C::off_bar(STAGES));
-    uint64_t *empty_bar = full_bar + MAX_STAGES;
-    uint64_t *tmem_full_bar = empty_bar + MAX_STAGES;
+    uint64_t *full_bar = reinterpret_cast<uint64_t *>(smem + C::off_bar(UNITS));
+    uint64_t *empty_bar = full_bar + C::MAX_UNITS;
+    uint64_t *tmem_full_bar = empty_bar + C::MAX_UNITS;
     uint64_t *tmem_empty_bar = tmem_full_bar + ACC_STAGES;
-    uint32_t *tmem_base_slot = reinterpret_cast<uint32_t *>(tmem_empty_bar + ACC_STAGES);
+    uint64_t *res_bar = tmem_empty_bar + ACC_STAGES;
+    uint32_t *tmem_base_slot = reinterpret_cast<uint32_t *>(res_bar + 1);
 
     const int warp = threadIdx.x >> 5, lane = threadIdx.x & 31;
     const uint32_t cta_rank = CG == 2 ? cluster_ctarank() : 0;
@@ -36,13 +41,17 @@
     const int W = gridDim.x / p.q_tiles;
     const int64_t n_tiles = (p.n + BN - 1) / BN;
     const int kb_count = p.d_pad / BK;
-    const int KPS = p.kps;
-    const int NST = STAGES / KPS;
+    auto a_streamed = [&](int &err) {
+        err += kb_count - S;
+        if (err < kb_count) return false;
+        err -= kb_count;
+        return true;
+    };
 
     if (warp == 0 && lane == 0) {
         asm volatile("prefetch.tensormap [%0];" ::"l"(reinterpret_cast<uint64_t>(&map_q)) : "memory");
         asm volatile("prefetch.tensormap [%0];" ::"l"(reinterpret_cast<uint64_t>(&map_c)) : "memory");
-        for (int i = 0; i < STAGES; i++) {
+        for (int i = 0; i < UNITS; i++) {
             mbar_init(&full_bar[i], 1);
             mbar_init(&empty_bar[i], MC);
         }
@@ -50,6 +59,7 @@
             mbar_init(&tmem_full_bar[i], 1);
             mbar_init(&tmem_empty_bar[i], 4 * CG);
         }
+        mbar_init(res_bar, 1);
         asm volatile("fence.mbarrier_init.release.cluster;" ::: "memory");
     }
     if (warp == 1) {
@@ -71,10 +81,48 @@
     const uint32_t tmem_base = *tmem_base_slot;
 
     if (warp == 0) {
-        int stage = 0;
+        int slot = 0;
         uint32_t phase = 0;
         int ordinal = 0;
         bool pacing = p.progress != nullptr;
+        if (S > 0 && elect_one()) {
+            if (is_leader) mbar_arrive_expect_tx(res_bar, (uint32_t)(S * A_BYTES * CG));
+            for (int kb = 0, r = 0, err = 0; kb < kb_count; kb++)
+                if (!a_streamed(err)) tma_load_2d_cg2(&map_q, res_bar, sA + (r++) * A_BYTES, kb * BK, qt * BM);
+        }
+        __syncwarp();
+        auto fill = [&](int kb, bool is_a, int64_t t) {
+            mbar_wait(&empty_bar[slot], phase ^ 1);
+            const bool skip_a = (p.debug & 8) && ordinal > 0;
+            if ((p.debug & 4) || (CG == 2 && is_a && skip_a)) {
+                if ((CG == 1 || is_leader) && elect_one()) mbar_arrive(&full_bar[slot]);
+            } else if (elect_one()) {
+                if (CG == 1) {
+                    mbar_arrive_expect_tx(&full_bar[slot], skip_a ? C::B_BYTES : C::TX_BYTES);
+                    if (!skip_a) tma_load_2d(&map_q, &full_bar[slot], sA + slot * A_BYTES, kb * BK, qt * BM);
+                    tma_load_2d(&map_c, &full_bar[slot], sB + slot * C::B_BYTES, kb * BK, (int)(t * BN));
+                } else {
+                    if (is_leader) mbar_arrive_expect_tx(&full_bar[slot], (uint32_t)(C::UNIT_BYTES * CG));
+                    unsigned char *dst = sRing + slot * C::UNIT_BYTES;
+                    if (is_a) {
+                        tma_load_2d_cg2(&map_q, &full_bar[slot], dst, kb * BK, qt * BM);
+                    } else if (MC == 1) {
+                        tma_load_2d_cg2(&map_c, &full_bar[slot], dst, kb * BK, (int)(t * BN + half * C::B_ROWS));
+                    } else {
+                        constexpr int SLICE_ROWS = C::B_ROWS / MC;
+                        uint16_t mask = 0;
+                        for (int pp = 0; pp < MC; pp++) mask |= (uint16_t)(1u << (pp * 2 + half));
+                        tma_load_2d_cg2_mc(&map_c, &full_bar[slot], dst + pair_in_cluster * (SLICE_ROWS * BK * 2), kb * BK,
+                                           (int)(t * BN + half * C::B_ROWS + pair_in_cluster * SLICE_ROWS), mask);
+                    }
+                }
+            }
+            __syncwarp();
+            if (++slot == R) {
+                slot = 0;
+                phase ^= 1;
+            }
+        };
         for (int64_t t = worker; t < n_tiles; t += W, ordinal++) {
             if (pacing && paces) {
                 int ok = 1;
@@ -93,78 +141,65 @@
                 pacing = __shfl_sync(0xffffffffu, ok, 0) != 0;
             }
             __syncwarp();
-            for (int kb0 = 0; kb0 < kb_count; kb0 += KPS) {
-                mbar_wait(&empty_bar[stage], phase ^ 1);
-                if (p.debug & 4) {
-                    if (is_leader && elect_one()) mbar_arrive(&full_bar[stage]);
-                } else if (elect_one()) {
-                    if (CG == 1 || is_leader) mbar_arrive_expect_tx(&full_bar[stage], C::TX_BYTES * KPS);
-                    for (int sub = 0; sub < KPS; sub++) {
-                        const int kb = kb0 + sub, slot = stage * KPS + sub;
-                        if (CG == 1) {
-                            tma_load_2d(&map_q, &full_bar[stage], sA + slot * A_BYTES, kb * BK, qt * BM);
-                            tma_load_2d(&map_c, &full_bar[stage], sB + slot * C::B_BYTES, kb * BK, (int)(t * BN));
-                        } else {
-                            tma_load_2d_cg2(&map_q, &full_bar[stage], sA + slot * A_BYTES, kb * BK, qt * BM);
-                            if (MC == 1) {
-                                tma_load_2d_cg2(&map_c, &full_bar[stage], sB + slot * C::B_BYTES, kb * BK,
-                                                (int)(t * BN + half * C::B_ROWS));
-                            } else {
-                                constexpr int SLICE_ROWS = C::B_ROWS / MC;
-                                uint16_t mask = 0;
-                                for (int pp = 0; pp < MC; pp++) mask |= (uint16_t)(1u << (pp * 2 + half));
-                                tma_load_2d_cg2_mc(&map_c, &full_bar[stage],
-                                                   sB + slot * C::B_BYTES + pair_in_cluster * (SLICE_ROWS * BK * 2), kb * BK,
-                                                   (int)(t * BN + half * C::B_ROWS + pair_in_cluster * SLICE_ROWS), mask);
-                            }
-                        }
-                    }
-                }
-                __syncwarp();
-                if (++stage == NST) {
-                    stage = 0;
-                    phase ^= 1;
-                }
+            for (int kb = 0, err = 0; kb < kb_count; kb++) {
+                if (CG == 2 && a_streamed(err)) fill(kb, true, t);
+                fill(kb, false, t);
             }
         }
     } else if (warp == 1) {
         if (is_leader) {
             constexpr uint32_t idesc = make_idesc(CG);
             const uint64_t adesc0 = make_smem_desc(smem_u32(sA));
-            const uint64_t bdesc0 = make_smem_desc(smem_u32(sB));
-            int stage = 0, as = 0;
+            const uint64_t bdesc0 = make_smem_desc(smem_u32(CG == 1 ? sB : sRing));
+            int slot = 0, as = 0;
             uint32_t phase = 0, aphase = 0;
+            auto take = [&]() {
+                const int s = slot;
+                mbar_wait(&full_bar[s], phase);
+                if (++slot == R) {
+                    slot = 0;
+                    phase ^= 1;
+                }
+                return s;
+            };
+            if (S > 0) mbar_wait(res_bar, 0);
             for (int64_t t = worker; t < n_tiles; t += W) {
                 mbar_wait(&tmem_empty_bar[as], aphase ^ 1);
                 tc_fence_after();
                 const uint32_t tmem_d = tmem_base + (uint32_t)(as * BN);
-                for (int kb0 = 0; kb0 < kb_count; kb0 += KPS) {
-                    mbar_wait(&full_bar[stage], phase);
+                for (int kb = 0, r = 0, err = 0; kb < kb_count; kb++) {
+                    int a_slot = -1;
+                    uint64_t adesc;
+                    if (CG == 1) {
+                        adesc = adesc0 + (uint64_t)(slot * (A_BYTES >> 4));
+                    } else if (a_streamed(err)) {
+                        a_slot = take();
+                        adesc = bdesc0 + (uint64_t)(a_slot * (C::B_BYTES >> 4));
+                    } else {
+                        adesc = adesc0 + (uint64_t)((r++) * (A_BYTES >> 4));
+                    }
+                    const int b_slot = take();
+                    const uint64_t bdesc = bdesc0 + (uint64_t)(b_slot * (C::B_BYTES >> 4));
                     tc_fence_after();
                     if (elect_one()) {
-                        for (int sub = 0; sub < KPS; sub++) {
-                            const int slot = stage * KPS + sub;
-                            const uint64_t adesc = adesc0 + (uint64_t)(slot * (A_BYTES >> 4));
-                            const uint64_t bdesc = bdesc0 + (uint64_t)(slot * (C::B_BYTES >> 4));
 #pragma unroll
-                            for (int k = 0; k < BK / UMMA_K; k++) {
-                                const uint32_t acc = (kb0 | sub | k) != 0 ? 1u : 0u;
-                                if (CG == 1) umma(tmem_d, adesc + k * (UMMA_K * 2 >> 4), bdesc + k * (UMMA_K * 2 >> 4), idesc, acc);
-                                else umma_cg2(tmem_d, adesc + k * (UMMA_K * 2 >> 4), bdesc + k * (UMMA_K * 2 >> 4), idesc, acc);
-                            }
+                        for (int k = 0; k < BK / UMMA_K; k++) {
+                            const uint32_t acc = (kb | k) != 0 ? 1u : 0u;
+                            if (CG == 1) umma(tmem_d, adesc + k * (UMMA_K * 2 >> 4), bdesc + k * (UMMA_K * 2 >> 4), idesc, acc);
+                            else umma_cg2(tmem_d, adesc + k * (UMMA_K * 2 >> 4), bdesc + k * (UMMA_K * 2 >> 4), idesc, acc);
                         }
-                        if (CG == 1) umma_commit(&empty_bar[stage]);
-                        else umma_commit_cg2(&empty_bar[stage], (uint16_t)((1u << (CG * MC)) - 1));
-                        if (kb0 + KPS >= kb_count) {
+                        if (CG == 1) {
+                            umma_commit(&empty_bar[b_slot]);
+                        } else {
+                            if (a_slot >= 0) umma_commit_cg2(&empty_bar[a_slot], (uint16_t)((1u << (CG * MC)) - 1));
+                            umma_commit_cg2(&empty_bar[b_slot], (uint16_t)((1u << (CG * MC)) - 1));
+                        }
+                        if (kb + 1 == kb_count) {
                             if (CG == 1) umma_commit(&tmem_full_bar[as]);
                             else umma_commit_cg2(&tmem_full_bar[as], (uint16_t)(3u << leader_rank));
                         }
                     }
                     __syncwarp();
-                    if (++stage == NST) {
-                        stage = 0;
-                        phase ^= 1;
-                    }
                 }
                 if (++as == ACC_STAGES) {
                     as = 0;
@@ -177,15 +212,15 @@
         const int row = quarter * 32 + lane;
         const int et = threadIdx.x - 64;
         const bool use_side = p.row_scale || p.row_bias || p.alive || p.scale_const != -1.f;
-        float *scratch = reinterpret_cast<float *>(smem + C::off_scratch(STAGES)) + et;
+        float *scratch = reinterpret_cast<float *>(smem + C::off_scratch(UNITS)) + et;
         ThreadTopK list;
         list.n = 0;
         list.worst = 0;
         list.thr_key = (qt * BM + row < p.nq_valid) ? FLT_MAX : -FLT_MAX;
         list.thr_id = 0;
         if (p.lists_in_smem)
-            list_bind(list, reinterpret_cast<float *>(smem + C::off_list(STAGES)),
-                      reinterpret_cast<uint32_t *>(smem + C::off_list(STAGES) + (size_t)p.list_cap * EPI_THREADS * 4), row, p.k, p.list_cap);
+            list_bind(list, reinterpret_cast<float *>(smem + C::off_list(UNITS)),
+                      reinterpret_cast<uint32_t *>(smem + C::off_list(UNITS) + (size_t)p.list_cap * EPI_THREADS * 4), row, p.k, p.list_cap);
         else
             list_bind(list, p.list_keys_gmem + (size_t)blockIdx.x * p.list_cap * EPI_THREADS,
                       p.list_ids_gmem + (size_t)blockIdx.x * p.list_cap * EPI_THREADS, row, p.k, p.list_cap);
@@ -274,20 +309,32 @@
     }
 }
 
+struct SmemPlan {
+    int list_cap, lists_in_smem, units;
+    size_t bytes;
+};
+template <int CG>
+static SmemPlan smem_plan(int k) {
+    static const int min_stages = getenv("B200_GEMM_LIST_SMEM_MIN_STAGES") ? atoi(getenv("B200_GEMM_LIST_SMEM_MIN_STAGES")) : 2;
+    using C = Cfg<CG>;
+    SmemPlan sp;
+    sp.list_cap = list_cap_for(k);
+    sp.lists_in_smem = (C::lists_fit(sp.list_cap) && C::units_for(sp.list_cap) * C::UNIT_BYTES >= min_stages * C::STAGE_BYTES) ? 1 : 0;
+    const int k_smem = sp.lists_in_smem ? sp.list_cap : 0;
+    sp.units = C::units_for(k_smem);
+    sp.bytes = (size_t)C::off_list(sp.units) + (size_t)k_smem * EPI_THREADS * 8 + SMEM_ALIGN_SLACK;
+    return sp;
+}
+
 template <int CG, int MC>
 static cudaError_t launch_cg(const CUtensorMap &map_q, const CUtensorMap &map_c, const GemmTopkParams &p_in, int grid,
                              cudaStream_t s) {
     GemmTopkParams p = p_in;
-    static const int min_stages = getenv("B200_GEMM_LIST_SMEM_MIN_STAGES") ? atoi(getenv("B200_GEMM_LIST_SMEM_MIN_STAGES")) : 2;
-    p.list_cap = list_cap_for(p.k);
-    p.lists_in_smem = (Cfg<CG>::lists_fit(p.list_cap) && Cfg<CG>::stages_for(p.list_cap) >= min_stages) ? 1 : 0;
-    const int k_smem = p.lists_in_smem ? p.list_cap : 0;
-    p.stages = Cfg<CG>::stages_for(k_smem);
-    {
-        static const int env_kps = getenv("B200_GEMM_KPS") ? atoi(getenv("B200_GEMM_KPS")) : 1;
-        p.kps = (env_kps == 2 && (p.d_pad / BK) % 2 == 0 && p.stages >= 4) ? 2 : 1;
-    }
-    const size_t smem = (size_t)Cfg<CG>::off_list(p.stages) + (size_t)k_smem * EPI_THREADS * 8 + SMEM_ALIGN_SLACK;
+    const SmemPlan sp = smem_plan<CG>(p.k);
+    p.list_cap = sp.list_cap;
+    p.lists_in_smem = sp.lists_in_smem;
+    p.units = sp.units;
+    const size_t smem = sp.bytes;
     auto kern = gemm_topk_kernel<CG, MC>;
     cudaError_t e = cudaFuncSetAttribute(kern, cudaFuncAttributeMaxDynamicSharedMemorySize, (int)smem);
     if (e != cudaSuccess) return e;
@@ -310,11 +357,7 @@
 
 template <int CG, int MC>
 static int max_clusters(int k) {
-    static const int min_stages = getenv("B200_GEMM_LIST_SMEM_MIN_STAGES") ? atoi(getenv("B200_GEMM_LIST_SMEM_MIN_STAGES")) : 2;
-    const int cap = list_cap_for(k);
-    const int k_smem = (Cfg<CG>::lists_fit(cap) && Cfg<CG>::stages_for(cap) >= min_stages) ? cap : 0;
-    const int stages = Cfg<CG>::stages_for(k_smem);
-    const size_t smem = (size_t)Cfg<CG>::off_list(stages) + (size_t)k_smem * EPI_THREADS * 8 + SMEM_ALIGN_SLACK;
+    const size_t smem = smem_plan<CG>(k).bytes;
     auto kern = gemm_topk_kernel<CG, MC>;
     if (cudaFuncSetAttribute(kern, cudaFuncAttributeMaxDynamicSharedMemorySize, (int)smem) != cudaSuccess) return 0;
     cudaLaunchConfig_t cfg{};
@@ -346,6 +389,12 @@
     return (int)g;
 }
 
+int gemm_resident_kblocks(int cta_group, int d_pad, int k) {
+    if (cta_group != 2 || d_pad < gemm::BK || d_pad % gemm::BK) return 0;
+    const int s = gemm::smem_plan<2>(k).units - kGemmRingMinSlots;
+    return std::max(0, std::min(s, d_pad / gemm::BK));
+}
+
 int gemm_topk_max_clusters(int cta_group, int pairs_per_cluster, int k) {
     if (cta_group == 2 && pairs_per_cluster == 4) return gemm::max_clusters<2, 4>(k);
     if (cta_group == 2 && pairs_per_cluster == 2) return gemm::max_clusters<2, 2>(k);
@@ -361,6 +410,10 @@
         *err_detail = "grid must be a multiple of q_tiles, q_tiles a multiple of the cluster size";
         return cudaErrorInvalidValue;
     }
+    if (p.a_resident < 0 || p.a_resident > gemm_resident_kblocks(cg, p.d_pad, p.k)) {
+        *err_detail = "a_resident exceeds what the shared-memory plan leaves next to the operand ring";
+        return cudaErrorInvalidValue;
+    }
     CUtensorMap map_q, map_c;
     if (!gemm::encode_rows_map(&map_q, p.queries_bf16, p.nq_pad, p.d_pad, gemm::BM) ||
         !gemm::encode_rows_map(&map_c, p.corpus_bf16, p.n, p.d_pad, gemm::BN / cg / mc)) {
diff --git a/myscaledb_b200/csrc/ip_gemm_tf32x3_sm100.cu b/myscaledb_b200/csrc/ip_gemm_tf32x3_sm100.cu
--- a/myscaledb_b200/csrc/ip_gemm_tf32x3_sm100.cu
+++ b/myscaledb_b200/csrc/ip_gemm_tf32x3_sm100.cu
@@ -389,7 +389,6 @@
     GemmTopkParams p = p_in;
     p.list_cap = list_cap_for(p.k);
     p.lists_in_smem = C::lists_fit(p.list_cap) ? 1 : 0;
-    p.stages = C::STAGES;
     const size_t smem = (size_t)C::OFF_LIST + (p.lists_in_smem ? (size_t)p.list_cap * EPI_THREADS * 8 : 0) + SMEM_ALIGN_SLACK;
     auto kern = gemm3_topk_kernel<CG>;
     cudaError_t e = cudaFuncSetAttribute(kern, cudaFuncAttributeMaxDynamicSharedMemorySize, (int)smem);
diff --git a/myscaledb_b200/csrc/kernels.h b/myscaledb_b200/csrc/kernels.h
--- a/myscaledb_b200/csrc/kernels.h
+++ b/myscaledb_b200/csrc/kernels.h
@@ -88,14 +88,15 @@
     int cta_group;
     int pairs_per_cluster;
     int *progress;
-    int stages;
-    int kps;
+    int units;
+    int a_resident;
     int lists_in_smem;
     int list_cap;
     int debug;
     int sync_slack;
 };
 constexpr int kGemmSmemK = 128;
+constexpr int kGemmRingMinSlots = 4;
 __host__ __device__ inline int list_cap_append(int k) { return 2 * k + 32; }
 __host__ __device__ inline int list_tourn_group(int k) { return k <= 64 ? 8 : 16; }
 __host__ __device__ inline int list_cap_tourn(int k) { return k + (k + list_tourn_group(k) - 1) / list_tourn_group(k); }
@@ -103,6 +104,7 @@
 int gemm_topk_grid(int q_tiles, int64_t n, int num_sms);
 cudaError_t launch_gemm_topk(const GemmTopkParams &p, int grid, cudaStream_t s, const char **err_detail);
 int gemm_topk_max_clusters(int cta_group, int pairs_per_cluster, int k);
+int gemm_resident_kblocks(int cta_group, int d_pad, int k);
 bool gemm_topk_ts_supported(int d_pad, int q_tiles);
 int gemm_topk_ts_tile_rows(int d_pad);
 cudaError_t launch_gemm_topk_ts(const GemmTopkParams &p, int grid, cudaStream_t s, const char **err_detail);
diff --git a/myscaledb_b200/search.py b/myscaledb_b200/search.py
--- a/myscaledb_b200/search.py
+++ b/myscaledb_b200/search.py
@@ -113,6 +113,11 @@
         _check(lib().b200_corpus_last_variant(self._h, C.byref(kern), C.byref(cg), C.byref(mc), C.byref(grid)))
         return kern.value, cg.value, mc.value, grid.value
 
+    def last_gemm_resident(self):
+        kb = C.c_int()
+        _check(lib().b200_corpus_last_gemm_resident(self._h, C.byref(kb)))
+        return kb.value
+
     @property
     def size(self):
         n = C.c_int64()
@@ -180,6 +185,12 @@
 
 def launch_count(reset=False) -> int:
     return int(lib().b200_launch_count(C.c_int(1 if reset else 0)))
+
+
+def gemm_resident_kblocks(cta_group: int, d_pad: int, k: int) -> int:
+    out = C.c_int()
+    _check(lib().b200_gemm_resident_kblocks(C.c_int(cta_group), C.c_int(d_pad), C.c_int(k), C.byref(out)))
+    return out.value
 
 
 class BM25Index:
```
